# sbokov/AddingDisparityFiltering

Measured on AMD Instinct MI355X. Metric: filtered Mpixels/s (+ achieved HBM GB/s) on 4K disparity, 1/2/4/8 GPUs vs CPU ref, higher is better.
Workload: dtype f32

## Files before the change

addingdisparityfiltering_amd/__init__.py:

```python
from .ximgproc import (
    AdfError,
    COLOR_BGR2GRAY,
    DisparityFilter,
    DisparityWLSFilter,
    FastGlobalSmootherFilter,
    INTER_LINEAR,
    PATH_CONF_BAND,
    PATH_FUSED_FIRST_PASS,
    PATH_MERGED_PREP,
    PATH_SCALED_FUSED,
    PATH_SCALED_HALF,
    SGBM_COST_BT,
    SGBM_COST_CENSUS_DENSE,
    SGBM_COST_CENSUS_SPARSE,
    SOLVER_EXACT,
    SOLVER_WAVE,
    StereoBM,
    StereoMatcher,
    StereoSGBM,
    UNKNOWN_DISPARITY,
    censusTransform,
    computeBadPixelPercent,
    computeMSE,
    createDisparityWLSFilter,
    createDisparityWLSFilterGeneric,
    createFastGlobalSmootherFilter,
    createRightMatcher,
    cvtColor,
    fastGlobalSmootherFilter,
    filterSpeckles,
    releaseCachedMemory,
    getDisparityVis,
    halfSize,
    matcherViews,
    readGT,
    resize,
    speckleWorkspaceBytes,
)

__version__ = "0.1.0"
```

addingdisparityfiltering_amd/_lib.py:

```python
import ctypes as C
import os

_HERE = os.path.dirname(os.path.abspath(__file__))
LIB_PATH = os.environ.get("ADF_WLS_LIB") or os.path.join(_HERE, "libadf_wls.so")

ADF_OK, ADF_EBADARG, ADF_ESIZE, ADF_EHIP, ADF_ENOMEM, ADF_ENODEV = range(6)
SOLVER_EXACT, SOLVER_WAVE = 0, 1
PATH_CONF_BAND, PATH_FUSED_FIRST_PASS, PATH_MERGED_PREP, PATH_SCALED_FUSED, PATH_SCALED_HALF = 1, 2, 4, 8, 16
DEPTH_8U, DEPTH_16S, DEPTH_32F = 0, 3, 5
SGBM_COST_BT, SGBM_COST_CENSUS_DENSE, SGBM_COST_CENSUS_SPARSE = 0, 1, 2


class AdfError(RuntimeError):

    def __init__(self, code, msg):
        super().__init__("adf error %d: %s" % (code, msg))
        self.code = code


class KernelTime(C.Structure):
    _fields_ = [("name", C.c_char * 48), ("launches", C.c_int), ("total_ms", C.c_double),
                ("alg_bytes", C.c_double), ("moved_bytes", C.c_double)]


class Rect(C.Structure):
    _fields_ = [("x", C.c_int), ("y", C.c_int), ("width", C.c_int), ("height", C.c_int)]


_vp, _i, _d, _pd, _sz = C.c_void_p, C.c_int, C.c_double, C.c_ssize_t, C.c_size_t
_FILTER_DEV = [_vp, _i, _vp, _pd, _pd, _vp, _pd, _pd, _i, _i, _i, _vp, _pd, _pd, _vp, _pd, _pd,
               C.POINTER(Rect), _vp]
_FILTER_SCALED_DEV = [_vp, _i, _vp, _pd, _pd, _i, _i, _vp, _pd, _pd, _i, _i, _i, _vp, _pd, _pd, _vp, _pd, _pd,
                      C.POINTER(Rect), _vp]
SYMBOLS = [
    ("adf_version", _i, []),
    ("adf_last_error", C.c_char_p, []),
    ("adf_device_count", _i, []),
    ("adf_device_pci_bus_id", _i, [_i, C.c_char_p, _i]),
    ("adf_wls_create", _i, [C.POINTER(_vp), _i, _i, _i, _i, _i, _i]),
    ("adf_wls_destroy", None, [_vp]),
    ("adf_wls_set_lambda", _i, [_vp, _d]),
    ("adf_wls_get_lambda", _i, [_vp, C.POINTER(_d)]),
    ("adf_wls_set_sigma_color", _i, [_vp, _d]),
    ("adf_wls_get_sigma_color", _i, [_vp, C.POINTER(_d)]),
    ("adf_wls_set_lrc_thresh", _i, [_vp, _i]),
    ("adf_wls_get_lrc_thresh", _i, [_vp, C.POINTER(_i)]),
    ("adf_wls_set_depth_discontinuity_radius", _i, [_vp, _i]),
    ("adf_wls_get_depth_discontinuity_radius", _i, [_vp, C.POINTER(_i)]),
    ("adf_wls_set_fgs_params", _i, [_vp, _d, _i]),
    ("adf_wls_set_solver", _i, [_vp, _i]),
    ("adf_wls_get_solver", _i, [_vp, C.POINTER(_i)]),
    ("adf_wls_get_last_solver", _i, [_vp, C.POINTER(_i)]),
    ("adf_wls_get_last_path", _i, [_vp, C.POINTER(_i)]),
    ("adf_wls_filter_device", _i, _FILTER_DEV),
    ("adf_wls_filter_host", _i, _FILTER_DEV[:-1]),
    ("adf_wls_filter_scaled_device", _i, _FILTER_SCALED_DEV),
    ("adf_wls_filter_scaled_host", _i, _FILTER_SCALED_DEV[:-1]),
    ("adf_wls_filter_f32_device", _i, _FILTER_DEV),
    ("adf_wls_filter_f32_host", _i, _FILTER_DEV[:-1]),
    ("adf_wls_filter_scaled_f32_device", _i, _FILTER_SCALED_DEV),
    ("adf_wls_filter_scaled_f32_host", _i, _FILTER_SCALED_DEV[:-1]),
    ("adf_wls_get_confidence_device", _i, [_vp, _i, _vp, _pd, _vp]),
    ("adf_wls_get_confidence_host", _i, [_vp, _i, _vp, _pd]),
    ("adf_wls_get_device", _i, [_vp, C.POINTER(_i)]),
    ("adf_wls_get_roi", _i, [_vp, C.POINTER(Rect)]),
    ("adf_wls_sync", _i, [_vp, _vp]),
    ("adf_wls_workspace_bytes", _sz, [_vp]),
    ("adf_wls_profile_enable", _i, [_vp, _i]),
    ("adf_wls_profile_read", _i, [_vp, _vp, _i, C.POINTER(_i)]),
    ("adf_fgs_create", _i, [C.POINTER(_vp), _vp, _pd, _i, _i, _i, _d, _d, _d, _i, _i]),
    ("adf_fgs_create_device", _i, [C.POINTER(_vp), _vp, _pd, _i, _i, _i, _d, _d, _d, _i, _i, _vp]),
    ("adf_fgs_destroy", None, [_vp]),
    ("adf_release_cached_memory", None, []),
    ("adf_weight_table_host", _i, [C.c_float, _vp, _i]),
    ("adf_fgs_get_device", _i, [_vp, C.POINTER(_i)]),
    ("adf_fgs_get_solver", _i, [_vp, C.POINTER(_i)]),
    ("adf_fgs_filter_host", _i, [_vp, _vp, _pd, _vp, _pd, _i, _i]),
    ("adf_fgs_filter_device", _i, [_vp, _vp, _pd, _vp, _pd, _i, _i, _vp]),
    ("adf_compute_mse_host", _i, [_vp, _pd, _vp, _pd, _i, _i, C.POINTER(Rect), C.POINTER(_d)]),
    ("adf_compute_mse_device", _i, [_vp, _pd, _vp, _pd, _i, _i, C.POINTER(Rect), C.POINTER(_d), _vp]),
    ("adf_compute_bad_pixel_percent_host", _i, [_vp, _pd, _vp, _pd, _i, _i, C.POINTER(Rect), _i, C.POINTER(_d)]),
    ("adf_compute_bad_pixel_percent_device", _i, [_vp, _pd, _vp, _pd, _i, _i, C.POINTER(Rect), _i, C.POINTER(_d), _vp]),
    ("adf_get_disparity_vis_host", _i, [_vp, _pd, _vp, _pd, _i, _i, _d]),
    ("adf_get_disparity_vis_device", _i, [_vp, _pd, _vp, _pd, _i, _i, _d, _vp]),
    ("adf_bm_create", _i, [C.POINTER(_vp), _i, _i]),
    ("adf_bm_destroy", None, [_vp]),
    ("adf_bm_set_params", _i, [_vp, _i, _i, _i, _i, _i, _i]),
    ("adf_bm_get_device", _i, [_vp, C.POINTER(_i)]),
    ("adf_bm_get_params", _i, [_vp] + [C.POINTER(_i)] * 6),
    ("adf_bm_compute_device", _i, [_vp, _i, _vp, _pd, _pd, _vp, _pd, _pd, _i, _i, _vp, _pd, _pd, _vp]),
    ("adf_bm_compute_both_device", _i, [_vp, _i, _vp, _pd, _pd, _vp, _pd, _pd, _i, _i, _vp, _pd, _pd, _vp, _pd, _pd, _vp]),
    ("adf_bm_compute_host", _i, [_vp, _i, _vp, _pd, _pd, _vp, _pd, _pd, _i, _i, _vp, _pd, _pd]),
    ("adf_sgbm_create", _i, [C.POINTER(_vp), _i, _i, _i]),
    ("adf_sgbm_destroy", None, [_vp]),
    ("adf_sgbm_get_device", _i, [_vp, C.POINTER(_i)]),
    ("adf_sgbm_set_params", _i, [_vp] + [_i] * 8),
    ("adf_sgbm_get_params", _i, [_vp] + [C.POINTER(_i)] * 8),
    ("adf_sgbm_set_disp12_max_diff", _i, [_vp, _i]),
    ("adf_sgbm_get_disp12_max_diff", _i, [_vp, C.POINTER(_i)]),
    ("adf_sgbm_set_cost", _i, [_vp, _i, _i]),
    ("adf_sgbm_get_cost", _i, [_vp, C.POINTER(_i), C.POINTER(_i)]),
    ("adf_sgbm_compute_device", _i, [_vp, _i, _vp, _pd, _pd, _vp, _pd, _pd, _i, _i, _i, _vp, _pd, _pd, _vp]),
    ("adf_sgbm_compute_host", _i, [_vp, _i, _vp, _pd, _pd, _vp, _pd, _pd, _i, _i, _i, _vp, _pd, _pd]),
    ("adf_census_transform_device", _i, [_i, _vp, _pd, _pd, _i, _i, _i, _i, _vp, _pd, _pd, _vp]),
    ("adf_census_transform_host", _i, [_i, _vp, _pd, _pd, _i, _i, _i, _i, _vp, _pd, _pd]),
    ("adf_filter_speckles_workspace_bytes", _sz, [_i, _i, _i]),
    ("adf_filter_speckles_device", _i, [_i, _vp, _pd, _pd, _i, _i, _i, _i, _i, _vp, _sz, _vp]),
    ("adf_filter_speckles_host", _i, [_i, _vp, _pd, _pd, _i, _i, _i, _i, _i]),
    ("adf_half_size", _i, [_i, C.POINTER(_i)]),
    ("adf_prepare_views_device", _i, [_i, _vp, _pd, _pd, _i, _i, _i, _vp, _pd, _pd, _i, _i, _i, _vp]),
    ("adf_prepare_views_host", _i, [_i, _vp, _pd, _pd, _i, _i, _i, _vp, _pd, _pd, _i, _i, _i]),
]

_lib = None


def lib():
    global _lib
    if _lib is None:
        if not os.path.exists(LIB_PATH):
            raise ImportError(
                "%s is missing: build the HIP extension first "
                "(python -c 'import __graft_entry__ as g; g.build()')" % LIB_PATH)
        L = C.CDLL(LIB_PATH)
        for name, res, args in SYMBOLS:
            try:
                fn = getattr(L, name)
            except AttributeError:
                if os.environ.get("ADF_WLS_LIB"):
                    continue
                raise
            fn.restype = res
            fn.argtypes = args
        _lib = L
    return _lib


def check(rc):
    if rc != ADF_OK:
        raise AdfError(rc, lib().adf_last_error().decode("utf-8", "replace"))


def device_pci_bus_id(device):
    buf = C.create_string_buffer(64)
    check(lib().adf_device_pci_bus_id(int(device), buf, 64))
    return buf.value.decode()
```

addingdisparityfiltering_amd/csrc/adf_api.hip:

```cpp
#include "adf_host.h"

#include <cmath>
#include <cstdio>
#include <cstdlib>
#include <cstring>
#include <new>

using namespace adf;

static inline int round_up(int v, int m) { return (v + m - 1) / m * m; }

static Geom make_geom(int W, int H, int rx, int ry, int rw, int rh)
{
    Geom g;
    g.W = W; g.H = H; g.rx = rx; g.ry = ry; g.rw = rw; g.rh = rh;
    g.pw = round_up(rw, 64);
    g.ph = round_up(rh, 64);
    size_t a = (size_t)round_up(rh, TILE_ROWS) * g.pw, b = (size_t)rw * g.ph;
    g.plane = ((a > b ? a : b) + 63) / 64 * 64;
    g.frame = (size_t)W * H;
    g.cx0 = (4 - (rx & 3)) & 3;
    g.cpitch = round_up(W + g.cx0 + 3, 4);
    g.cframe = (size_t)g.cpitch * H;
    return g;
}

static Geom plain_conf_layout(Geom g) { g.cx0 = 0; g.cpitch = g.W; g.cframe = g.frame; return g; }

enum KClass { K_FILL = 0, K_WEIGHTS, K_DISC, K_LRC, K_PROLOGUE, K_PASS_H_FIRST, K_PASS_H, K_PASS_V, K_PASS_V_LAST, K_RESIZE, K_COUNT };
static const char* const kclass_names[K_COUNT] = {"fill_outside", "weights", "discontinuity", "lrc_confidence",
                                                  "plain_prologue", "pass_h_first", "pass_h", "pass_v", "pass_v_last", "resize"};
struct Profiler {
    bool on = false;
    struct Rec { int cls; hipEvent_t a, b; double alg, moved; };
    std::vector<Rec> recs;
    std::vector<hipEvent_t> pool;
    hipEvent_t get()
    {
        if (!pool.empty()) { hipEvent_t e = pool.back(); pool.pop_back(); return e; }
        hipEvent_t e = nullptr;
        if (hipEventCreate(&e) != hipSuccess) return nullptr;
        return e;
    }
    void clear() { for (auto& r : recs) { pool.push_back(r.a); pool.push_back(r.b); } recs.clear(); }
    void destroy() { clear(); for (auto e : pool) hipEventDestroy(e); pool.clear(); }
};
struct ProfScope {
    Profiler* p; hipStream_t st; Profiler::Rec r{};
    ProfScope(Profiler* prof, int cls, double alg, double moved, hipStream_t s) : p(prof && prof->on ? prof : nullptr), st(s)
    {
        if (!p) return;
        r.cls = cls; r.alg = alg; r.moved = moved; r.a = p->get(); r.b = p->get();
        if (r.a) hipEventRecord(r.a, st);
    }
    ~ProfScope()
    {
        if (!p) return;
        if (r.b) hipEventRecord(r.b, st);
        if (r.a && r.b) p->recs.push_back(r);
    }
};

struct SolvePlanes {
    float* CH; float* CV;
    float* D; float* F0; float* F1;
    float* A0; float* A1;
    float* B0; float* B1;
};

struct FinalOut {
    int epilogue; void* out; ptrdiff_t stride, pair_stride; int x0, y0, cn, c;
};

static double epilogue_bytes(int epilogue)
{
    return (epilogue == EPI_F32 || epilogue == EPI_WLS_CONF_F32) ? 4.0 : epilogue == EPI_U8 ? 1.0 : 2.0;
}

template <class Args>
static void set_final_out(Args& a, const FinalOut& fo)
{
    a.out = fo.out; a.out_stride = fo.stride; a.out_pair_stride = fo.pair_stride;
    a.out_x0 = fo.x0; a.out_y0 = fo.y0; a.out_cn = fo.cn; a.out_c = fo.c;
}

static int run_passes(bool wave, const Geom& g, const SolvePlanes& p, int n_rhs, float lambda, float atten, int num_iter,
                      const FinalOut& fo, int n_pairs, hipStream_t st, Profiler* prof = nullptr,
                      const FusedInputs* fuse = nullptr)
{
    const double px = (double)g.rw * g.rh * n_pairs;
    float lam = lambda;
    for (int it = 0; it < num_iter; it++, lam *= atten) {
        const bool fused = it == 0 && fuse, last = it == num_iter - 1;
        const int epi = last ? fo.epilogue : EPI_PLANES;
        const double lo_b = (fused && fuse->lo_conf) ? 6.0 * fuse->lo_scale_x * fuse->lo_scale_y : 6.0;
        const double hb = fused ? (4.0 + lo_b + 8.0) * px : (4.0 + 8.0 * n_rhs) * px;
        const double out_b = (last ? epilogue_bytes(fo.epilogue) : 4.0 * n_rhs) * px;
        const double vb = (4.0 + 4.0 * n_rhs) * px + out_b;
        if (wave) {
            WavePassArgs h{}, v{};
            h.C = p.CH; h.U0 = p.A0; h.U1 = p.A1;
            h.nscan = g.rh; h.len = g.rw; h.pitch = g.pw; h.plane = g.plane; h.lambda = lam;
            if (fused) h.fuse = *fuse;
            v.C = p.CV; v.U0 = p.A0; v.U1 = p.A1;
            v.nscan = g.rw; v.len = g.rh; v.pitch = g.pw; v.plane = g.plane; v.lambda = lam;
            if (last) set_final_out(v, fo);
            {
                ProfScope ps(prof, fused ? K_PASS_H_FIRST : K_PASS_H, hb, hb, st);
                HIP_TRY(launch_wave_hpass(h, n_rhs, n_pairs, st));
            }
            ProfScope ps(prof, last ? K_PASS_V_LAST : K_PASS_V, vb, vb, st);
            HIP_TRY(launch_wave_vpass(v, n_rhs, epi, n_pairs, st));
        } else {
            PassArgs h{}, v{};
            h.C = p.CH; h.U0 = p.A0; h.U1 = p.A1; h.D = p.D; h.F0 = p.F0; h.F1 = p.F1; h.O0 = p.B0; h.O1 = p.B1;
            h.nscan = g.rh; h.len = g.rw; h.pitch_in = g.ph; h.pitch_out = g.pw; h.plane = g.plane; h.lambda = lam;
            v.C = p.CV; v.U0 = p.B0; v.U1 = p.B1; v.D = p.D; v.F0 = p.F0; v.F1 = p.F1; v.O0 = p.A0; v.O1 = p.A1;
            v.nscan = g.rw; v.len = g.rh; v.pitch_in = g.pw; v.pitch_out = g.ph; v.plane = g.plane; v.lambda = lam;
            if (last) set_final_out(v, fo);
            {
                ProfScope ps(prof, K_PASS_H, hb, (12.0 + 16.0 * n_rhs) * px, st);
                HIP_TRY(launch_exact_pass(h, n_rhs, EPI_PLANES, n_pairs, st));
            }
            ProfScope ps(prof, last ? K_PASS_V_LAST : K_PASS_V, vb, (12.0 + 12.0 * n_rhs) * px + out_b, st);
            HIP_TRY(launch_exact_pass(v, n_rhs, epi, n_pairs, st));
        }
    }
    return ADF_OK;
}

static bool wave_fits(const Geom& g)
{
    return g.rw >= 2 && g.rh >= 2 && g.rw <= wave_max_row_len() && g.rh <= wave_max_col_len();
}

struct ConfResize {
    float* clo; int dW, dH; adf_rect rlo;
    Geom ghi;
    bool band_map;
    int n_pairs;
};

struct adf_wls {
    int device = 0;
    int left_offset = 0, right_offset = 0, top_offset = 0, bottom_offset = 0;
    int min_disp = 0;
    bool use_confidence = true;
    double lambda = 8000.0, sigma_color = 1.0;
    int lrc_thresh = 24, disc_radius = 5;
    float roll_off = 0.001f;
    double atten = 0.25; int num_iter = 3;
    int solver = ADF_SOLVER_WAVE;
    int last_solver = ADF_SOLVER_WAVE;
    adf_rect roi{0, 0, 0, 0};
    int last_W = 0, last_H = 0, last_pairs = 0;
    int last_cpitch = 0, last_cx0 = 0;
    long long conf_sig[4] = {0, 0, 0, 0};
    int last_path = 0;
    Lut lut;
    DevBuf ws;
    DevBuf conf;
    DevBuf stage;
    DevBuf scaled;
    size_t ws_limit = (size_t)64 << 30;
    Profiler prof;
    long long ws_sig[8] = {0, 0, 0, 0, 0, 0, 0, 0};
    hipStream_t side = nullptr;
    hipEvent_t ev_fork = nullptr, ev_join = nullptr;
    bool overlap = true;
    struct LazyConf { bool pending = false; ConfResize resize{}; } lazy_conf;
    bool scaled_half = true;
    bool scaled_fuse = true;
    bool conf_band = true;
    bool merge_small = true;
    static bool null_caller_of(hipStream_t s) { return s == nullptr || s == hipStreamLegacy || s == hipStreamPerThread; }
    int ensure_side(hipStream_t caller)
    {
        if (side) return ADF_OK;
        int least = 0, greatest = 0, prio = 0, cp = 0;
        if (hipDeviceGetStreamPriorityRange(&least, &greatest) != hipSuccess) { least = greatest = 0; (void)hipGetLastError(); }
        if (null_caller_of(caller) || stream_is_capturing(caller) || hipStreamGetPriority(caller, &cp) != hipSuccess) { cp = 0; (void)hipGetLastError(); }
        prio = (cp != greatest) ? greatest : (greatest < least ? greatest + 1 : greatest);
        if (null_caller_of(caller)) HIP_TRY(hipStreamCreateWithFlags(&side, hipStreamNonBlocking));
        else HIP_TRY(hipStreamCreateWithPriority(&side, hipStreamNonBlocking, prio));
        HIP_TRY(hipEventCreateWithFlags(&ev_fork, hipEventDisableTiming));
        HIP_TRY(hipEventCreateWithFlags(&ev_join, hipEventDisableTiming));
        return ADF_OK;
    }
};

extern "C" int adf_wls_create(adf_wls_t** out, int use_confidence, int l, int r, int t, int b, int min_disp)
{
    if (!out) return fail(ADF_EBADARG, "adf_wls_create: out is NULL");
    *out = nullptr;
    if (l < 0 || r < 0 || t < 0 || b < 0) return fail(ADF_EBADARG, "adf_wls_create: negative offset");
    int n = 0;
    if (hipGetDeviceCount(&n) != hipSuccess || n <= 0)
        return fail(ADF_ENODEV, "adf_wls_create: no HIP device visible");
    adf_wls* h = new (std::nothrow) adf_wls();
    if (!h) return fail(ADF_ENOMEM, "adf_wls_create: out of host memory");
    if (hipGetDevice(&h->device) != hipSuccess) { delete h; return fail(ADF_EHIP, "hipGetDevice failed"); }
    h->use_confidence = use_confidence != 0;
    h->left_offset = l; h->right_offset = r; h->top_offset = t; h->bottom_offset = b;
    h->min_disp = 0; (void)min_disp;
    if (const char* e = getenv("ADF_WS_LIMIT_GB")) {
        double gb = atof(e);
        if (gb > 0) h->ws_limit = (size_t)(gb * (double)((size_t)1 << 30));
    }
    if (const char* e = getenv("ADF_NO_OVERLAP")) h->overlap = atoi(e) == 0;
    if (const char* e = getenv("ADF_CONF_BAND")) h->conf_band = atoi(e) != 0;
    if (const char* e = getenv("ADF_SCALED_FUSE")) h->scaled_fuse = atoi(e) != 0;
    if (const char* e = getenv("ADF_LO_HALF")) h->scaled_half = atoi(e) != 0;
    if (const char* e = getenv("ADF_MERGE_SMALL")) h->merge_small = atoi(e) != 0;
    *out = h;
    return ADF_OK;
}

extern "C" void adf_wls_destroy(adf_wls_t* h)
{
    if (!h) return;
    DeviceScope ds(h->device);
    h->lut.release(); h->ws.release(); h->conf.release(); h->stage.release(); h->scaled.release();
    h->prof.destroy();
    if (h->ev_fork) hipEventDestroy(h->ev_fork);
    if (h->ev_join) hipEventDestroy(h->ev_join);
    if (h->side) hipStreamDestroy(h->side);
    delete h;
}


extern "C" int adf_wls_set_lambda(adf_wls_t* h, double v) { NEED_HANDLE(h); h->lambda = v; return ADF_OK; }
extern "C" int adf_wls_get_lambda(const adf_wls_t* h, double* v) { NEED_HANDLE(h); if (v) *v = h->lambda; return ADF_OK; }
extern "C" int adf_wls_set_sigma_color(adf_wls_t* h, double v) { NEED_HANDLE(h); h->sigma_color = v; return ADF_OK; }
extern "C" int adf_wls_get_sigma_color(const adf_wls_t* h, double* v) { NEED_HANDLE(h); if (v) *v = h->sigma_color; return ADF_OK; }
extern "C" int adf_wls_set_lrc_thresh(adf_wls_t* h, int v) { NEED_HANDLE(h); h->lrc_thresh = v; return ADF_OK; }
extern "C" int adf_wls_get_lrc_thresh(const adf_wls_t* h, int* v) { NEED_HANDLE(h); if (v) *v = h->lrc_thresh; return ADF_OK; }
extern "C" int adf_wls_set_depth_discontinuity_radius(adf_wls_t* h, int v) { NEED_HANDLE(h); h->disc_radius = v; return ADF_OK; }
extern "C" int adf_wls_get_depth_discontinuity_radius(const adf_wls_t* h, int* v) { NEED_HANDLE(h); if (v) *v = h->disc_radius; return ADF_OK; }

extern "C" int adf_wls_set_fgs_params(adf_wls_t* h, double atten, int num_iter)
{
    NEED_HANDLE(h);
    if (num_iter < 1) return fail(ADF_EBADARG, "num_iter must be >= 1 (FGS.cpp:143)");
    h->atten = atten; h->num_iter = num_iter;
    return ADF_OK;
}

extern "C" int adf_wls_set_solver(adf_wls_t* h, int solver)
{
    NEED_HANDLE(h);
    if (solver != ADF_SOLVER_EXACT && solver != ADF_SOLVER_WAVE) return fail(ADF_EBADARG, "unknown solver %d", solver);
    h->solver = solver;
    return ADF_OK;
}
extern "C" int adf_wls_get_solver(const adf_wls_t* h, int* v) { NEED_HANDLE(h); if (v) *v = h->solver; return ADF_OK; }
extern "C" int adf_wls_get_last_solver(const adf_wls_t* h, int* v) { NEED_HANDLE(h); if (v) *v = h->last_solver; return ADF_OK; }
extern "C" int adf_wls_get_last_path(const adf_wls_t* h, int* v) { NEED_HANDLE(h); if (v) *v = h->last_path; return ADF_OK; }

extern "C" int adf_wls_get_device(const adf_wls_t* h, int* device) { NEED_HANDLE(h); if (device) *device = h->device; return ADF_OK; }
extern "C" int adf_wls_get_roi(const adf_wls_t* h, adf_rect* roi) { NEED_HANDLE(h); if (roi) *roi = h->roi; return ADF_OK; }
extern "C" size_t adf_wls_workspace_bytes(const adf_wls_t* h)
{
    return h ? h->ws.bytes + h->conf.bytes + h->stage.bytes + h->scaled.bytes + h->lut.bytes() : 0;
}

extern "C" int adf_wls_sync(adf_wls_t* h, void* stream)
{
    NEED_HANDLE(h);
    DeviceScope ds(h->device);
    HIP_TRY(hipStreamSynchronize((hipStream_t)stream));
    return ADF_OK;
}

static int ensure_conf_planes(adf_wls* h, const Geom& g, int n_pairs, hipStream_t st)
{
    int rc = h->conf.reserve(g.cframe * sizeof(float) * (size_t)n_pairs, st, FILL_ZERO);
    if (rc) return rc;
    const long long sig[4] = {g.W, g.H, g.cx0, n_pairs};
    if (memcmp(sig, h->conf_sig, sizeof(sig)) != 0) {
        HIP_TRY(hipMemsetAsync(h->conf.p, 0, h->conf.bytes, st));
        memcpy(h->conf_sig, sig, sizeof(sig));
    }
    return ADF_OK;
}

static size_t wls_pair_ws_bytes(const Geom& g, bool conf, bool wave, bool disc_maps)
{
    size_t planes = wave ? (conf ? 4 : 3) : (conf ? 9 : 6);
    return planes * g.plane * sizeof(float) + (conf && disc_maps ? 2 * g.frame * sizeof(float) : 0);
}

static int resolve_roi(const adf_wls* h, const adf_rect* roi_in, int w, int hgt, adf_rect& roi)
{
    if (roi_in && roi_in->width * roi_in->height != 0) roi = *roi_in;
    else roi = adf_rect{h->left_offset, h->top_offset, w - h->left_offset - h->right_offset, hgt - h->top_offset - h->bottom_offset};
    if (roi.width <= 0 || roi.height <= 0 || roi.x < 0 || roi.y < 0 || roi.x + roi.width > w || roi.y + roi.height > hgt)
        return fail(ADF_ESIZE, "ROI (%d,%d,%d,%d) does not fit a %dx%d map", roi.x, roi.y, roi.width, roi.height, w, hgt);
    return ADF_OK;
}

static int check_right_map(const int16_t* dispR, ptrdiff_t sR, int w)
{
    if (!dispR) return fail(ADF_EBADARG, "disparity_map_right is required with use_confidence");
    if (sR < (ptrdiff_t)w * 2) return fail(ADF_ESIZE, "right disparity stride smaller than a row");
    return ADF_OK;
}

static int check_radius(const adf_wls* h)
{
    if (h->disc_radius < 0 || h->disc_radius > max_disc_radius())
        return fail(ADF_EBADARG, "depth discontinuity radius %d outside [0,%d]", h->disc_radius, max_disc_radius());
    return ADF_OK;
}

static float* const UNALLOCATED = reinterpret_cast<float*>(uintptr_t(256));

static WavePassArgs first_pass_probe(const FusedInputs& f, int len)
{
    WavePassArgs a{};
    a.fuse = f; a.len = len;
    return a;
}

static FusedInputs view_fuse(const float* conf, const int16_t* dl, ptrdiff_t sL, ptrdiff_t psL, const Geom& g)
{
    FusedInputs f{};
    f.conf_in = conf; f.conf_frame = g.cframe; f.conf_pitch = g.cpitch; f.conf_x0 = g.cx0 + g.rx; f.conf_y0 = g.ry;
    f.dl_in = dl; f.dl_stride = sL; f.dl_pair_stride = psL; f.dl_x0 = g.rx; f.dl_y0 = g.ry;
    return f;
}

struct ScaledStage {
    const int16_t* dispL; ptrdiff_t sL, psL;
    const int16_t* dispR; ptrdiff_t sR, psR;
    float resize_factor, x_ratio;
    char* dhi; size_t dhi_bytes;
    float *cl, *cr;
    ConfResize lo;
    bool fuse_lo;
    float* taps;
};

static FusedInputs lo_fuse(const adf_wls* h, const ScaledStage& s, int first, const Geom& g)
{
    const ConfResize& c = s.lo;
    const size_t lo = (size_t)c.dW * c.dH;
    FusedInputs f{};
    f.lo_conf = c.clo + (size_t)first * lo; f.lo_conf_stride = c.dW; f.lo_conf_pair = (ptrdiff_t)lo;
    f.lo_dl = (const int16_t*)((const char*)s.dispL + (ptrdiff_t)first * s.psL); f.lo_dl_stride = s.sL; f.lo_dl_pair = s.psL;
    f.lo_w = c.dW; f.lo_h = c.dH; f.hi_x0 = g.rx; f.hi_y0 = g.ry;
    f.lo_scale_x = (double)c.dW / c.ghi.W; f.lo_scale_y = (double)c.dH / c.ghi.H; f.lo_post_scale = s.x_ratio;
    if (c.band_map) {
        f.lo_zero_outside = 1; f.lo_vx0 = c.rlo.x; f.lo_vy0 = c.rlo.y; f.lo_vx1 = c.rlo.x + c.rlo.width; f.lo_vy1 = c.rlo.y + c.rlo.height;
    }
    f.lo_taps = s.taps; f.lo_half = h->scaled_half ? 1 : 0;
    return f;
}

static int resize_conf_planes(adf_wls_t* h, const ConfResize& c, hipStream_t st, Profiler* prof)
{
    const size_t lo = (size_t)c.dW * c.dH;
    const Geom& ghi = c.ghi;
    const double Fhi = (double)ghi.W * ghi.H * c.n_pairs;
    ResizeArgs rc32{c.clo, (ptrdiff_t)c.dW * 4, (ptrdiff_t)(lo * 4), c.dW, c.dH, (float*)h->conf.p + ghi.cx0, (ptrdiff_t)ghi.cpitch * 4,
                    (ptrdiff_t)(ghi.cframe * 4), ghi.W, ghi.H, (double)c.dW / ghi.W, (double)c.dH / ghi.H, 1.0f, 0};
    if (c.band_map) { rc32.zero_outside = 1; rc32.vx0 = c.rlo.x; rc32.vy0 = c.rlo.y; rc32.vx1 = c.rlo.x + c.rlo.width; rc32.vy1 = c.rlo.y + c.rlo.height; }
    ProfScope ps(prof, K_RESIZE, 4.0 * Fhi + 4.0 * (double)lo * c.n_pairs, 4.0 * Fhi + 4.0 * (double)lo * c.n_pairs, st);
    HIP_TRY(launch_resize_linear(rc32, c.n_pairs, st));
    return ADF_OK;
}

static int scaled_conf_map(adf_wls_t* h, const ScaledStage& s, hipStream_t st, Profiler* prof)
{
    const ConfResize& c = s.lo;
    const Geom glo = plain_conf_layout(make_geom(c.dW, c.dH, c.rlo.x, c.rlo.y, c.rlo.width, c.rlo.height));
    const size_t lo = (size_t)c.dW * c.dH;
    const double Plo = (double)c.rlo.width * c.rlo.height * c.n_pairs;
    const int rrx = c.dW - (c.rlo.x + c.rlo.width);
    const float roll_off = h->roll_off / (s.resize_factor * s.resize_factor);
    const int thresh_lo = (int)(s.resize_factor * h->lrc_thresh);
    if (c.band_map) {
        ConfBandArgs ba{s.dispL, s.sL, s.psL, s.dispR, s.sR, s.psR, c.clo, glo, rrx, thresh_lo, h->disc_radius, roll_off, 0};
        ProfScope ps(prof, K_LRC, 8.0 * Plo, 8.0 * Plo, st);
        HIP_TRY(launch_conf_band(ba, c.n_pairs, st));
        return ADF_OK;
    }
    DiscArgs da{{s.dispL, s.dispR}, {s.sL, s.sR}, {s.psL, s.psR}, {c.rlo.x, rrx}, c.rlo.y, c.rlo.width, c.rlo.height,
                h->disc_radius, roll_off, {s.cl, s.cr}, c.dW, lo, -1};
    {
        ProfScope ps(prof, K_DISC, 4.0 * Plo, 12.0 * Plo, st);
        HIP_TRY(launch_discontinuity(da, c.n_pairs, st));
    }
    LrcArgs la{s.dispL, s.sL, s.psL, s.dispR, s.sR, s.psR, s.cl, s.cr, c.clo, nullptr, 0, 0, 0, 0, nullptr, nullptr, glo, rrx, thresh_lo, ORIENT_N};
    ProfScope ps(prof, K_LRC, 4.0 * (double)lo * c.n_pairs, 4.0 * (double)lo * c.n_pairs + 12.0 * Plo, st);
    HIP_TRY(launch_lrc_prologue(la, c.n_pairs, st));
    return ADF_OK;
}

static int scaled_resize(adf_wls_t* h, const ScaledStage& s, hipStream_t st, Profiler* prof)
{
    const ConfResize& c = s.lo;
    int rc = h->use_confidence ? resize_conf_planes(h, c, st, prof) : ADF_OK;
    if (rc) return rc;
    const int W = c.ghi.W, H = c.ghi.H;
    const size_t lo = (size_t)c.dW * c.dH;
    const double Fhi = (double)W * H * c.n_pairs;
    ResizeArgs r16{s.dispL, s.sL, s.psL, c.dW, c.dH, s.dhi, (ptrdiff_t)W * 2, (ptrdiff_t)s.dhi_bytes, W, H, (double)c.dW / W, (double)c.dH / H, s.x_ratio, 1};
    ProfScope ps(prof, K_RESIZE, 2.0 * Fhi + 2.0 * (double)lo * c.n_pairs, 2.0 * Fhi + 2.0 * (double)lo * c.n_pairs, st);
    HIP_TRY(launch_resize_linear(r16, c.n_pairs, st));
    return ADF_OK;
}

enum ConfStage {
    CONF_NONE,
    CONF_SCALED,
    CONF_SCALED_LO,
    CONF_MERGED,
    CONF_BAND,
    CONF_LEFT,
    CONF_TWO_KERNEL,
};

struct ChunkPlan {
    ConfStage stage;
    bool fork_weights;
    bool outside_on_side;
};

struct WlsPlan {
    bool wave;
    bool fused_first;
    bool band;
    size_t per_pair; int chunk;
    ChunkPlan full, tail;
    int path;
};

static ChunkPlan plan_chunk(const adf_wls* h, ConfStage stage, bool wave)
{
    const bool fork = stage != CONF_NONE && stage != CONF_MERGED && h->overlap;
    return ChunkPlan{stage, fork, fork && wave && stage != CONF_TWO_KERNEL};
}

static WlsPlan plan_wls(const adf_wls* h, const Geom& g, int n_pairs, const int16_t* dispL, ptrdiff_t sL, ptrdiff_t psL,
                        ptrdiff_t sG, int gch, const ScaledStage* scaled)
{
    WlsPlan p{};
    const bool conf = h->use_confidence;
    p.wave = h->solver == ADF_SOLVER_WAVE && wave_fits(g);
    ConfStage stage = !conf ? CONF_NONE
                    : scaled ? (scaled->fuse_lo ? CONF_SCALED_LO : CONF_SCALED)
                    : (p.wave && h->disc_radius <= conf_left_max_radius()) ? CONF_LEFT : CONF_TWO_KERNEL;
    const float* planes = h->conf.p ? (const float*)h->conf.p : UNALLOCATED;
    p.fused_first = stage == CONF_SCALED_LO ||
                    ((stage == CONF_SCALED || stage == CONF_LEFT) && p.wave &&
                     wave_hpass_can_fuse(first_pass_probe(view_fuse(planes, dispL, sL, psL, g), g.rw)));
    p.band = stage == CONF_LEFT && p.fused_first && h->conf_band && conf_band_fits(g, h->disc_radius);
    if (p.band) stage = CONF_BAND;
    p.per_pair = wls_pair_ws_bytes(g, conf, p.wave, !p.band);
    p.chunk = (int)(h->ws_limit / p.per_pair);
    if (p.chunk < 1) p.chunk = 1;
    if (p.chunk > n_pairs) p.chunk = n_pairs;
    auto chunk_of = [&](int n) {
        const bool merged = p.band && h->merge_small && prep_small_fits(g, h->disc_radius, gch, n) && prep_small_guide_fits(g, sG, gch);
        return plan_chunk(h, merged ? CONF_MERGED : stage, p.wave);
    };
    p.full = chunk_of(p.chunk);
    p.tail = chunk_of(n_pairs % p.chunk ? n_pairs % p.chunk : p.chunk);
    p.path = ((p.band || (scaled && scaled->lo.band_map)) ? ADF_PATH_CONF_BAND : 0) |
             (p.fused_first ? ADF_PATH_FUSED_FIRST_PASS : 0) |
             ((p.full.stage == CONF_MERGED || p.tail.stage == CONF_MERGED) ? ADF_PATH_MERGED_PREP : 0);
    if (stage == CONF_SCALED_LO)
        p.path |= ADF_PATH_SCALED_FUSED |
                  (wave_hpass_lo_half(first_pass_probe(lo_fuse(h, *scaled, 0, g), g.rw)) ? ADF_PATH_SCALED_HALF : 0);
    return p;
}

struct OutMap {
    void* p; ptrdiff_t stride, pair_stride; bool f32;
    size_t esz() const { return f32 ? sizeof(float) : sizeof(int16_t); }
};

static int wls_filter_impl(adf_wls_t* h, int n_pairs,
                           const int16_t* dispL, ptrdiff_t sL, ptrdiff_t psL,
                           const uint8_t* view, ptrdiff_t sG, ptrdiff_t psG, int gch, int W, int H,
                           const OutMap& om,
                           const int16_t* dispR, ptrdiff_t sR, ptrdiff_t psR,
                           const adf_rect* roi_in, hipStream_t st, const ScaledStage* scaled = nullptr)
{
    NEED_HANDLE(h);
    if (!dispL || W <= 0 || H <= 0) return fail(ADF_EBADARG, "disparity_map_left is empty");
    if (!view || (gch != 1 && gch != 3)) return fail(ADF_EBADARG, "left_view must be CV_8UC1 or CV_8UC3");
    void* const out = om.p;
    const ptrdiff_t sO = om.stride, psO = om.pair_stride;
    const double ob_px = (double)om.esz();
    if (!out) return fail(ADF_EBADARG, "filtered_disparity_map is NULL");
    if (n_pairs < 1) return fail(ADF_EBADARG, "n_pairs must be >= 1");
    if (sL < (ptrdiff_t)W * 2 || sO < (ptrdiff_t)(W * om.esz()) || sG < (ptrdiff_t)W * gch)
        return fail(ADF_ESIZE, "row stride smaller than a row");
    if (om.f32 && ((reinterpret_cast<uintptr_t>(out) | (uintptr_t)sO | (uintptr_t)psO) & 3u))
        return fail(ADF_EBADARG, "a float filtered_disparity_map needs a 4-byte aligned base and strides");
    const bool conf = h->use_confidence;
    int rc;
    if (conf && !scaled && (rc = check_right_map(dispR, sR, W))) return rc;
    if (h->lambda < 0 || h->sigma_color < 0) return fail(ADF_EBADARG, "lambda and sigma_color must be >= 0 (FGS.cpp:143)");
    adf_rect roi;
    if ((rc = resolve_roi(h, roi_in, W, H, roi))) return rc;
    if (conf && (rc = check_radius(h))) return rc;

    DeviceScope ds(h->device);
    const Geom g = make_geom(W, H, roi.x, roi.y, roi.width, roi.height);
    h->lazy_conf.pending = false;
    h->roi = roi; h->last_W = W; h->last_H = H; h->last_pairs = n_pairs;
    h->last_cpitch = g.cpitch; h->last_cx0 = g.cx0; h->last_path = 0;

    if ((rc = h->lut.ensure((float)h->sigma_color, st))) return rc;
    const WlsPlan plan = plan_wls(h, g, n_pairs, dispL, sL, psL, sG, gch, scaled);
    const bool wave = plan.wave;
    h->last_solver = wave ? ADF_SOLVER_WAVE : ADF_SOLVER_EXACT;
    if ((rc = h->ws.reserve(plan.per_pair * (size_t)plan.chunk, st, FILL_ZERO))) return rc;
    if (conf && !scaled && (rc = ensure_conf_planes(h, g, n_pairs, st))) return rc;
    {
        const long long sig[8] = {W, H, roi.x, roi.y, roi.width, roi.height, (long long)plan.band * 4 + (long long)wave * 2 + conf, plan.chunk};
        if (memcmp(sig, h->ws_sig, sizeof(sig)) != 0) {
            HIP_TRY(hipMemsetAsync(h->ws.p, 0, h->ws.bytes, st));
            memcpy(h->ws_sig, sig, sizeof(sig));
        }
    }
    float* base = (float*)h->ws.p;
    auto take = [&](size_t elems) { float* p = base; base += elems * (size_t)plan.chunk; return p; };
    SolvePlanes p{};
    p.CH = take(g.plane); p.CV = take(g.plane); p.A0 = take(g.plane);
    if (!wave) { p.D = take(g.plane); p.F0 = take(g.plane); p.B0 = take(g.plane); }
    float *cL = nullptr, *cR = nullptr;
    if (conf) {
        p.A1 = take(g.plane);
        if (!wave) { p.F1 = take(g.plane); p.B1 = take(g.plane); }
        if (!plan.band) { cL = take(g.frame); cR = take(g.frame); }
    }
    const int orient_h = wave ? ORIENT_N : ORIENT_T;
    const int orient_u2 = wave ? ORIENT_PAIR : ORIENT_T;
    const int orient_cv = wave ? ORIENT_STRIP : ORIENT_N;
    const int16_t fill = (int16_t)(16 * (h->min_disp - 1));
    const int rrx = W - (roi.x + roi.width);
    const int thresh = (int)(1.0f * h->lrc_thresh);
    Profiler* prof = &h->prof;
    h->last_path = plan.path;

    for (int first = 0; first < n_pairs; first += plan.chunk) {
        const int n = (n_pairs - first < plan.chunk) ? n_pairs - first : plan.chunk;
        const ChunkPlan& cp = n == plan.chunk ? plan.full : plan.tail;
        const int16_t* dL = (const int16_t*)((const char*)dispL + (ptrdiff_t)first * psL);
        const int16_t* dR = dispR ? (const int16_t*)((const char*)dispR + (ptrdiff_t)first * psR) : nullptr;
        const uint8_t* gv = view + (ptrdiff_t)first * psG;
        void* o = (char*)out + (ptrdiff_t)first * psO;
        float* confp = conf ? (float*)h->conf.p + (size_t)first * g.cframe : nullptr;
        const double F = (double)g.frame * n, P = (double)g.rw * g.rh * n;
        OutsideArgs oa{o, sO, psO, fill, om.f32 ? 1 : 0, scaled ? nullptr : confp, g};
        const double ob = ((oa.conf ? 4.0 : 0.0) + ob_px) * (F - P);
        auto fill_outside = [&](hipStream_t s) { ProfScope ps(prof, K_FILL, ob, ob, s); return launch_outside(oa, n, s); };
        WeightArgs wa{gv, sG, psG, gch, h->lut.cur, p.CH, p.CV, orient_h, orient_cv, g,
                      wave ? nullptr : p.B0};
        ConfBandArgs ba{dL, sL, psL, dR, sR, psR, confp, g, rrx, thresh, h->disc_radius, h->roll_off, 0};
        DiscArgs da{{dL, dR}, {sL, sR}, {psL, psR}, {roi.x, rrx}, roi.y, roi.width, roi.height, h->disc_radius, h->roll_off,
                    {cL, cR}, W, g.frame, cp.stage == CONF_LEFT ? 1 : -1};
        const FusedInputs fuse = cp.stage == CONF_SCALED_LO ? lo_fuse(h, *scaled, first, g) : view_fuse(confp, dL, sL, psL, g);

        hipStream_t wst = st;
        if (cp.fork_weights) {
            if ((rc = h->ensure_side(st))) return rc;
            HIP_TRY(hipEventRecord(h->ev_fork, st));
            HIP_TRY(hipStreamWaitEvent(h->side, h->ev_fork, 0));
            wst = h->side;
        }
        if (cp.stage == CONF_NONE || cp.outside_on_side) HIP_TRY(fill_outside(wst));
        if (cp.stage == CONF_NONE && scaled && first == 0 && (rc = scaled_resize(h, *scaled, st, prof))) return rc;
        if (cp.stage != CONF_MERGED) {
            ProfScope ps(prof, K_WEIGHTS, (gch + 8.0) * P, (gch + 8.0) * P, wst);
            HIP_TRY(launch_weights(wa, n, wst));
        }
        if (cp.fork_weights) HIP_TRY(hipEventRecord(h->ev_join, h->side));

        switch (cp.stage) {
        case CONF_NONE: {
            PlainPrologueArgs pa{dL, sL, psL, ADF_16S, 1, 0, p.A0, g, orient_h};
            ProfScope ps(prof, K_PROLOGUE, 6.0 * P, 6.0 * P, st);
            HIP_TRY(launch_plain_prologue(pa, n, st));
            break;
        }
        case CONF_SCALED: {
            if (!cp.outside_on_side) HIP_TRY(fill_outside(st));
            if (first == 0 && ((rc = scaled_conf_map(h, *scaled, st, prof)) || (rc = scaled_resize(h, *scaled, st, prof)))) return rc;
            if (plan.fused_first) break;
            PlainPrologueArgs pa{dL, sL, psL, ADF_16S, 1, 0, p.A0, g, orient_u2, confp, p.A1};
            ProfScope ps(prof, K_PROLOGUE, 14.0 * P, 14.0 * P, st);
            HIP_TRY(launch_plain_prologue(pa, n, st));
            break;
        }
        case CONF_SCALED_LO:
            if (!cp.outside_on_side) HIP_TRY(fill_outside(st));
            if (first != 0) break;
            if ((rc = scaled_conf_map(h, *scaled, st, prof))) return rc;
            if (!stream_is_capturing(st)) h->lazy_conf = adf_wls::LazyConf{true, scaled->lo};
            else if ((rc = resize_conf_planes(h, scaled->lo, st, prof))) return rc;
            break;
        case CONF_MERGED: {
            const double b = (8.0 + gch + 8.0) * P + (4.0 + ob_px) * (F - P);
            ProfScope ps(prof, K_LRC, b, b, st);
            HIP_TRY(launch_prep_small(ba, wa, oa, n, st));
            break;
        }
        case CONF_BAND: {
            {
                ProfScope ps(prof, K_LRC, 8.0 * P, 8.0 * P, st);
                HIP_TRY(launch_conf_band(ba, n, st));
            }
            if (!cp.outside_on_side) HIP_TRY(fill_outside(st));
            break;
        }
        case CONF_LEFT: {
            {
                ProfScope ps(prof, K_DISC, 2.0 * P, 6.0 * P, st);
                HIP_TRY(launch_discontinuity(da, n, st));
            }
            const bool fused = plan.fused_first;
            ConfLeftArgs ca{dL, sL, psL, dR, sR, psR, cR, confp, fused ? nullptr : p.A0, fused ? nullptr : p.A1,
                            g, rrx, thresh, h->disc_radius, h->roll_off};
            {
                const double wu = fused ? 0.0 : 8.0;
                ProfScope ps(prof, K_LRC, (4.0 + wu) * P, (12.0 + wu) * P, st);
                HIP_TRY(launch_conf_left(ca, n, st));
            }
            if (!cp.outside_on_side) HIP_TRY(fill_outside(st));
            break;
        }
        case CONF_TWO_KERNEL: {
            {
                ProfScope ps(prof, K_DISC, 4.0 * P, 12.0 * P, st);
                HIP_TRY(launch_discontinuity(da, n, st));
            }
            LrcArgs la{dL, sL, psL, dR, sR, psR, cL, cR, confp, o, sO, psO, fill, om.f32 ? 1 : 0, p.A0, p.A1, g, rrx, thresh, orient_u2};
            ProfScope ps(prof, K_LRC, 4.0 * F + 8.0 * P + ob_px * (F - P), 4.0 * F + 20.0 * P + ob_px * (F - P), st);
            HIP_TRY(launch_lrc_prologue(la, n, st));
            break;
        }
        }
        if (cp.fork_weights) HIP_TRY(hipStreamWaitEvent(st, h->ev_join, 0));
        const int epi = conf ? (om.f32 ? EPI_WLS_CONF_F32 : EPI_WLS_CONF) : (om.f32 ? EPI_F32 : EPI_I16);
        FinalOut fo{epi, o, sO, psO, roi.x, roi.y, 1, 0};
        rc = run_passes(wave, g, p, conf ? 2 : 1, (float)h->lambda, (float)h->atten, h->num_iter, fo, n, st, prof,
                        plan.fused_first ? &fuse : nullptr);
        if (rc) return rc;
    }
    return ADF_OK;
}

static int wls_filter_scaled_device(adf_wls_t* h, int n_pairs,
                                    const int16_t* dispL, ptrdiff_t sL, ptrdiff_t psL, int dW, int dH,
                                    const uint8_t* view, ptrdiff_t sG, ptrdiff_t psG, int gch, int W, int H,
                                    const OutMap& om,
                                    const int16_t* dispR, ptrdiff_t sR, ptrdiff_t psR,
                                    const adf_rect* roi_in, hipStream_t st)
{
    NEED_HANDLE(h);
    if (dW == W && dH == H)
        return wls_filter_impl(h, n_pairs, dispL, sL, psL, view, sG, psG, gch, W, H, om, dispR, sR, psR, roi_in, st);
    if (!dispL || dW <= 0 || dH <= 0 || W <= 0 || H <= 0) return fail(ADF_EBADARG, "disparity_map_left is empty");
    if (n_pairs < 1) return fail(ADF_EBADARG, "n_pairs must be >= 1");
    if (sL < (ptrdiff_t)dW * 2) return fail(ADF_ESIZE, "row stride smaller than a row");
    const bool conf = h->use_confidence;
    int rc;
    if (conf && ((rc = check_right_map(dispR, sR, dW)) || (rc = check_radius(h)))) return rc;
    adf_rect rlo;
    if ((rc = resolve_roi(h, roi_in, dW, dH, rlo))) return rc;
    const float resize_factor = dW / (float)W;
    const float x_ratio = W / (float)dW, y_ratio = H / (float)dH;
    adf_rect rhi{(int)(rlo.x * x_ratio), (int)(rlo.y * y_ratio), (int)(rlo.width * x_ratio), (int)(rlo.height * y_ratio)};
    if (rhi.width <= 0 || rhi.height <= 0 || rhi.x + rhi.width > W || rhi.y + rhi.height > H)
        return fail(ADF_ESIZE, "scaled ROI (%d,%d,%d,%d) does not fit the %dx%d view", rhi.x, rhi.y, rhi.width, rhi.height, W, H);

    DeviceScope ds(h->device);
    h->lazy_conf.pending = false;
    const size_t lo = (size_t)dW * dH, hi = (size_t)W * H;
    const Geom ghi = make_geom(W, H, rhi.x, rhi.y, rhi.width, rhi.height);
    ScaledStage s{dispL, sL, psL, dispR, sR, psR, resize_factor, x_ratio, nullptr, 0, nullptr, nullptr,
                  ConfResize{UNALLOCATED, dW, dH, rlo, ghi, false, n_pairs}, false, nullptr};
    s.lo.band_map = conf && h->conf_band &&
                    conf_band_fits(plain_conf_layout(make_geom(dW, dH, rlo.x, rlo.y, rlo.width, rlo.height)), h->disc_radius);
    s.fuse_lo = conf && h->scaled_fuse && h->solver == ADF_SOLVER_WAVE && wave_fits(ghi) &&
                wave_hpass_can_fuse_lo(first_pass_probe(lo_fuse(h, s, 0, ghi), ghi.rw));
    s.dhi_bytes = s.fuse_lo ? 0 : (hi * 2 + 255) / 256 * 256;
    const size_t maps_bytes = ((size_t)n_pairs * (s.dhi_bytes + (conf ? 3 * lo * sizeof(float) : 0)) + 255) / 256 * 256;
    const size_t need = maps_bytes + (s.fuse_lo ? 2 * ((size_t)rhi.width + 4) * sizeof(float) : 0);
    if ((rc = h->scaled.reserve(need, st, FILL_ZERO))) return rc;
    s.dhi = (char*)h->scaled.p;
    s.cl = (float*)(s.dhi + (size_t)n_pairs * s.dhi_bytes);
    s.cr = s.cl + (size_t)n_pairs * lo;
    s.lo.clo = s.cr + (size_t)n_pairs * lo;
    s.taps = s.fuse_lo ? (float*)((char*)h->scaled.p + maps_bytes) : nullptr;
    if (conf && (rc = ensure_conf_planes(h, ghi, n_pairs, st))) return rc;
    rc = wls_filter_impl(h, n_pairs, s.fuse_lo ? dispL : (const int16_t*)s.dhi, (ptrdiff_t)W * 2, (ptrdiff_t)s.dhi_bytes,
                         view, sG, psG, gch, W, H, om, nullptr, 0, 0, &rhi, st, &s);
    h->roi = rlo;
    return rc;
}

static int wls_filter_scaled_host(adf_wls_t* h, int n_pairs,
                                  const int16_t* dispL, ptrdiff_t sL, ptrdiff_t psL, int dW, int dH,
                                  const uint8_t* view, ptrdiff_t sG, ptrdiff_t psG, int gch, int W, int H,
                                  const OutMap& om,
                                  const int16_t* dispR, ptrdiff_t sR, ptrdiff_t psR,
                                  const adf_rect* roi)
{
    NEED_HANDLE(h);
    if (!dispL || !view || !om.p || W <= 0 || H <= 0 || dW <= 0 || dH <= 0 || n_pairs < 1)
        return fail(ADF_EBADARG, "adf_wls_filter_host: empty input");
    if (gch != 1 && gch != 3) return fail(ADF_EBADARG, "left_view must be CV_8UC1 or CV_8UC3");
    if (h->use_confidence && !dispR) return fail(ADF_EBADARG, "disparity_map_right is required with use_confidence");
    DeviceScope ds(h->device);
    hipStream_t st = nullptr;
    const size_t orow = (size_t)W * om.esz();
    const size_t dbytes = (size_t)dW * dH * 2, obytes = orow * H, gbytes = (size_t)W * H * gch;
    const size_t dpad = (dbytes + 255) / 256 * 256, opad = (obytes + 255) / 256 * 256, gpad = (gbytes + 255) / 256 * 256;
    const size_t need = (size_t)n_pairs * (2 * dpad + opad + gpad);
    int rc = h->stage.reserve(need, st, FILL_ZERO);
    if (rc) return rc;
    char* dLd = (char*)h->stage.p;
    char* dRd = dLd + (size_t)n_pairs * dpad;
    char* od = dRd + (size_t)n_pairs * dpad;
    char* gd = od + (size_t)n_pairs * opad;
    if ((rc = copy_images(dLd, (size_t)dW * 2, dpad, dispL, sL, psL, (size_t)dW * 2, dH, n_pairs, hipMemcpyHostToDevice, st))) return rc;
    if (dispR && (rc = copy_images(dRd, (size_t)dW * 2, dpad, dispR, sR, psR, (size_t)dW * 2, dH, n_pairs, hipMemcpyHostToDevice, st))) return rc;
    if ((rc = copy_images(gd, (size_t)W * gch, gpad, view, sG, psG, (size_t)W * gch, H, n_pairs, hipMemcpyHostToDevice, st))) return rc;
    rc = wls_filter_scaled_device(h, n_pairs, (const int16_t*)dLd, (ptrdiff_t)dW * 2, (ptrdiff_t)dpad, dW, dH,
                                  (const uint8_t*)gd, (ptrdiff_t)W * gch, (ptrdiff_t)gpad, gch, W, H,
                                  OutMap{od, (ptrdiff_t)orow, (ptrdiff_t)opad, om.f32},
                                  dispR ? (const int16_t*)dRd : nullptr, (ptrdiff_t)dW * 2, (ptrdiff_t)dpad, roi, st);
    if (rc) return rc;
    if ((rc = copy_images(om.p, om.stride, om.pair_stride, od, orow, opad, orow, H, n_pairs, hipMemcpyDeviceToHost, st))) return rc;
    HIP_TRY(hipStreamSynchronize(st));
    return ADF_OK;
}

#define ADF_WLS_SAME_ARGS const int16_t* dispL, ptrdiff_t sL, ptrdiff_t psL, \
                          const uint8_t* view, ptrdiff_t sG, ptrdiff_t psG, int gch, int W, int H
#define ADF_WLS_SCALED_ARGS const int16_t* dispL, ptrdiff_t sL, ptrdiff_t psL, int dW, int dH, \
                            const uint8_t* view, ptrdiff_t sG, ptrdiff_t psG, int gch, int W, int H
#define ADF_WLS_RIGHT_ARGS const int16_t* dispR, ptrdiff_t sR, ptrdiff_t psR, const adf_rect* roi
#define ADF_WLS_ENTRIES(SUFFIX, T, F32)                                                                                       \
    extern "C" int adf_wls_filter##SUFFIX##_device(adf_wls_t* h, int n_pairs, ADF_WLS_SAME_ARGS, T* out, ptrdiff_t sO,        \
                                                   ptrdiff_t psO, ADF_WLS_RIGHT_ARGS, void* stream)                           \
    {                                                                                                                         \
        return wls_filter_impl(h, n_pairs, dispL, sL, psL, view, sG, psG, gch, W, H, OutMap{out, sO, psO, F32}, dispR, sR,    \
                               psR, roi, (hipStream_t)stream);                                                                \
    }                                                                                                                         \
    extern "C" int adf_wls_filter_scaled##SUFFIX##_device(adf_wls_t* h, int n_pairs, ADF_WLS_SCALED_ARGS, T* out,             \
                                                          ptrdiff_t sO, ptrdiff_t psO, ADF_WLS_RIGHT_ARGS, void* stream)      \
    {                                                                                                                         \
        return wls_filter_scaled_device(h, n_pairs, dispL, sL, psL, dW, dH, view, sG, psG, gch, W, H,                         \
                                        OutMap{out, sO, psO, F32}, dispR, sR, psR, roi, (hipStream_t)stream);                 \
    }                                                                                                                         \
    extern "C" int adf_wls_filter_scaled##SUFFIX##_host(adf_wls_t* h, int n_pairs, ADF_WLS_SCALED_ARGS, T* out, ptrdiff_t sO, \
                                                        ptrdiff_t psO, ADF_WLS_RIGHT_ARGS)                                    \
    {                                                                                                                         \
        return wls_filter_scaled_host(h, n_pairs, dispL, sL, psL, dW, dH, view, sG, psG, gch, W, H,                           \
                                      OutMap{out, sO, psO, F32}, dispR, sR, psR, roi);                                        \
    }                                                                                                                         \
    extern "C" int adf_wls_filter##SUFFIX##_host(adf_wls_t* h, int n_pairs, ADF_WLS_SAME_ARGS, T* out, ptrdiff_t sO,          \
                                                 ptrdiff_t psO, ADF_WLS_RIGHT_ARGS)                                           \
    {                                                                                                                         \
        return wls_filter_scaled_host(h, n_pairs, dispL, sL, psL, W, H, view, sG, psG, gch, W, H, OutMap{out, sO, psO, F32},  \
                                      dispR, sR, psR, roi);                                                                   \
    }
ADF_WLS_ENTRIES(, int16_t, false)
ADF_WLS_ENTRIES(_f32, float, true)
#undef ADF_WLS_ENTRIES
#undef ADF_WLS_SAME_ARGS
#undef ADF_WLS_SCALED_ARGS
#undef ADF_WLS_RIGHT_ARGS

extern "C" int adf_wls_profile_enable(adf_wls_t* h, int on)
{
    NEED_HANDLE(h);
    DeviceScope ds(h->device);
    h->prof.clear();
    h->prof.on = on != 0;
    return ADF_OK;
}

extern "C" int adf_wls_profile_read(adf_wls_t* h, adf_kernel_time* out, int capacity, int* count)
{
    NEED_HANDLE(h);
    if (!out || !count || capacity < 1) return fail(ADF_EBADARG, "adf_wls_profile_read: bad output buffer");
    DeviceScope ds(h->device);
    adf_kernel_time acc[K_COUNT];
    memset(acc, 0, sizeof(acc));
    for (int k = 0; k < K_COUNT; k++) snprintf(acc[k].name, sizeof(acc[k].name), "%s", kclass_names[k]);
    for (auto& r : h->prof.recs) {
        HIP_TRY(hipEventSynchronize(r.b));
        float ms = 0.0f;
        HIP_TRY(hipEventElapsedTime(&ms, r.a, r.b));
        acc[r.cls].launches++; acc[r.cls].total_ms += ms; acc[r.cls].alg_bytes += r.alg; acc[r.cls].moved_bytes += r.moved;
    }
    int n = 0;
    for (int k = 0; k < K_COUNT && n < capacity; k++)
        if (acc[k].launches) out[n++] = acc[k];
    *count = n;
    return ADF_OK;
}

static int conf_copy(adf_wls_t* h, int pair, float* dst, ptrdiff_t stride, hipMemcpyKind kind, hipStream_t st)
{
    if (!dst) return fail(ADF_EBADARG, "confidence destination is NULL");
    if (!h->use_confidence || !h->conf.p || h->last_pairs == 0)
        return fail(ADF_EBADARG, "no confidence map: filter() has not run with use_confidence");
    if (pair < 0 || pair >= h->last_pairs) return fail(ADF_EBADARG, "pair %d out of range [0,%d)", pair, h->last_pairs);
    if (stride < (ptrdiff_t)h->last_W * 4) return fail(ADF_ESIZE, "confidence stride smaller than a row");
    if (h->lazy_conf.pending) {
        int rc = resize_conf_planes(h, h->lazy_conf.resize, st, nullptr);
        if (rc) return rc;
        h->lazy_conf.pending = false;
    }
    const float* src = (const float*)h->conf.p + (size_t)pair * h->last_cpitch * h->last_H + h->last_cx0;
    HIP_TRY(hipMemcpy2DAsync(dst, stride, src, (size_t)h->last_cpitch * 4, (size_t)h->last_W * 4, h->last_H, kind, st));
    return ADF_OK;
}

extern "C" int adf_wls_get_confidence_device(adf_wls_t* h, int pair, float* dst, ptrdiff_t stride, void* stream)
{
    NEED_HANDLE(h);
    DeviceScope ds(h->device);
    return conf_copy(h, pair, dst, stride, hipMemcpyDeviceToDevice, (hipStream_t)stream);
}

extern "C" int adf_wls_get_confidence_host(adf_wls_t* h, int pair, float* dst, ptrdiff_t stride)
{
    NEED_HANDLE(h);
    DeviceScope ds(h->device);
    int rc = conf_copy(h, pair, dst, stride, hipMemcpyDeviceToHost, nullptr);
    if (rc) return rc;
    HIP_TRY(hipStreamSynchronize(nullptr));
    return ADF_OK;
}

struct adf_fgs {
    int device = 0;
    int w = 0, h = 0;
    float lambda = 0, sigma = 0, atten = 0.25f; int num_iter = 3; int solver = ADF_SOLVER_EXACT;
    Geom g{};
    Lut lut;
    void* block = nullptr; size_t block_bytes = 0;
    DevBuf planes, io;
    hipEvent_t busy = nullptr;
    bool in_capture = false;
};

static int fgs_begin(adf_fgs* f, hipStream_t st)
{
    if (f->busy && !stream_is_capturing(st)) HIP_TRY(hipStreamWaitEvent(st, f->busy, 0));
    return ADF_OK;
}

static int fgs_end(adf_fgs* f, hipStream_t st)
{
    if (stream_is_capturing(st)) { f->in_capture = true; return ADF_OK; }
    if (f->busy) HIP_TRY(hipEventRecord(f->busy, st));
    return ADF_OK;
}

static int fgs_create_impl(adf_fgs_t** out, const uint8_t* guide, ptrdiff_t gstride, int gch, int w, int hgt,
                           double lambda, double sigma_color, double atten, int num_iter, int solver,
                           bool guide_on_device, hipStream_t st)
{
    if (!out) return fail(ADF_EBADARG, "adf_fgs_create: out is NULL");
    *out = nullptr;
    if (!guide || w <= 0 || hgt <= 0) return fail(ADF_EBADARG, "guide is empty");
    if (lambda < 0 || sigma_color < 0 || num_iter < 1) return fail(ADF_EBADARG, "lambda>=0, sigma_color>=0, num_iter>=1 required");
    if (gch != 1 && gch != 3) return fail(ADF_EBADARG, "guide must be CV_8UC1 or CV_8UC3");
    if (gstride < (ptrdiff_t)w * gch) return fail(ADF_ESIZE, "guide stride smaller than a row");
    if (solver != ADF_SOLVER_EXACT && solver != ADF_SOLVER_WAVE) return fail(ADF_EBADARG, "unknown solver %d", solver);
    int n = 0;
    if (hipGetDeviceCount(&n) != hipSuccess || n <= 0) return fail(ADF_ENODEV, "adf_fgs_create: no HIP device visible");
    adf_fgs* f = new (std::nothrow) adf_fgs();
    if (!f) return fail(ADF_ENOMEM, "out of host memory");
    hipGetDevice(&f->device);
    f->w = w; f->h = hgt;
    f->lambda = (float)lambda; f->sigma = (float)sigma_color; f->atten = (float)atten;
    f->num_iter = num_iter;
    f->g = make_geom(w, hgt, 0, 0, w, hgt);
    f->solver = (solver == ADF_SOLVER_WAVE && wave_fits(f->g)) ? ADF_SOLVER_WAVE : ADF_SOLVER_EXACT;
    int rc = f->lut.ensure(f->sigma, st);
    if (rc) { adf_fgs_destroy(f); return rc; }
    const size_t gbytes = (size_t)w * hgt * gch;
    const size_t planes_bytes = (6 * f->g.plane * sizeof(float) + 255) / 256 * 256;
    const size_t io_bytes = ((gbytes > (size_t)w * hgt * 16 ? gbytes : (size_t)w * hgt * 16) + 255) / 256 * 256;
    hipError_t e = hipSuccess;
    f->block = cache_take(f->device, planes_bytes + io_bytes, st, &f->block_bytes);
    if (!f->block) {
        e = device_malloc(&f->block, planes_bytes + io_bytes);
        if (e != hipSuccess) {
            f->block = nullptr; adf_fgs_destroy(f);
            return fail(e == hipErrorOutOfMemory ? ADF_ENOMEM : ADF_EHIP, "adf_fgs_create: %s", hipGetErrorString(e));
        }
        f->block_bytes = planes_bytes + io_bytes;
    }
    f->planes.p = f->block; f->planes.bytes = planes_bytes;
    f->io.p = (char*)f->block + planes_bytes; f->io.bytes = io_bytes;
    e = hipMemsetAsync(f->block, 0, planes_bytes + io_bytes, st);
    if (e == hipSuccess) e = hipEventCreateWithFlags(&f->busy, hipEventDisableTiming);
    if (e == hipSuccess) e = guide_on_device
        ? hipMemcpy2DAsync(f->io.p, (size_t)w * gch, guide, gstride, (size_t)w * gch, hgt, hipMemcpyDeviceToDevice, st)
        : hipMemcpy2D(f->io.p, (size_t)w * gch, guide, gstride, (size_t)w * gch, hgt, hipMemcpyHostToDevice);
    if (e == hipSuccess) {
        float* base = (float*)f->planes.p;
        WeightArgs wa{(const uint8_t*)f->io.p, (ptrdiff_t)w * gch, 0, gch, f->lut.cur,
                      base, base + f->g.plane, f->solver == ADF_SOLVER_WAVE ? ORIENT_N : ORIENT_T,
                      f->solver == ADF_SOLVER_WAVE ? ORIENT_STRIP : ORIENT_N, f->g,
                      f->solver == ADF_SOLVER_WAVE ? nullptr : base + 5 * f->g.plane};
        e = launch_weights(wa, 1, st);
    }
    if (e == hipSuccess && !guide_on_device) e = hipStreamSynchronize(st);
    if (e != hipSuccess) { hipStreamSynchronize(st); adf_fgs_destroy(f); return fail(ADF_EHIP, "adf_fgs_create: %s", hipGetErrorString(e)); }
    if ((rc = fgs_end(f, st))) { hipStreamSynchronize(st); adf_fgs_destroy(f); return rc; }
    *out = f;
    return ADF_OK;
}

extern "C" int adf_fgs_create(adf_fgs_t** out, const uint8_t* guide, ptrdiff_t gstride, int gch, int w, int hgt,
                              double lambda, double sigma_color, double atten, int num_iter, int solver)
{
    return fgs_create_impl(out, guide, gstride, gch, w, hgt, lambda, sigma_color, atten, num_iter, solver, false, nullptr);
}

extern "C" int adf_fgs_create_device(adf_fgs_t** out, const uint8_t* guide, ptrdiff_t gstride, int gch, int w, int hgt,
                                     double lambda, double sigma_color, double atten, int num_iter, int solver, void* stream)
{
    return fgs_create_impl(out, guide, gstride, gch, w, hgt, lambda, sigma_color, atten, num_iter, solver, true,
                           (hipStream_t)stream);
}

extern "C" int adf_fgs_get_device(const adf_fgs_t* f, int* device) { NEED_HANDLE(f); if (device) *device = f->device; return ADF_OK; }
extern "C" int adf_fgs_get_solver(const adf_fgs_t* f, int* solver) { NEED_HANDLE(f); if (solver) *solver = f->solver; return ADF_OK; }

extern "C" void adf_fgs_destroy(adf_fgs_t* f)
{
    if (!f) return;
    DeviceScope ds(f->device);
    if (f->block) {
        if (f->busy && !f->in_capture) {
            cache_give_event(f->device, f->block, f->block_bytes, f->busy);
            f->busy = nullptr;
        } else {
            hipDeviceSynchronize();
            hipFree(f->block);
// ... 79 lines not shown
```

addingdisparityfiltering_amd/csrc/adf_internal.h:

```cpp
#pragma once

#include <hip/hip_runtime.h>
#include <stddef.h>
#include <stdint.h>
#include "../../include/adf_wls.h"

#define ADF_LUT_LEVELS (3 * 256 * 256)
#define ADF_EPS 1e-43f

namespace adf {

struct Geom {
    int W, H;
    int rx, ry, rw, rh;
    int pw, ph;
    size_t plane;
    size_t frame;
    int cpitch, cx0;
    size_t cframe;
};

enum Orient { ORIENT_N = 0, ORIENT_T = 1, ORIENT_PAIR = 2, ORIENT_STRIP = 3 };
#define ADF_STRIP 16
constexpr int TILE_ROWS = 2;

enum Epilogue {
    EPI_PLANES = 0,
    EPI_WLS_CONF = 1,
    EPI_I16 = 2,
    EPI_F32 = 3,
    EPI_U8 = 4,
    EPI_WLS_CONF_F32 = 5
};
constexpr int N_EPILOGUES = EPI_WLS_CONF_F32 + 1;

struct DiscArgs {
    const int16_t* disp[2]; ptrdiff_t stride[2], pair_stride[2];
    int rx[2]; int ry, rw, rh;
    int radius; float roll_off;
    float* dst[2]; int W; size_t frame;
    int only_view;
};

struct ConfLeftArgs {
    const int16_t* dL; ptrdiff_t sL, psL;
    const int16_t* dR; ptrdiff_t sR, psR;
    const float* cR;
    float* conf;
    float* U0; float* U1;
    Geom g; int rrx; int thresh;
    int radius; float roll_off;
};

struct ConfBandArgs {
    const int16_t* dL; ptrdiff_t sL, psL;
    const int16_t* dR; ptrdiff_t sR, psR;
    float* conf;
    Geom g; int rrx; int thresh;
    int radius; float roll_off;
    int rows_per_band;
};

struct OutsideArgs {
    void* out; ptrdiff_t stride, pair_stride; int16_t fill; int out_f32;
    float* conf;
    Geom g;
};

struct LrcArgs {
    const int16_t* dL; ptrdiff_t sL, psL;
    const int16_t* dR; ptrdiff_t sR, psR;
    const float* cL; const float* cR;
    float* conf;
    void* out; ptrdiff_t sO, psO; int16_t fill; int out_f32;
    float* U0; float* U1;
    Geom g; int rrx;
    int thresh; int orient;
};

struct PlainPrologueArgs {
    const void* src; ptrdiff_t stride, pair_stride;
    int depth, cn, c;
    float* U0; Geom g; int orient;
    const float* conf; float* U1;
    int pair2, c2;
};

struct ResizeArgs {
    const void* src; ptrdiff_t sstride, spair; int sw, sh;
    void* dst; ptrdiff_t dstride, dpair; int dw, dh;
    double scale_x, scale_y;
    float post_scale; int is16;
    int zero_outside = 0, vx0 = 0, vy0 = 0, vx1 = 0, vy1 = 0;
};

struct WeightArgs {
    const uint8_t* guide; ptrdiff_t stride, pair_stride; int ch;
    const float* lut;
    float* chor; float* cvert; int chor_orient, cvert_orient;
    Geom g;
    float* scratch;
};

struct PassArgs {
    const float* C; const float* U0; const float* U1;
    float* D; float* F0; float* F1;
    float* O0; float* O1;
    void* out; ptrdiff_t out_stride, out_pair_stride;
    int out_x0, out_y0, out_cn, out_c;
    int nscan, len, pitch_in, pitch_out;
    size_t plane;
    float lambda;
};

struct FusedInputs {
    const float* conf_in; size_t conf_frame; int conf_pitch, conf_x0, conf_y0;
    const int16_t* dl_in; ptrdiff_t dl_stride, dl_pair_stride; int dl_x0, dl_y0;
    const float* lo_conf; ptrdiff_t lo_conf_stride, lo_conf_pair;
    const int16_t* lo_dl; ptrdiff_t lo_dl_stride, lo_dl_pair;
    int lo_w, lo_h, hi_x0, hi_y0;
    double lo_scale_x, lo_scale_y; float lo_post_scale;
    int lo_zero_outside, lo_vx0, lo_vy0, lo_vx1, lo_vy1;
    int lo_half;
    float* lo_taps;
};

struct WavePassArgs {
    const float* C; float* U0; float* U1;
    FusedInputs fuse;
    void* out; ptrdiff_t out_stride, out_pair_stride;
    int out_x0, out_y0, out_cn, out_c;
    int nscan, len, pitch;
    size_t plane;
    float lambda;
};
static_assert(sizeof(WavePassArgs) == 280 && offsetof(WavePassArgs, out) == 208 && offsetof(WavePassArgs, nscan) == 248 &&
              offsetof(WavePassArgs, plane) == 264 && offsetof(WavePassArgs, lambda) == 272, "WavePassArgs layout");

hipError_t launch_discontinuity(const DiscArgs& a, int n_pairs, hipStream_t st);
hipError_t launch_lrc_prologue(const LrcArgs& a, int n_pairs, hipStream_t st);
hipError_t launch_conf_left(const ConfLeftArgs& a, int n_pairs, hipStream_t st);
hipError_t launch_outside(const OutsideArgs& a, int n_pairs, hipStream_t st);
bool conf_band_fits(const Geom& g, int radius);
hipError_t launch_conf_band(const ConfBandArgs& a, int n_pairs, hipStream_t st);
bool prep_small_guide_fits(const Geom& g, ptrdiff_t guide_stride, int channels);
bool prep_small_fits(const Geom& g, int radius, int channels, int n_pairs);
hipError_t launch_prep_small(const ConfBandArgs& c, const WeightArgs& w, const OutsideArgs& o, int n_pairs, hipStream_t st);
int conf_left_max_radius();
hipError_t launch_plain_prologue(const PlainPrologueArgs& a, int n_pairs, hipStream_t st);
hipError_t launch_weights(const WeightArgs& a, int n_pairs, hipStream_t st);
hipError_t launch_resize_linear(const ResizeArgs& a, int n_pairs, hipStream_t st);
hipError_t launch_exact_pass(const PassArgs& a, int n_rhs, int epilogue, int n_pairs, hipStream_t st);
hipError_t launch_wave_hpass(const WavePassArgs& a, int n_rhs, int n_pairs, hipStream_t st);
hipError_t launch_wave_vpass(const WavePassArgs& a, int n_rhs, int epilogue, int n_pairs, hipStream_t st);
int wave_max_row_len();
bool wave_hpass_can_fuse(const WavePassArgs& a);
bool wave_hpass_can_fuse_lo(const WavePassArgs& a);
bool wave_hpass_lo_half(const WavePassArgs& a);
int wave_max_col_len();
int max_disc_radius();

namespace tile {
constexpr int TX = 64;
constexpr int TY = 32;
constexpr int NT = 256;
}

#if defined(__HIPCC__)
__device__ __forceinline__ size_t pair_index(int i, int j, int pw)
{
    constexpr int TR = TILE_ROWS;
    return (size_t)(i / TR) * (size_t)(2 * TR * pw) + (size_t)((j >> 4) * (32 * TR) + (i % TR) * 32 + (j & 15));
}
__device__ __forceinline__ size_t strip_index(int i, int j, int rh)
{
    return ((size_t)(j >> 4) * (size_t)rh + (size_t)i) * ADF_STRIP + (size_t)(j & 15);
}
struct RhsPlanes { float* U0; float* U1; };
__device__ __forceinline__ RhsPlanes rhs_planes(float* U0, float* U1, int orient, size_t pz, size_t plane)
{
    const bool pair = orient == ORIENT_PAIR;
    float* u0 = U0 + pz * (pair ? 2 : 1) * plane;
    return RhsPlanes{u0, pair ? u0 + ADF_STRIP : U1 ? U1 + pz * plane : nullptr};
}
__device__ __forceinline__ size_t rhs_index(int orient, int i, int j, const Geom& g)
{
    return orient == ORIENT_PAIR ? pair_index(i, j, g.pw) : orient == ORIENT_T ? (size_t)j * g.ph + i : (size_t)i * g.pw + j;
}
struct RhsTile {
    float t0[tile::TX * (tile::TY + 1)], t1[tile::TX * (tile::TY + 1)];
    __device__ __forceinline__ void stage(int tx, int y, float v0, float v1) { t0[tx * (tile::TY + 1) + y] = v0; t1[tx * (tile::TY + 1) + y] = v1; }
    __device__ __forceinline__ void store(float* U0, float* U1, const Geom& g, int j0, int i0) const
    {
        __syncthreads();
#pragma unroll
        for (int m = 0; m < tile::TX / 8; m++) {
            const int cidx = threadIdx.x / tile::TY + 8 * m, ridx = threadIdx.x % tile::TY, j = j0 + cidx, i = i0 + ridx;
            if ((unsigned)j < (unsigned)g.rw && (unsigned)i < (unsigned)g.rh) {
                const size_t o = rhs_index(ORIENT_T, i, j, g);
                U0[o] = t0[cidx * (tile::TY + 1) + ridx];
                if (U1) U1[o] = t1[cidx * (tile::TY + 1) + ridx];
            }
        }
    }
};
__device__ __forceinline__ void store_fill(void* map, ptrdiff_t row_offset_bytes, int j, int16_t fill, int f32)
{
    char* row = reinterpret_cast<char*>(map) + row_offset_bytes;
    if (f32) reinterpret_cast<float*>(row)[j] = (float)fill;
    else reinterpret_cast<int16_t*>(row)[j] = fill;
}
__device__ __forceinline__ float wls_f32_value(float x) { return !(__builtin_fabsf(x) < 2147483648.0f) ? -32768.0f : x; }
__device__ __forceinline__ int16_t sat16(float v)
{
    if (!(v >= -2147483648.0f && v < 2147483648.0f)) return (int16_t)-32768;
    float r = rintf(v);
    r = fminf(fmaxf(r, -32768.0f), 32767.0f);
    return (int16_t)(int)r;
}
__device__ __forceinline__ uint8_t sat8(float v)
{
    if (!(v >= -2147483648.0f && v < 2147483648.0f)) return (uint8_t)0;
    float r = rintf(v);
    r = fminf(fmaxf(r, 0.0f), 255.0f);
    return (uint8_t)(int)r;
}
__device__ __forceinline__ int reflect101(int p, int len)
{
    if (len == 1) return 0;
    while (p < 0 || p >= len) p = p < 0 ? -p : 2 * (len - 1) - p;
    return p;
}
#endif

}
```

addingdisparityfiltering_amd/csrc/fgs_wave_h.hip:

```cpp
#include "fgs_wave_common.h"

#include <algorithm>

namespace adf {

namespace {
using namespace wave;

constexpr int H_TWO_WAVE_MAX = 60;

constexpr int FUSE_NONE = 0, FUSE_VIEW = 1, FUSE_LO = 2, FUSE_LO_HALF = 3;

typedef float v4f __attribute__((ext_vector_type(4)));

struct RowPos {
    int lane, wv;
    int v0;
    int nvec;
    int nvecU;
    size_t off;
    size_t offU;
};

template <int M, bool PAIR, int NW>
__device__ __forceinline__ RowPos row_pos(const WavePassArgs& a)
{
    constexpr int TR = TILE_ROWS;
    RowPos p;
    p.lane = threadIdx.x & 63; p.wv = NW == 2 ? (int)(threadIdx.x >> 6) : 0;
    p.v0 = p.wv * 16 * M;
    p.off = (size_t)blockIdx.y * a.plane + (size_t)blockIdx.x * a.pitch;
    p.nvec = a.pitch >> 2;
    p.offU = PAIR ? (size_t)blockIdx.y * 2 * a.plane + (size_t)(blockIdx.x / TR) * (size_t)(2 * TR * a.pitch) + (size_t)(blockIdx.x % TR) * 32 : p.off;
    p.nvecU = PAIR ? 2 * p.nvec : p.nvec;
    return p;
}

template <bool PAIR>
__device__ __forceinline__ constexpr int rhs_vec(int q) { return PAIR ? (((q >> 3) * (8 * TILE_ROWS)) + (q & 7)) : q; }

__device__ __forceinline__ constexpr int pair_slot(int j) { return ((j >> 4) << 3) + ((j & 15) >> 2); }

__device__ __forceinline__ float4 load_nt(const float4* p)
{
    const v4f q = __builtin_nontemporal_load(reinterpret_cast<const v4f*>(p));
    return make_float4(q.x, q.y, q.z, q.w);
}
__device__ __forceinline__ void store_nt(float4 q, float4* p)
{
    const v4f o = {q.x, q.y, q.z, q.w};
    __builtin_nontemporal_store(o, reinterpret_cast<v4f*>(p));
}


__device__ __forceinline__ float4 load_c(const WavePassArgs& a, const RowPos& p, int k)
{
    const int idx = p.v0 + 64 * k + p.lane;
    float4 t = make_float4(0.f, 0.f, 0.f, 0.f);
    if (idx < p.nvec) t = load_nt(reinterpret_cast<const float4*>(a.C + p.off) + idx);
    return t;
}

template <int M, int R>
__device__ __forceinline__ void load_planes(const WavePassArgs& a, const RowPos& p, float4 (&tC)[M / 4], float4 (&t0)[M / 4], float4 (&t1)[M / 4])
{
    constexpr bool PAIR = R > 1;
    constexpr int MQ = M / 4;
    const float4* s0 = reinterpret_cast<const float4*>(a.U0 + p.offU);
    const int u0 = PAIR ? 2 * p.v0 : p.v0;
#pragma unroll
    for (int k = 0; k < MQ; k++) {
        const int uidx = u0 + 64 * k + p.lane;
        tC[k] = load_c(a, p, k);
        t0[k] = make_float4(0.f, 0.f, 0.f, 0.f); t1[k] = t0[k];
        if (uidx < p.nvecU) t0[k] = load_nt(s0 + rhs_vec<PAIR>(uidx));
        if (PAIR && uidx + 64 * MQ < p.nvecU) t1[k] = load_nt(s0 + rhs_vec<PAIR>(uidx + 64 * MQ));
    }
}

__device__ __forceinline__ int fused_vecs(int len) { return (len >> 2) + ((len & 3) ? 1 : 0); }

template <int M>
__device__ __forceinline__ void load_fused_view(const WavePassArgs& a, const RowPos& p, float4 (&tC)[M / 4], float4 (&t0)[M / 4], float4 (&t1)[M / 4])
{
    constexpr int MQ = M / 4;
    typedef short v4s_u __attribute__((ext_vector_type(4), aligned(2)));
    const float4* sF = reinterpret_cast<const float4*>(a.fuse.conf_in + (size_t)blockIdx.y * a.fuse.conf_frame +
                                                       (size_t)(a.fuse.conf_y0 + blockIdx.x) * a.fuse.conf_pitch + a.fuse.conf_x0);
    const char* sD = reinterpret_cast<const char*>(a.fuse.dl_in) + (ptrdiff_t)blockIdx.y * a.fuse.dl_pair_stride +
                     (ptrdiff_t)(a.fuse.dl_y0 + blockIdx.x) * a.fuse.dl_stride + (ptrdiff_t)a.fuse.dl_x0 * 2;
    const int nfull = a.len >> 2, rem = a.len & 3;
    const int nfused = fused_vecs(a.len);
    const unsigned dl_last = (unsigned)a.len * 2u - 8u;
    short4 draw[MQ];
#pragma unroll
    for (int k = 0; k < MQ; k++) {
        const int idx = p.v0 + 64 * k + p.lane;
        tC[k] = load_c(a, p, k);
        t0[k] = make_float4(0.f, 0.f, 0.f, 0.f); t1[k] = t0[k];
        draw[k] = make_short4(0, 0, 0, 0);
        if (idx < nfused) {
            const unsigned doff = min((unsigned)idx * 8u, dl_last);
            t1[k] = load_nt(sF + idx);
            const v4s_u dq = __builtin_nontemporal_load(reinterpret_cast<const v4s_u*>(sD + doff));
            draw[k] = make_short4(dq.x, dq.y, dq.z, dq.w);
        }
    }
    const int tl = nfull - p.v0;
    const int ktail = (rem && tl >= 0 && tl < 16 * M) ? (tl >> 6) : -1;
#pragma unroll
    for (int k = 0; k < MQ; k++) {
        if (k == ktail && p.lane == (tl & 63)) {
            const int sh = 16 * (4 - rem);
            unsigned long long w = (unsigned long long)(unsigned short)draw[k].x | ((unsigned long long)(unsigned short)draw[k].y << 16) |
                                   ((unsigned long long)(unsigned short)draw[k].z << 32) | ((unsigned long long)(unsigned short)draw[k].w << 48);
            w >>= sh;
            draw[k] = make_short4((short)(w & 0xffff), (short)((w >> 16) & 0xffff), (short)((w >> 32) & 0xffff), (short)(w >> 48));
            if (rem < 2) t1[k].y = 0.0f;
            if (rem < 3) t1[k].z = 0.0f;
            t1[k].w = 0.0f;
        }
        t0[k] = make_float4(t1[k].x * (float)draw[k].x, t1[k].y * (float)draw[k].y, t1[k].z * (float)draw[k].z, t1[k].w * (float)draw[k].w);
    }
}

__host__ __device__ __forceinline__ void lin_tap(int d, double scale, int sn, int& s0, float& fx)
{
    fx = (float)(((double)d + 0.5) * scale - 0.5);
    s0 = (int)floorf(fx);
    fx -= (float)s0;
    if (s0 < 0) { fx = 0.0f; s0 = 0; }
    if (s0 >= sn - 1) { fx = 0.0f; s0 = sn - 1; }
}
__global__ void __launch_bounds__(256) lo_tap_table_kernel(float* table, int n, int len, int hi_x0, double scale, int sn)
{
    const int j = blockIdx.x * 256 + threadIdx.x;
    if (j >= n) return;
    int s0; float fx;
    lin_tap(hi_x0 + min(j, len - 1), scale, sn, s0, fx);
    table[j] = (float)s0 + fx;
}
__host__ __device__ constexpr int lo_row_cap(int m) { return (((m * 64) / 3) & ~7) < 168 ? 168 : (((m * 64) / 3) & ~7); }
__host__ __device__ constexpr int lo_stage_vec4(int m) { return 12 * lo_row_cap(m) > 256 * m ? (12 * lo_row_cap(m) + 15) / 16 : m * 16; }

template <int M>
struct LoShape {
    static constexpr int MQ = M / 4;
    static constexpr int KH = (MQ + 1) / 2;
    static constexpr int CROW = lo_row_cap(M);
    static constexpr int TC4 = (CROW / 4 + 63) / 64, TD8 = (CROW / 8 + 63) / 64;
    static_assert(12 * CROW <= 16 * lo_stage_vec4(M) && CROW % 8 == 0, "two confidence rows and two disparity rows fit the staging buffer");
};
typedef float f4u __attribute__((ext_vector_type(4), aligned(4)));
typedef short s8u __attribute__((ext_vector_type(8), aligned(2)));

template <int M>
struct LoRaw { v4f c[2][LoShape<M>::TC4]; s8u d[2][LoShape<M>::TD8]; };

struct LoRow {
    int yr[2];
    float b0, b1;
    int ss[2], ns[2];
    bool need_mask[2];
};

template <int M>
__device__ __forceinline__ LoRow lo_row(const FusedInputs& f, int wv, int len)
{
    constexpr int MQ = LoShape<M>::MQ, KH = LoShape<M>::KH;
    const int sw = f.lo_w, sh = f.lo_h;
    LoRow r;
    int sy; float fy;
    {
        const int dy = f.hi_y0 + (int)blockIdx.x;
        fy = (float)(((double)dy + 0.5) * f.lo_scale_y - 0.5);
        sy = (int)floorf(fy);
        fy -= (float)sy;
    }
    r.b0 = 1.0f - fy; r.b1 = fy;
    r.yr[0] = min(max(sy, 0), sh - 1); r.yr[1] = min(max(sy + 1, 0), sh - 1);
    r.yr[0] = __builtin_amdgcn_readfirstlane(r.yr[0]); r.yr[1] = __builtin_amdgcn_readfirstlane(r.yr[1]);
#pragma unroll
    for (int hh = 0; hh < 2; hh++) {
        const int cfirst = 64 * M * wv + 256 * (hh ? KH : 0);
        const int clast = min(64 * M * wv + 256 * (hh ? MQ : KH), len) - 1;
        int s_first = 0, s_last = -2; float f_;
        if (clast >= cfirst) { lin_tap(f.hi_x0 + cfirst, f.lo_scale_x, sw, s_first, f_); lin_tap(f.hi_x0 + clast, f.lo_scale_x, sw, s_last, f_); }
        r.ss[hh] = __builtin_amdgcn_readfirstlane(s_first);
        r.ns[hh] = __builtin_amdgcn_readfirstlane(s_last + 2 - s_first);
    }
#pragma unroll
    for (int hh = 0; hh < 2; hh++)
        r.need_mask[hh] = f.lo_zero_outside && (r.yr[0] < f.lo_vy0 || r.yr[1] >= f.lo_vy1 || r.ss[hh] < f.lo_vx0 || min(r.ss[hh] + r.ns[hh], sw) > f.lo_vx1);
    return r;
}

template <int M>
__device__ inline void lo_fetch(const FusedInputs& f, const LoRow& row, int hh, int lane, LoRaw<M>& q)
{
    const int sw = f.lo_w;
    const float* cbase = f.lo_conf + (ptrdiff_t)blockIdx.y * f.lo_conf_pair;
    const char* dbase = reinterpret_cast<const char*>(f.lo_dl) + (ptrdiff_t)blockIdx.y * f.lo_dl_pair;
#pragma unroll
    for (int r = 0; r < 2; r++) {
        const float* crow = cbase + (ptrdiff_t)row.yr[r] * f.lo_conf_stride;
        const int16_t* drow = reinterpret_cast<const int16_t*>(dbase + (ptrdiff_t)row.yr[r] * f.lo_dl_stride);
#pragma unroll
        for (int t = 0; t < LoShape<M>::TC4; t++) {
            const int e = row.ss[hh] + 4 * (64 * t + lane);
            q.c[r][t] = v4f{0.f, 0.f, 0.f, 0.f};
            if (4 * (64 * t + lane) < row.ns[hh]) {
                if (e + 3 < sw) q.c[r][t] = *reinterpret_cast<const f4u*>(crow + e);
                else {
#pragma unroll
                    for (int c = 0; c < 4; c++) q.c[r][t][c] = crow[min(e + c, sw - 1)];
                }
            }
        }
#pragma unroll
        for (int t = 0; t < LoShape<M>::TD8; t++) {
            const int e = row.ss[hh] + 8 * (64 * t + lane);
            q.d[r][t] = s8u{0, 0, 0, 0, 0, 0, 0, 0};
            if (8 * (64 * t + lane) < row.ns[hh]) {
                if (e + 7 < sw) q.d[r][t] = *reinterpret_cast<const s8u*>(drow + e);
                else {
#pragma unroll
                    for (int c = 0; c < 8; c++) q.d[r][t][c] = drow[min(e + c, sw - 1)];
                }
            }
        }
    }
}

template <int M>
__device__ inline void lo_put(const FusedInputs& f, const LoRow& row, int hh, int lane, const LoRaw<M>& q, float4* stage)
{
    constexpr int CROW = LoShape<M>::CROW;
    typedef short s8a __attribute__((ext_vector_type(8)));
    v4f* Lf4 = reinterpret_cast<v4f*>(stage);
    s8a* Ls8 = reinterpret_cast<s8a*>(stage) + CROW / 2;
    const int sw = f.lo_w;
    const bool rin0 = !f.lo_zero_outside || (row.yr[0] >= f.lo_vy0 && row.yr[0] < f.lo_vy1);
    const bool rin1 = !f.lo_zero_outside || (row.yr[1] >= f.lo_vy0 && row.yr[1] < f.lo_vy1);
#pragma unroll
    for (int t = 0; t < LoShape<M>::TC4; t++) {
        const int i4 = 64 * t + lane, e = row.ss[hh] + 4 * i4;
        v4f q0 = q.c[0][t], q1 = q.c[1][t];
        if (row.need_mask[hh]) {
#pragma unroll
            for (int c = 0; c < 4; c++) {
                const int ec = min(e + c, sw - 1);
                const bool cin = ec >= f.lo_vx0 && ec < f.lo_vx1;
                if (!(rin0 && cin)) q0[c] = 0.0f;
                if (!(rin1 && cin)) q1[c] = 0.0f;
            }
        }
        if (4 * i4 < CROW) {
            Lf4[2 * i4] = v4f{q0[0], q1[0], q0[1], q1[1]};
            Lf4[2 * i4 + 1] = v4f{q0[2], q1[2], q0[3], q1[3]};
        }
    }
#pragma unroll
    for (int t = 0; t < LoShape<M>::TD8; t++) {
        const int i8 = 64 * t + lane;
        const s8u q0 = q.d[0][t], q1 = q.d[1][t];
        if (8 * i8 < CROW) {
            Ls8[2 * i8] = s8a{q0[0], q1[0], q0[1], q1[1], q0[2], q1[2], q0[3], q1[3]};
            Ls8[2 * i8 + 1] = s8a{q0[4], q1[4], q0[5], q1[5], q0[6], q1[6], q0[7], q1[7]};
        }
    }
}

template <int M>
__device__ inline void lo_load_taps(const WavePassArgs& a, const RowPos& p, int hh, v4f (&tp)[M / 4])
{
    constexpr int MQ = LoShape<M>::MQ, KH = LoShape<M>::KH;
    const int nfused = fused_vecs(a.len);
#pragma unroll
    for (int k = (hh ? KH : 0); k < (hh ? MQ : KH); k++) {
        const int idx = p.v0 + 64 * k + p.lane;
        tp[k] = v4f{0.f, 0.f, 0.f, 0.f};
        if (idx < nfused) tp[k] = reinterpret_cast<const v4f*>(a.fuse.lo_taps)[idx];
    }
}

template <int M, bool HALF>
__device__ inline void lo_interp4(const WavePassArgs& a, const LoRow& row, int hh, const float4* stage, v4f tpk, int vec0, int lane,
                                           float4& u0, float4& u1)
{
    const int idx = vec0 + lane;
    constexpr int CROW = LoShape<M>::CROW;
    typedef float f4a8 __attribute__((ext_vector_type(4), aligned(8)));
    typedef short s4a4 __attribute__((ext_vector_type(4), aligned(4)));
    const float* Lf = reinterpret_cast<const float*>(stage);
    const short* Ls = reinterpret_cast<const short*>(stage) + 4 * CROW;
    const v2f bb0 = {row.b0, row.b0}, bb1 = {row.b1, row.b1};
    const bool post_scaled = a.fuse.lo_post_scale != 1.0f;
    f4a8 cq[4]; s4a4 dq[4]; float fxs[4];
    if constexpr (HALF) {
        typedef short s8a4 __attribute__((ext_vector_type(8), aligned(4)));
        const int sl0 = min(max((int)tpk[0] - row.ss[hh], 0), CROW - 4);
        const f4a8 ca = *reinterpret_cast<const f4a8*>(Lf + 2 * sl0), cb = *reinterpret_cast<const f4a8*>(Lf + 2 * sl0 + 4);
        const s8a4 da = *reinterpret_cast<const s8a4*>(Ls + 2 * sl0);
        cq[0] = f4a8{ca[0], ca[1], ca[2], ca[3]}; dq[0] = s4a4{da[0], da[1], da[2], da[3]};
        cq[1] = f4a8{ca[2], ca[3], cb[0], cb[1]}; dq[1] = s4a4{da[2], da[3], da[4], da[5]};
        cq[2] = cq[1]; dq[2] = dq[1];
        cq[3] = f4a8{cb[0], cb[1], cb[2], cb[3]}; dq[3] = s4a4{da[4], da[5], da[6], da[7]};
#pragma unroll
        for (int c = 0; c < 4; c++) fxs[c] = __builtin_amdgcn_fractf(tpk[c]);
    } else {
#pragma unroll
        for (int c = 0; c < 4; c++) {
            const float t = tpk[c];
            fxs[c] = __builtin_amdgcn_fractf(t);
            const int sl = min(max((int)t - row.ss[hh], 0), CROW - 2);
            cq[c] = *reinterpret_cast<const f4a8*>(Lf + 2 * sl);
            dq[c] = *reinterpret_cast<const s4a4*>(Ls + 2 * sl);
        }
    }
    float cv[4], dv[4];
#pragma unroll
    for (int c = 0; c < 4; c++) {
        const float a0 = 1.0f - fxs[c], a1 = fxs[c];
        const v2f aa0 = {a0, a0}, aa1 = {a1, a1};
        const v2f p0 = {cq[c][0], (float)dq[c][0]}, p1 = {cq[c][1], (float)dq[c][1]};
        const v2f n0 = {cq[c][2], (float)dq[c][2]}, n1 = {cq[c][3], (float)dq[c][3]};
        const v2f h0 = p0 * aa0 + n0 * aa1, h1 = p1 * aa0 + n1 * aa1;
        const v2f v = h0 * bb0 + h1 * bb1;
        const float q1 = fminf(fmaxf(rintf(v[1]), -32768.0f), 32767.0f);
        const float q2 = fminf(fmaxf(rintf(q1 * a.fuse.lo_post_scale), -32768.0f), 32767.0f);
        cv[c] = v[0];
        dv[c] = post_scaled ? q2 : q1;
    }
    if (4 * (vec0 + 64) > a.len) {
        const int left = a.len - 4 * idx;
#pragma unroll
        for (int c = 0; c < 4; c++) { const bool on = c < left; cv[c] = on ? cv[c] : 0.0f; dv[c] = on ? dv[c] : 0.0f; }
    }
    u1 = make_float4(cv[0], cv[1], cv[2], cv[3]);
    u0 = make_float4(cv[0] * dv[0], cv[1] * dv[1], cv[2] * dv[2], cv[3] * dv[3]);
}

template <int M, bool HALF>
__device__ __forceinline__ void load_fused_lo(const WavePassArgs& a, const RowPos& p, float4* stage, float4 (&tC)[M / 4], float4 (&t0)[M / 4], float4 (&t1)[M / 4])
{
    constexpr int MQ = LoShape<M>::MQ, KH = LoShape<M>::KH;
#pragma unroll
    for (int k = 0; k < MQ; k++) {
        tC[k] = load_c(a, p, k);
        t0[k] = make_float4(0.f, 0.f, 0.f, 0.f); t1[k] = t0[k];
    }
    const LoRow row = lo_row<M>(a.fuse, p.wv, a.len);
    LoRaw<M> raw[2];
    v4f tp[MQ];
    lo_fetch<M>(a.fuse, row, 0, p.lane, raw[0]);
    lo_load_taps<M>(a, p, 0, tp); lo_load_taps<M>(a, p, 1, tp);
#pragma unroll
    for (int hh = 0; hh < 2; hh++) {
        lo_put<M>(a.fuse, row, hh, p.lane, raw[hh], stage);
        __syncthreads();
        if (hh == 0) {
            asm volatile("" ::: "memory");
            lo_fetch<M>(a.fuse, row, 1, p.lane, raw[1]);
        }
#pragma unroll
        for (int k = (hh ? KH : 0); k < (hh ? MQ : KH); k++) {
            int lane_t = p.lane;
            asm volatile("" : "+v"(lane_t) :: "memory");
            lo_interp4<M, HALF>(a, row, hh, stage, tp[k], p.v0 + 64 * k, lane_t, t0[k], t1[k]);
            asm volatile("" : "+v"(t1[k].x), "+v"(t1[k].y), "+v"(t1[k].z), "+v"(t1[k].w),
                              "+v"(t0[k].x), "+v"(t0[k].y), "+v"(t0[k].z), "+v"(t0[k].w));
            __builtin_amdgcn_sched_barrier(0);
        }
        __syncthreads();
    }
}

template <int M>
__device__ __forceinline__ void transpose_in(float4* stage, int lane, const float4 (&t)[M / 4], float (&dst)[M], float scale)
{
#pragma unroll
    for (int k = 0; k < M / 4; k++) stage[64 * k + lane] = t[k];
    __syncthreads();
#pragma unroll
    for (int k = 0; k < M / 4; k++) {
        const float4 v = stage[lane * (M / 4) + k];
        dst[4 * k + 0] = v.x * scale; dst[4 * k + 1] = v.y * scale;
        dst[4 * k + 2] = v.z * scale; dst[4 * k + 3] = v.w * scale;
    }
    __syncthreads();
}

template <int M>
__device__ __forceinline__ void pair_in(float4* stage, int lane, const float4 (&t)[M / 4], int half, float (&f0)[M], float (&f1)[M])
{
    constexpr int MQ = M / 4;
#pragma unroll
    for (int k = 0; k < MQ; k++) stage[64 * k + lane] = t[k];
    __syncthreads();
    if ((lane >> 5) == half) {
#pragma unroll
        for (int k = 0; k < MQ; k++) {
            const int sidx = pair_slot((lane & 31) * M + 4 * k);
            const float4 v = stage[sidx], w = stage[sidx + 4];
            f0[4 * k + 0] = v.x; f0[4 * k + 1] = v.y; f0[4 * k + 2] = v.z; f0[4 * k + 3] = v.w;
            f1[4 * k + 0] = w.x; f1[4 * k + 1] = w.y; f1[4 * k + 2] = w.z; f1[4 * k + 3] = w.w;
        }
    }
    __syncthreads();
}

template <int M>
__device__ __forceinline__ void store_plain(const WavePassArgs& a, const RowPos& p, float4* stage, int lane, const float (&f0)[M])
{
    constexpr int MQ = M / 4;
#pragma unroll
    for (int k = 0; k < MQ; k++)
        stage[p.lane * MQ + k] = make_float4(f0[4 * k], f0[4 * k + 1], f0[4 * k + 2], f0[4 * k + 3]);
    __syncthreads();
    float4* d4 = reinterpret_cast<float4*>(a.U0 + p.off);
#pragma unroll
    for (int k = 0; k < MQ; k++) {
        const int idx = 64 * k + lane;
        if (p.v0 + idx < p.nvec) store_nt(stage[idx], d4 + p.v0 + idx);
    }
}

template <int M>
__device__ __forceinline__ void store_pair(const WavePassArgs& a, const RowPos& p, float4* stage, int lane, const float (&f0)[M], const float (&f1)[M])
{
    constexpr int MQ = M / 4;
    float4* d4 = reinterpret_cast<float4*>(a.U0 + p.offU);
#pragma unroll
    for (int half = 0; half < 2; half++) {
        if ((p.lane >> 5) == half) {
#pragma unroll
            for (int k = 0; k < MQ; k++) {
                const int sidx = pair_slot((p.lane & 31) * M + 4 * k);
                stage[sidx] = make_float4(f0[4 * k], f0[4 * k + 1], f0[4 * k + 2], f0[4 * k + 3]);
                stage[sidx + 4] = make_float4(f1[4 * k], f1[4 * k + 1], f1[4 * k + 2], f1[4 * k + 3]);
            }
        }
        __syncthreads();
#pragma unroll
        for (int k = 0; k < MQ; k++) {
            const int idx = 2 * p.v0 + 64 * (k + half * MQ) + lane;
            if (idx < p.nvecU) store_nt(stage[64 * k + lane], d4 + rhs_vec<true>(idx));
        }
        __syncthreads();
    }
}

template <int M, int R, int FUSED, int NW = 1>
__global__ void __launch_bounds__(64 * NW, (M > (NW == 2 ? 40 : H_TWO_WAVE_MAX) && R > 1) ? 1 : 2) wave_hpass_kernel(WavePassArgs a)
{
    static_assert(M % 4 == 0 && M >= 4, "chunk length must be a multiple of 4");
    static_assert(NW == 1 || NW == 2, "one or two wavefronts per row");
    constexpr bool LO = FUSED == FUSE_LO || FUSED == FUSE_LO_HALF;
    constexpr bool PAIR = R > 1;
    __shared__ float4 stage_all[NW][LO ? lo_stage_vec4(M) : M * 16];
    __shared__ float xch[NW == 2 ? 5 : 1];
    __shared__ float red[NW == 2 ? 5 : 1][NW == 2 ? 128 : 1];
    __shared__ float xsol[NW == 2 ? 2 : 1][NW == 2 ? 128 : 1];
    const RowPos p = row_pos<M, PAIR, NW>(a);
    const int lane = p.lane, wv = p.wv;
    float4* stage = stage_all[wv];

    float4 tC[M / 4], t0[M / 4], t1[M / 4];
    if constexpr (LO) load_fused_lo<M, FUSED == FUSE_LO_HALF>(a, p, stage, tC, t0, t1);
    else if constexpr (FUSED == FUSE_VIEW) load_fused_view<M>(a, p, tC, t0, t1);
    else load_planes<M, R>(a, p, tC, t0, t1);

    float c[M], f0[M], f1[M];
    transpose_in<M>(stage, lane, tC, c, a.lambda);
    if constexpr (PAIR && FUSED == FUSE_NONE) {
        pair_in<M>(stage, lane, t0, 0, f0, f1);
        pair_in<M>(stage, lane, t1, 1, f0, f1);
    } else {
        transpose_in<M>(stage, lane, t0, f0, 1.0f);
        if constexpr (R > 1) transpose_in<M>(stage, lane, t1, f1, 1.0f);
        else {
#pragma unroll
            for (int i = 0; i < M; i++) f1[i] = 0.0f;
        }
    }

    float a_s = __shfl_up(c[M - 1], 1);
    if (lane == 0) a_s = 0.0f;
    if constexpr (NW == 2) {
        if (wv == 0 && lane == 63) xch[0] = c[M - 1];
        __syncthreads();
        if (wv == 1 && lane == 0) a_s = xch[0];
    }

    Boundary<float, R> bd;
    chunk_boundary<M, R>(c, f0, f1, a_s, bd);
    float nGS0 = __shfl_down(bd.GS0, 1), nGS1 = (R > 1) ? __shfl_down(bd.GS1, 1) : 0.0f;
    float nPS = __shfl_down(bd.PS, 1), nQS = __shfl_down(bd.QS, 1);
    if (lane == 63) { nGS0 = 0.0f; nGS1 = 0.0f; nPS = 0.0f; nQS = 0.0f; }
    if constexpr (NW == 2) {
        if (wv == 1 && lane == 0) { xch[1] = bd.GS0; xch[2] = (R > 1) ? bd.GS1 : 0.0f; xch[3] = bd.PS; xch[4] = bd.QS; }
        __syncthreads();
        if (wv == 0 && lane == 63) { nGS0 = xch[1]; nGS1 = xch[2]; nPS = xch[3]; nQS = xch[4]; }
    }
    float al, be, ga, p0, p1, xs0, xs1;
    separator_row<M, R>(c, f0, f1, bd, nGS0, nGS1, nPS, nQS, al, be, ga, p0, p1);
    float xL0, xL1;
    if constexpr (NW == 2) {
        const int g = 64 * wv + lane;
        red[0][g] = al; red[1][g] = be; red[2][g] = ga; red[3][g] = p0; red[4][g] = p1;
        __syncthreads();
        if (wv == 0) reduced128<R>(lane, red[0], red[1], red[2], red[3], red[4], 1, xsol[0], xsol[1]);
        __syncthreads();
        xs0 = xsol[0][g]; xs1 = (R > 1) ? xsol[1][g] : 0.0f;
        xL0 = g > 0 ? xsol[0][g - 1] : 0.0f; xL1 = (R > 1 && g > 0) ? xsol[1][g - 1] : 0.0f;
    } else {
        pcr64<R>(lane, al, be, ga, p0, p1, xs0, xs1);
        xL0 = __shfl_up(xs0, 1); xL1 = (R > 1) ? __shfl_up(xs1, 1) : 0.0f;
        if (lane == 0) { xL0 = 0.0f; xL1 = 0.0f; }
    }
    chunk_solve<M, R>(c, f0, f1, a_s, xL0, xL1, xs0, xs1);

    int lane_s = lane;
    asm volatile("" : "+v"(lane_s));
    if constexpr (PAIR) store_pair<M>(a, p, stage, lane_s, f0, f1);
    else store_plain<M>(a, p, stage, lane_s, f0);
}

constexpr bool lo_half_bucket(int m, int nw) { return !(m == 60 && nw == 1); }

template <int M, int NW = 1>
hipError_t launch_h(const WavePassArgs& a, int n_rhs, int n_pairs, hipStream_t st)
{
    dim3 grid(a.nscan, n_pairs), block(64 * NW);
    if (a.fuse.lo_conf) {
        if (n_rhs != 2 || !a.fuse.lo_taps) return hipErrorInvalidValue;
        const int n = ((a.len + 3) / 4) * 4;
        hipLaunchKernelGGL(lo_tap_table_kernel, dim3((n + 255) / 256), dim3(256), 0, st, a.fuse.lo_taps, n, a.len, a.fuse.hi_x0, a.fuse.lo_scale_x, a.fuse.lo_w);
        bool half = false;
        if constexpr (lo_half_bucket(M, NW)) {
            half = wave_hpass_lo_half(a);
            if (half) hipLaunchKernelGGL((wave_hpass_kernel<M, 2, FUSE_LO_HALF, NW>), grid, block, 0, st, a);
        }
        if (!half) hipLaunchKernelGGL((wave_hpass_kernel<M, 2, FUSE_LO, NW>), grid, block, 0, st, a);
    } else if (a.fuse.conf_in) {
        if (n_rhs != 2) return hipErrorInvalidValue;
        hipLaunchKernelGGL((wave_hpass_kernel<M, 2, FUSE_VIEW, NW>), grid, block, 0, st, a);
    } else if (n_rhs == 2) hipLaunchKernelGGL((wave_hpass_kernel<M, 2, FUSE_NONE, NW>), grid, block, 0, st, a);
    else hipLaunchKernelGGL((wave_hpass_kernel<M, 1, FUSE_NONE, NW>), grid, block, 0, st, a);
    return hipGetLastError();
}

constexpr Bucket ROW_BUCKETS[] = {{4, 64}, {8, 64}, {16, 64}, {20, 64}, {28, 64}, {40, 64}, {56, 64}, {60, 64}, {64, 64},
                                  {40, 128}, {48, 128}, {56, 128}, {60, 128}, {64, 128}};
constexpr int N_ROW_BUCKETS = sizeof(ROW_BUCKETS) / sizeof(ROW_BUCKETS[0]);

void pick_row_bucket(int len, int& m, int& nw)
{
    const Bucket& b = ROW_BUCKETS[bucket_index(ROW_BUCKETS, len)];
    m = b.m; nw = b.chunks / 64;
}

}

int wave_max_row_len() { return ROW_BUCKETS[N_ROW_BUCKETS - 1].m * ROW_BUCKETS[N_ROW_BUCKETS - 1].chunks; }

bool wave_hpass_can_fuse(const WavePassArgs& a)
{
    if (!a.fuse.conf_in || !a.fuse.dl_in) return false;
    if (a.len < 4 || a.fuse.conf_pitch % 4 != 0 || a.fuse.conf_x0 % 4 != 0 || a.fuse.conf_frame % 4 != 0) return false;
    if ((reinterpret_cast<uintptr_t>(a.fuse.conf_in) & 15u) != 0) return false;
    if (a.fuse.dl_stride % 2 != 0 || a.fuse.dl_pair_stride % 2 != 0 || (reinterpret_cast<uintptr_t>(a.fuse.dl_in) & 1u) != 0) return false;
    return true;
}

bool wave_hpass_lo_half(const WavePassArgs& a)
{
    if (!(a.fuse.lo_conf && a.fuse.lo_half && a.fuse.lo_scale_x == 0.5 && (a.fuse.hi_x0 & 1) == 0 && a.fuse.hi_x0 >= 2)) return false;
    int m, nw;
    pick_row_bucket(a.len, m, nw);
    return lo_half_bucket(m, nw);
}

bool wave_hpass_can_fuse_lo(const WavePassArgs& a)
{
    if (!a.fuse.lo_conf || !a.fuse.lo_dl || a.fuse.lo_w < 2 || a.fuse.lo_w > 65535 || a.fuse.lo_h < 1 || a.len < 2 || a.len > wave_max_row_len()) return false;
    if ((reinterpret_cast<uintptr_t>(a.fuse.lo_conf) & 3u) != 0 || (reinterpret_cast<uintptr_t>(a.fuse.lo_dl) & 1u) != 0) return false;
    if (a.fuse.lo_dl_stride % 2 != 0 || a.fuse.lo_dl_pair % 2 != 0) return false;
    if (!(a.fuse.lo_scale_x > 0.0 && a.fuse.lo_scale_y > 0.0) || a.fuse.hi_x0 < 0 || a.fuse.hi_y0 < 0) return false;
    int m, nw;
    pick_row_bucket(a.len, m, nw);
    const int mq = m / 4, kh = (mq + 1) / 2, cap = lo_row_cap(m);
    for (int wv = 0; wv < nw; wv++)
        for (int hh = 0; hh < 2; hh++) {
            const int cfirst = 64 * m * wv + 256 * (hh ? kh : 0);
            const int clast = std::min(64 * m * wv + 256 * (hh ? mq : kh), a.len) - 1;
            if (clast < cfirst) continue;
            int s_first, s_last; float f_;
            lin_tap(a.fuse.hi_x0 + cfirst, a.fuse.lo_scale_x, a.fuse.lo_w, s_first, f_);
            lin_tap(a.fuse.hi_x0 + clast, a.fuse.lo_scale_x, a.fuse.lo_w, s_last, f_);
            if (s_last + 2 - s_first > cap) return false;
        }
    return true;
}

hipError_t launch_wave_hpass(const WavePassArgs& a, int n_rhs, int n_pairs, hipStream_t st)
{
    if (a.len < 2 || a.len > wave_max_row_len() || a.pitch % 64 != 0 || a.pitch < a.len) return hipErrorInvalidValue;
    if (a.fuse.lo_conf && !wave_hpass_can_fuse_lo(a)) return hipErrorInvalidValue;
    if (!a.fuse.lo_conf && a.fuse.conf_in && !wave_hpass_can_fuse(a)) return hipErrorInvalidValue;
    return dispatch_index<N_ROW_BUCKETS>(bucket_index(ROW_BUCKETS, a.len), [&](auto I) {
        constexpr Bucket b = ROW_BUCKETS[decltype(I)::value];
        return launch_h<b.m, b.chunks / 64>(a, n_rhs, n_pairs, st);
    });
}

}
```

addingdisparityfiltering_amd/csrc/prep_bodies.h:

```cpp
#pragma once
#include "adf_internal.h"

namespace adf {
namespace prep {

#define ADF_PREP_ST(p, v) __builtin_nontemporal_store((v), (p))

constexpr int WS_U = 4;
constexpr int WS_NT = 128;
constexpr int WS_COLS = 4;
constexpr int WS_BCOLS = WS_NT * WS_COLS;
constexpr int WS_LUT_HEAD = 2048;

template <int CH>
struct WsShared {
    float lut_head[WS_LUT_HEAD];
};

typedef unsigned ws_v4u __attribute__((ext_vector_type(4)));
typedef unsigned ws_v2u __attribute__((ext_vector_type(2)));
typedef float ws_v4f __attribute__((ext_vector_type(4)));

template <int CH> struct WsWin;
template <> struct WsWin<3> { ws_v4u a; unsigned b; };
template <> struct WsWin<1> { ws_v2u a; };
template <int CH> struct WsPrev { unsigned q[WS_COLS], qa[WS_COLS]; };

struct WsGuide {
    __amdgpu_buffer_rsrc_t rsrc; unsigned mis, stride;
};
__device__ __forceinline__ WsGuide ws_guide(uintptr_t base0, ptrdiff_t stride_bytes, int rows, int row_bytes)
{
    WsGuide gd;
    gd.mis = (unsigned)__builtin_amdgcn_readfirstlane((int)(base0 & 3u));
    const unsigned blo = (unsigned)__builtin_amdgcn_readfirstlane((int)(unsigned)((base0 - gd.mis) & 0xffffffffu));
    const unsigned bhi = (unsigned)__builtin_amdgcn_readfirstlane((int)(unsigned)((base0 - gd.mis) >> 32));
    gd.stride = (unsigned)__builtin_amdgcn_readfirstlane((int)(unsigned)stride_bytes);
    const unsigned records = (unsigned)__builtin_amdgcn_readfirstlane(
        (int)((gd.mis + (unsigned)(rows - 1) * gd.stride + (unsigned)row_bytes + 3u) & ~3u));
    gd.rsrc = __builtin_amdgcn_make_buffer_rsrc(reinterpret_cast<void*>((uintptr_t)blo | ((uintptr_t)bhi << 32)), (short)0, (int)records, 0x00020000);
    return gd;
}

template <int CH>
__device__ __forceinline__ WsWin<CH> ws_load(const WsGuide& gd, unsigned wo)
{
    WsWin<CH> w;
    if constexpr (CH == 3) {
        w.a = __builtin_amdgcn_raw_buffer_load_b128(gd.rsrc, wo, 0, 0);
        w.b = __builtin_amdgcn_raw_buffer_load_b32(gd.rsrc, wo + 16u, 0, 0);
    } else {
        w.a = __builtin_amdgcn_raw_buffer_load_b64(gd.rsrc, wo, 0, 0);
    }
    return w;
}

template <int CH>
__device__ __forceinline__ void ws_indices(const WsWin<CH>& w, unsigned m, WsPrev<CH>& pv, int (&hidx)[WS_COLS], int (&vidx)[WS_COLS])
{
    if constexpr (CH == 3) {
        const unsigned e0 = __builtin_amdgcn_alignbyte(w.a.y, w.a.x, m), e1 = __builtin_amdgcn_alignbyte(w.a.z, w.a.y, m);
        const unsigned e2 = __builtin_amdgcn_alignbyte(w.a.w, w.a.z, m), e3 = __builtin_amdgcn_alignbyte(w.b, w.a.w, m);
        unsigned p[WS_COLS + 1], pa[WS_COLS + 1];
        p[0] = e0 & 0x00ffffffu;
        p[1] = __builtin_amdgcn_perm(e1, e0, 0x0c050403u);
        p[2] = __builtin_amdgcn_perm(e2, e1, 0x0c040302u);
        p[3] = e2 >> 8;
        p[4] = e3 & 0x00ffffffu;
#pragma unroll
        for (int k = 0; k <= WS_COLS; k++) pa[k] = __builtin_amdgcn_udot4(p[k], p[k], 0u, false);
#pragma unroll
        for (int k = 0; k < WS_COLS; k++) {
            hidx[k] = (int)(pa[k] + pa[k + 1]) - 2 * (int)__builtin_amdgcn_udot4(p[k], p[k + 1], 0u, false);
            vidx[k] = (int)(pa[k] + pv.qa[k]) - 2 * (int)__builtin_amdgcn_udot4(p[k], pv.q[k], 0u, false);
            pv.q[k] = p[k]; pv.qa[k] = pa[k];
        }
    } else {
        const unsigned e = __builtin_amdgcn_alignbyte(w.a.y, w.a.x, m);
        const unsigned nb = __builtin_amdgcn_alignbyte(0u, w.a.y, m) & 0xffu;
#pragma unroll
        for (int k = 0; k < WS_COLS; k++) {
            const int v = (int)((e >> (8 * k)) & 0xffu);
            const int r = k < WS_COLS - 1 ? (int)((e >> (8 * k + 8)) & 0xffu) : (int)nb;
            const int u = (int)((pv.q[0] >> (8 * k)) & 0xffu);
            hidx[k] = (v - r) * (v - r);
            vidx[k] = (u - v) * (u - v);
        }
        pv.q[0] = e;
    }
}

__device__ __forceinline__ __amdgpu_buffer_rsrc_t ws_window(const void* p, size_t bytes)
{
    const uintptr_t b = reinterpret_cast<uintptr_t>(p);
    const unsigned lo = (unsigned)__builtin_amdgcn_readfirstlane((int)(unsigned)(b & 0xffffffffu));
    const unsigned hi = (unsigned)__builtin_amdgcn_readfirstlane((int)(unsigned)(b >> 32));
    const unsigned n = (unsigned)__builtin_amdgcn_readfirstlane((int)(unsigned)bytes);
    return __builtin_amdgcn_make_buffer_rsrc(reinterpret_cast<void*>((uintptr_t)lo | ((uintptr_t)hi << 32)), (short)0, (int)n, 0x00020000);
}
constexpr unsigned WS_DROP = 0x80000000u;

struct WsPending { float wl[2 * WS_COLS]; unsigned g[2 * WS_COLS]; };
__device__ __forceinline__ void ws_lookup_issue(const float* lut_head, const __amdgpu_buffer_rsrc_t& lutwin, const int (&hidx)[WS_COLS],
                                                const int (&vidx)[WS_COLS], WsPending& p)
{
#pragma unroll
    for (int k = 0; k < WS_COLS; k++) {
        p.wl[k] = lut_head[min(hidx[k], WS_LUT_HEAD - 1)];
        p.wl[WS_COLS + k] = lut_head[min(vidx[k], WS_LUT_HEAD - 1)];
    }
#pragma unroll
    for (int k = 0; k < WS_COLS; k++) {
        p.g[k] = __builtin_amdgcn_raw_buffer_load_b32(lutwin, hidx[k] >= WS_LUT_HEAD ? (unsigned)hidx[k] * 4u : WS_DROP, 0, 0);
        p.g[WS_COLS + k] = __builtin_amdgcn_raw_buffer_load_b32(lutwin, vidx[k] >= WS_LUT_HEAD ? (unsigned)vidx[k] * 4u : WS_DROP, 0, 0);
    }
}
__device__ __forceinline__ void ws_lookup_finish(const WsPending& p, float (&wh)[WS_COLS], float (&wv)[WS_COLS])
{
#pragma unroll
    for (int k = 0; k < WS_COLS; k++) {
        wh[k] = p.g[k] != 0u ? __uint_as_float(p.g[k]) : p.wl[k];
        wv[k] = p.g[WS_COLS + k] != 0u ? __uint_as_float(p.g[WS_COLS + k]) : p.wl[WS_COLS + k];
    }
}

struct WsOut {
    __amdgpu_buffer_rsrc_t chor, cvert; unsigned mh[WS_COLS], mv[WS_COLS]; unsigned ho, vo, hstep, vstep; bool st_ok, strip;
    __device__ __forceinline__ void init(const WeightArgs& a, size_t pz, int j0, int y_first)
    {
        const Geom& g = a.g;
        chor = ws_window(a.chor + pz * g.plane, g.plane * sizeof(float));
        cvert = ws_window(a.cvert + pz * g.plane, g.plane * sizeof(float));
        strip = a.cvert_orient == ORIENT_STRIP;
#pragma unroll
        for (int k = 0; k < WS_COLS; k++) { mh[k] = (j0 + k < g.rw - 1) ? 0xffffffffu : 0u; mv[k] = (j0 + k < g.rw) ? 0xffffffffu : 0u; }
        st_ok = j0 >= 0 && j0 < g.pw;
        ho = ((unsigned)y_first * (unsigned)g.pw + (unsigned)j0) * 4u;
        vo = (strip ? ((unsigned)(j0 >> 4) * (unsigned)g.rh + (unsigned)y_first) * ADF_STRIP + (unsigned)(j0 & 15)
                    : (unsigned)y_first * (unsigned)g.pw + (unsigned)j0) * 4u;
        hstep = (unsigned)g.pw * 4u; vstep = (strip ? (unsigned)ADF_STRIP : (unsigned)g.pw) * 4u;
    }
    __device__ __forceinline__ void store_h(int t, const float (&wh)[WS_COLS], bool on) const
    {
        ws_v4u o;
#pragma unroll
        for (int k = 0; k < WS_COLS; k++) o[k] = __float_as_uint(wh[k]) & mh[k];
        __builtin_amdgcn_raw_buffer_store_b128(o, chor, (on && st_ok) ? ho + (unsigned)t * hstep : WS_DROP, 0, 2 );
    }
    __device__ __forceinline__ void store_v(int t, const float (&wv)[WS_COLS], bool last_row, bool on) const
    {
        const unsigned last = last_row ? 0u : 0xffffffffu;
        ws_v4u o;
#pragma unroll
        for (int k = 0; k < WS_COLS; k++) o[k] = __float_as_uint(wv[k]) & mv[k] & last;
        const unsigned off = (on && st_ok) ? vo + (unsigned)t * vstep : WS_DROP;
        if (strip) __builtin_amdgcn_raw_buffer_store_b128(o, cvert, off, 0, 0);
        else __builtin_amdgcn_raw_buffer_store_b128(o, cvert, off, 0, 2);
    }
};

template <int CH>
__device__ __forceinline__ void weights_stream_body(const WeightArgs& a, int bx, int by, int nby, size_t pz, WsShared<CH>& sh, bool active)
{
    static_assert(CH == 1 || CH == 3, "guides have one or three channels");
    float (&lut_head)[WS_LUT_HEAD] = sh.lut_head;
    const Geom& g = a.g;
    const int tid = active ? (int)threadIdx.x : 0;
    if (active)
        for (int q = tid; q < WS_LUT_HEAD; q += WS_NT) lut_head[q] = a.lut[q];
    __syncthreads();
    const int ws_rows = (g.rh + nby - 1) / nby;
    const int x0 = bx * WS_BCOLS, y0 = by * ws_rows;
    if (!active || y0 >= g.rh) return;
    constexpr int WS_PRIO = 3;
    __builtin_amdgcn_s_setprio(WS_PRIO);
    const int nrows = min(ws_rows, g.rh - y0) + 1;
    const int j0 = x0 + WS_COLS * tid;

    const int r_first = g.ry + y0, r_last = g.ry + min(y0 + nrows - 1, g.rh - 1);
    const WsGuide gd = ws_guide(reinterpret_cast<uintptr_t>(a.guide) + (uintptr_t)((ptrdiff_t)pz * a.pair_stride + (ptrdiff_t)r_first * a.stride),
                                a.stride, r_last - r_first + 1, g.W * CH);
    const unsigned col_off = gd.mis + (unsigned)((g.rx + x0) * CH);
    const unsigned lane_off = (unsigned)(tid * WS_COLS * CH);
    auto row_off = [&](int n) -> unsigned { return col_off + (unsigned)(min(y0 + n, g.rh - 1) - y0) * gd.stride; };
    auto load = [&](int n) -> WsWin<CH> { return ws_load<CH>(gd, (row_off(n) & ~3u) + lane_off); };

    WsOut out;
    out.init(a, pz, j0, y0);
    const __amdgpu_buffer_rsrc_t lutwin = ws_window(a.lut, sizeof(float) * ADF_LUT_LEVELS);
    WsPrev<CH> pv;
#pragma unroll
    for (int k = 0; k < WS_COLS; k++) { pv.q[k] = 0; pv.qa[k] = 0; }
    WsWin<CH> nxt[WS_U], cur[WS_U];
#pragma unroll
    for (int s = 0; s < WS_U; s++) nxt[s] = load(s < nrows ? s : nrows - 1);
    WsPending pend;
    {
        int hidx[WS_COLS], vidx[WS_COLS];
        ws_indices<CH>(nxt[0], row_off(0) & 3u, pv, hidx, vidx);
        ws_lookup_issue(lut_head, lutwin, hidx, vidx, pend);
    }
    for (int n0 = 0; n0 < nrows; n0 += WS_U) {
#pragma unroll
        for (int s = 0; s < WS_U; s++) {
            cur[s] = nxt[s];
            if constexpr (CH == 3) asm volatile("" : "+v"(cur[s].a), "+v"(cur[s].b)); else asm volatile("" : "+v"(cur[s].a));
        }
#pragma unroll
        for (int s = 0; s < WS_U; s++) nxt[s] = load(min(n0 + WS_U + s, nrows - 1));
#pragma unroll
        for (int s = 0; s < WS_U; s++) {
            const int n = n0 + s;
            WsPending ahead;
            {
                int hidx[WS_COLS], vidx[WS_COLS];
                ws_indices<CH>(s + 1 < WS_U ? cur[s + 1 < WS_U ? s + 1 : 0] : nxt[0], row_off(min(n + 1, nrows - 1)) & 3u, pv, hidx, vidx);
                ws_lookup_issue(lut_head, lutwin, hidx, vidx, ahead);
            }
            float wh[WS_COLS], wv[WS_COLS];
            ws_lookup_finish(pend, wh, wv);
            out.store_h(n, wh, n < nrows - 1);
            out.store_v(n - 1, wv, y0 + n - 1 == g.rh - 1, n >= 1 && n < nrows);
            pend = ahead;
        }
    }
}


}
}
```

addingdisparityfiltering_amd/csrc/weights_kernels.hip:

```cpp
#include "adf_internal.h"
#include "prep_bodies.h"
#include <cstdlib>

namespace adf {

namespace {

#define ADF_ST(p, v) __builtin_nontemporal_store((v), (p))
constexpr int TX = 64, TY = 32, NT = 256;
constexpr int LUT_HEAD = 2048;

template <int CH>
__global__ void __launch_bounds__(NT) weights_kernel(WeightArgs a)
{
    constexpr int RB = (TX + 1) * CH;
    constexpr int RW = (RB + 3) / 4 + 1;
    __shared__ unsigned gw[(TY + 1) * RW];
    __shared__ int mis[TY + 1];
    __shared__ float th[TX * (TY + 1)];
    __shared__ float lut_head[LUT_HEAD];
    const Geom& g = a.g;
    const int tid = threadIdx.x, tx = tid % TX, ty = tid / TX;
    const int x0 = blockIdx.x * TX, y0 = blockIdx.y * TY;
    const size_t pz = blockIdx.z;
    const unsigned char* gp = a.guide + (ptrdiff_t)pz * a.pair_stride;
    const int last_px = min(x0 + TX, g.rw - 1);
    const int need = (last_px - x0 + 1) * CH;

    for (int rr = ty; rr < TY + 1; rr += NT / TX) {
        const int gi = min(y0 + rr, g.rh - 1);
        const unsigned char* rowp = gp + (ptrdiff_t)(g.ry + gi) * a.stride + (ptrdiff_t)(g.rx + x0) * CH;
        const int m = (int)(reinterpret_cast<uintptr_t>(rowp) & 3u);
        const unsigned* wp = reinterpret_cast<const unsigned*>(rowp - m);
        const int nw = (m + need + 3) >> 2;
        for (int w = tx; w < nw; w += TX) gw[rr * RW + w] = wp[w];
        if (tx == 0) mis[rr] = m;
    }
    for (int q = tid; q < LUT_HEAD; q += NT) lut_head[q] = a.lut[q];
    __syncthreads();

    const unsigned char* gb = reinterpret_cast<const unsigned char*>(gw);
    float* chor = a.chor + pz * g.plane;
    float* cvert = a.cvert + pz * g.plane;
    int hidx[TY / 4], vidx[TY / 4];
#pragma unroll
    for (int kk = 0; kk < TY / 4; kk++) {
        const int r = ty + 4 * kk;
        const unsigned char* p = gb + r * (RW * 4) + mis[r] + tx * CH;
        const unsigned char* pd = gb + (r + 1) * (RW * 4) + mis[r + 1] + tx * CH;
        int hi = 0, vi = 0;
#pragma unroll
        for (int c = 0; c < CH; c++) {
            const int v = p[c];
            const int dh = v - (int)p[CH + c];
            const int dv = v - (int)pd[c];
            hi += dh * dh; vi += dv * dv;
        }
        hidx[kk] = hi; vidx[kk] = vi;
    }
    float wh[TY / 4], wv[TY / 4];
    bool big = false;
#pragma unroll
    for (int kk = 0; kk < TY / 4; kk++) {
        wh[kk] = lut_head[min(hidx[kk], LUT_HEAD - 1)];
        wv[kk] = lut_head[min(vidx[kk], LUT_HEAD - 1)];
        big = big || hidx[kk] >= LUT_HEAD || vidx[kk] >= LUT_HEAD;
    }
    if (big) {
#pragma unroll
        for (int kk = 0; kk < TY / 4; kk++) {
            if (hidx[kk] >= LUT_HEAD) wh[kk] = a.lut[hidx[kk]];
            if (vidx[kk] >= LUT_HEAD) wv[kk] = a.lut[vidx[kk]];
        }
    }
    const int j = x0 + tx;
#pragma unroll
    for (int kk = 0; kk < TY / 4; kk++) {
        const int r = ty + 4 * kk;
        const int i = y0 + r;
        const bool ok = i < g.rh && j < g.rw;
        const float h = (j == g.rw - 1) ? 0.0f : wh[kk];
        const float v = (i == g.rh - 1) ? 0.0f : wv[kk];
        if (a.chor_orient == ORIENT_N) { if (ok) chor[(size_t)i * g.pw + j] = h; }
        else th[tx * (TY + 1) + r] = ok ? h : 0.0f;
        if (ok) cvert[a.cvert_orient == ORIENT_STRIP ? strip_index(i, j, g.rh) : (size_t)i * g.pw + j] = v;
    }
    if (a.chor_orient == ORIENT_T) {
        __syncthreads();
#pragma unroll
        for (int m = 0; m < TX / 8; m++) {
            const int cidx = tid / TY + 8 * m, ridx = tid % TY;
            const int jj = x0 + cidx, ii = y0 + ridx;
            if (jj < g.rw && ii < g.rh) chor[(size_t)jj * g.ph + ii] = th[cidx * (TY + 1) + ridx];
        }
    }
}

template <int CH>
__global__ void __launch_bounds__(prep::WS_NT) weights_stream_kernel(WeightArgs a)
{
    __shared__ prep::WsShared<CH> sh;
    prep::weights_stream_body<CH>(a, blockIdx.x, blockIdx.y, gridDim.y, blockIdx.z, sh, true);
}

__global__ void __launch_bounds__(256) transpose_n_to_t_kernel(const float* __restrict__ src, float* __restrict__ dst, Geom g)
{
    __shared__ float tile[64][65];
    const int tid = threadIdx.x;
    const int j0 = blockIdx.x * 64, i0 = blockIdx.y * 64;
    const size_t pb = (size_t)blockIdx.z * g.plane;
    const int c4 = tid & 15, r = tid >> 4;
#pragma unroll
    for (int m = 0; m < 4; m++) {
        const int row = r + 16 * m;
        float4 v = make_float4(0.f, 0.f, 0.f, 0.f);
        if (i0 + row < g.rh) v = *reinterpret_cast<const float4*>(src + pb + (size_t)(i0 + row) * g.pw + j0 + 4 * c4);
        tile[row][4 * c4 + 0] = v.x; tile[row][4 * c4 + 1] = v.y; tile[row][4 * c4 + 2] = v.z; tile[row][4 * c4 + 3] = v.w;
    }
    __syncthreads();
#pragma unroll
    for (int m = 0; m < 4; m++) {
        const int col = r + 16 * m;
        if (j0 + col < g.rw) {
            const float4 v = make_float4(tile[4 * c4 + 0][col], tile[4 * c4 + 1][col], tile[4 * c4 + 2][col], tile[4 * c4 + 3][col]);
            *reinterpret_cast<float4*>(dst + pb + (size_t)(j0 + col) * g.ph + i0 + 4 * c4) = v;
        }
    }
}

}

hipError_t launch_weights(const WeightArgs& a, int n_pairs, hipStream_t st)
{
    if (a.chor_orient == ORIENT_T && a.cvert_orient == ORIENT_N && a.scratch) {
        WeightArgs b = a;
        b.chor = a.scratch; b.chor_orient = ORIENT_N; b.scratch = nullptr;
        hipError_t e = launch_weights(b, n_pairs, st);
        if (e != hipSuccess) return e;
        dim3 grid(a.g.pw / 64, a.g.ph / 64, n_pairs);
        hipLaunchKernelGGL(transpose_n_to_t_kernel, grid, dim3(256), 0, st, a.scratch, a.chor, a.g);
        return hipGetLastError();
    }
    if (a.cvert_orient != ORIENT_N && !(a.cvert_orient == ORIENT_STRIP && a.chor_orient == ORIENT_N)) return hipErrorInvalidValue;
    static const bool force_generic = [] { const char* e = getenv("ADF_WEIGHTS_GENERIC"); return e && atoi(e) != 0; }();
    if (!force_generic && a.chor_orient == ORIENT_N && a.stride > 0 && a.stride < ((ptrdiff_t)1 << 29) && (size_t)a.g.W * a.ch < ((size_t)1 << 29)) {
        dim3 sgrid((a.g.rw + prep::WS_BCOLS - 1) / prep::WS_BCOLS, 1, n_pairs);
        {
            int rpb = 128;
            while (rpb > 16 && ((a.g.rh + rpb - 1) / rpb) * (int)(sgrid.x * sgrid.z) < 2048) rpb >>= 1;
            while (rpb > 4 && ((a.g.rh + rpb - 1) / rpb) * (int)(sgrid.x * sgrid.z) < 512) rpb >>= 1;
            while (rpb > 1 && (size_t)(rpb + 1) * (size_t)a.stride >= ((size_t)1 << 30)) rpb >>= 1;
            sgrid.y = (a.g.rh + rpb - 1) / rpb;
        }
        if (a.ch == 1) hipLaunchKernelGGL(weights_stream_kernel<1>, sgrid, dim3(prep::WS_NT), 0, st, a);
        else if (a.ch == 3) hipLaunchKernelGGL(weights_stream_kernel<3>, sgrid, dim3(prep::WS_NT), 0, st, a);
        else return hipErrorInvalidValue;
        return hipGetLastError();
    }
    dim3 grid((a.g.rw + TX - 1) / TX, (a.g.rh + TY - 1) / TY, n_pairs);
    if (a.ch == 1) hipLaunchKernelGGL(weights_kernel<1>, grid, dim3(NT), 0, st, a);
    else if (a.ch == 3) hipLaunchKernelGGL(weights_kernel<3>, grid, dim3(NT), 0, st, a);
    else return hipErrorInvalidValue;
    return hipGetLastError();
}

}
```

addingdisparityfiltering_amd/ximgproc.py:

```python
import ctypes as C
import math

import numpy as np

from . import _lib
from ._lib import SGBM_COST_BT, SGBM_COST_CENSUS_DENSE, SGBM_COST_CENSUS_SPARSE
from ._lib import AdfError, PATH_CONF_BAND, PATH_FUSED_FIRST_PASS, PATH_MERGED_PREP, PATH_SCALED_FUSED, PATH_SCALED_HALF, Rect, SOLVER_EXACT, SOLVER_WAVE

try:
    import torch
except Exception:
    torch = None


def _is_torch(a):
    return torch is not None and isinstance(a, torch.Tensor)


def _as_rect(roi):
    if roi is None:
        return None
    if isinstance(roi, Rect):
        return roi
    x, y, w, h = roi
    return Rect(int(x), int(y), int(w), int(h))


_ITEMSIZE = {np.int16: 2, np.uint8: 1, np.float32: 4, np.uint64: 8}
_TORCH_DTYPE = {np.int16: torch.int16, np.uint8: torch.uint8, np.float32: torch.float32, np.uint64: torch.int64} if torch is not None else {}
_raw_stream = getattr(getattr(torch, "_C", None), "_cuda_getCurrentRawStream", None) if torch is not None else None


class _Image:

    def __init__(self, arr, dtype_np, what, batched, allow_channels=(1,)):
        self.keep = arr
        if _is_torch(arr):
            if not arr.is_cuda:
                arr = arr.cpu().numpy()
            else:
                if arr.dtype != _TORCH_DTYPE[dtype_np]:
                    raise AdfError(_lib.ADF_EBADARG, "%s must have dtype %s" % (what, _TORCH_DTYPE[dtype_np]))
                self.device = True
                isz = _ITEMSIZE[dtype_np]
                self.ptr = arr.data_ptr()
                self._finish(arr.shape, [q * isz for q in arr.stride()], isz, what, batched, allow_channels)
                return
        a = np.asarray(arr)
        if a.dtype != np.dtype(dtype_np):
            raise AdfError(_lib.ADF_EBADARG, "%s must have dtype %s (got %s)" % (what, np.dtype(dtype_np), a.dtype))
        self.device = False
        self.keep = a
        self.ptr = a.ctypes.data
        self._finish(a.shape, a.strides, a.itemsize, what, batched, allow_channels)

    def _finish(self, shape, strides, itemsize, what, batched, allow_channels):
        nd = len(shape)
        k = 1 if batched else 0
        if nd - k == 2:
            self.c, sc, sx = 1, itemsize, strides[k + 1]
        elif nd - k == 3:
            self.c, sc, sx = shape[k + 2], strides[k + 2], strides[k + 1]
        else:
            raise AdfError(_lib.ADF_EBADARG, "%s has an unsupported shape %s" % (what, tuple(shape)))
        self.n, self.pair_stride = (shape[0], strides[0]) if batched else (1, 0)
        self.h, self.w, self.stride = shape[k], shape[k + 1], strides[k]
        if self.n < 1 or self.h < 1 or self.w < 1:
            raise AdfError(_lib.ADF_EBADARG, "%s is empty" % what)
        if self.c not in allow_channels:
            raise AdfError(_lib.ADF_EBADARG, "%s must have %s channel(s)" % (what, " or ".join(map(str, allow_channels))))
        if sc != itemsize or sx != itemsize * self.c:
            raise AdfError(_lib.ADF_ESIZE, "%s rows must be dense (channel-interleaved, unit pixel stride)" % what)


def _empty(img, shape, dtype_np):
    if img.device:
        return torch.empty(shape, dtype=_TORCH_DTYPE[dtype_np], device=img.keep.device)
    return np.empty(shape, dtype_np)


def _out_like(img, batched, dtype_np):
    return _empty(img, (img.n, img.h, img.w) if batched else (img.h, img.w), dtype_np)


def _stream_of(img):
    if img.device:
        dev = img.keep.device
        if _raw_stream is not None and dev.index is not None:
            return _raw_stream(dev.index)
        return torch.cuda.current_stream(dev).cuda_stream
    return None


def _read(fn, ctype, *args):
    v = ctype()
    _lib.check(fn(*args, C.byref(v)))
    return v.value


_entries = {}


def _call(name, img, args):
    pair = _entries.get(name)
    if pair is None:
        pair = _entries[name] = (getattr(_lib.lib(), name + "_host"), getattr(_lib.lib(), name + "_device"))
    if img.device:
        _lib.check(pair[1](*args, _stream_of(img)))
    else:
        _lib.check(pair[0](*args))


class _Handle:
    _h, _destroy = None, None

    def __del__(self):
        h, self._h = self._h, None
        if h:
            try:
                getattr(_lib.lib(), self._destroy)(h)
            except Exception:
                pass


def _check_device(dev, imgs, what):
    for im in imgs:
        if im is not None and im.device and im.keep.device.index != dev:
            raise AdfError(_lib.ADF_EBADARG, "%s lives on cuda:%d; tensors on cuda:%s cannot be passed to it "
                                             "(create one handle per GPU)" % (what, dev, im.keep.device.index))


class DisparityFilter:

    def filter(self, disparity_map_left, left_view, filtered_disparity_map=None,
               disparity_map_right=None, ROI=None, right_view=None):
        raise NotImplementedError


class DisparityWLSFilter(_Handle, DisparityFilter):
    _destroy = "adf_wls_destroy"

    def __init__(self, use_confidence, left_offset=0, right_offset=0, top_offset=0, bottom_offset=0,
                 min_disp=0):
        self._h = C.c_void_p()
        _lib.check(_lib.lib().adf_wls_create(C.byref(self._h), int(bool(use_confidence)), left_offset,
                                             right_offset, top_offset, bottom_offset, min_disp))
        self._use_confidence = bool(use_confidence)
        self._last = None
        self._dev = _read(_lib.lib().adf_wls_get_device, C.c_int, self._h)

    def getLambda(self):
        return _read(_lib.lib().adf_wls_get_lambda, C.c_double, self._h)

    def setLambda(self, _lambda):
        _lib.check(_lib.lib().adf_wls_set_lambda(self._h, float(_lambda)))

    def getSigmaColor(self):
        return _read(_lib.lib().adf_wls_get_sigma_color, C.c_double, self._h)

    def setSigmaColor(self, _sigma_color):
        _lib.check(_lib.lib().adf_wls_set_sigma_color(self._h, float(_sigma_color)))

    def getLRCthresh(self):
        return _read(_lib.lib().adf_wls_get_lrc_thresh, C.c_int, self._h)

    def setLRCthresh(self, _LRC_thresh):
        _lib.check(_lib.lib().adf_wls_set_lrc_thresh(self._h, int(_LRC_thresh)))

    def getDepthDiscontinuityRadius(self):
        return _read(_lib.lib().adf_wls_get_depth_discontinuity_radius, C.c_int, self._h)

    def setDepthDiscontinuityRadius(self, _disc_radius):
        _lib.check(_lib.lib().adf_wls_set_depth_discontinuity_radius(self._h, int(_disc_radius)))

    def setFGSParams(self, lambda_attenuation=0.25, num_iter=3):
        _lib.check(_lib.lib().adf_wls_set_fgs_params(self._h, float(lambda_attenuation), int(num_iter)))

    def setSolver(self, solver):
        _lib.check(_lib.lib().adf_wls_set_solver(self._h, int(solver)))

    def getSolver(self):
        return _read(_lib.lib().adf_wls_get_solver, C.c_int, self._h)

    def getLastSolver(self):
        return _read(_lib.lib().adf_wls_get_last_solver, C.c_int, self._h)

    def getLastPath(self):
        return _read(_lib.lib().adf_wls_get_last_path, C.c_int, self._h)

    def enableProfiling(self, on=True):
        _lib.check(_lib.lib().adf_wls_profile_enable(self._h, int(bool(on))))

    def readProfile(self):
        buf = (_lib.KernelTime * 16)()
        n = C.c_int()
        _lib.check(_lib.lib().adf_wls_profile_read(self._h, buf, 16, C.byref(n)))
        return {buf[k].name.decode(): dict(launches=buf[k].launches, total_ms=buf[k].total_ms,
                                           alg_bytes=buf[k].alg_bytes, moved_bytes=buf[k].moved_bytes)
                for k in range(n.value)}

    def workspaceBytes(self):
        return int(_lib.lib().adf_wls_workspace_bytes(self._h))

    def filter(self, disparity_map_left, left_view, filtered_disparity_map=None,
               disparity_map_right=None, ROI=None, right_view=None):
        return self._filter("adf_wls_filter_scaled", np.int16, disparity_map_left, left_view, filtered_disparity_map,
                            disparity_map_right, ROI)

    def filterFloat(self, disparity_map_left, left_view, filtered_disparity_map=None,
                    disparity_map_right=None, ROI=None):
        return self._filter("adf_wls_filter_scaled_f32", np.float32, disparity_map_left, left_view, filtered_disparity_map,
                            disparity_map_right, ROI)

    def _filter(self, entry, out_dtype, disparity_map_left, left_view, filtered_disparity_map, disparity_map_right, ROI):
        if disparity_map_left is None:
            raise AdfError(_lib.ADF_EBADARG, "disparity_map_left is empty")
        if left_view is None:
            raise AdfError(_lib.ADF_EBADARG, "left_view is empty")
        batched = len(disparity_map_left.shape) == 3
        dl = _Image(disparity_map_left, np.int16, "disparity_map_left", batched)
        gv = _Image(left_view, np.uint8, "left_view", batched, allow_channels=(1, 3))
        if gv.n != dl.n:
            raise AdfError(_lib.ADF_ESIZE, "batch sizes of disparity maps and views differ")
        dr = None
        if disparity_map_right is not None and getattr(disparity_map_right, "size", 1) != 0:
            dr = _Image(disparity_map_right, np.int16, "disparity_map_right", batched)
            if (dr.n, dr.h, dr.w) != (dl.n, dl.h, dl.w):
                raise AdfError(_lib.ADF_ESIZE, "left and right disparity maps differ in size")
        elif self._use_confidence:
            raise AdfError(_lib.ADF_EBADARG, "disparity_map_right is required with use_confidence")
        if gv.device != dl.device or (dr is not None and dr.device != dl.device):
            raise AdfError(_lib.ADF_EBADARG, "inputs must all be numpy arrays or all be CUDA tensors")
        if filtered_disparity_map is None:
            filtered_disparity_map = _out_like(gv, batched, out_dtype)
        out = _Image(filtered_disparity_map, out_dtype, "filtered_disparity_map", batched)
        if (out.n, out.h, out.w) != (gv.n, gv.h, gv.w) or out.device != dl.device:
            raise AdfError(_lib.ADF_ESIZE, "filtered_disparity_map has the wrong size or placement")
        if dl.device:
            _check_device(self._dev, (dl, gv, dr, out), "this DisparityWLSFilter")
        roi = _as_rect(ROI)
        args = (self._h, dl.n,
                dl.ptr, dl.stride, dl.pair_stride, dl.w, dl.h,
                gv.ptr, gv.stride, gv.pair_stride, gv.c, gv.w, gv.h,
                out.ptr, out.stride, out.pair_stride,
                dr.ptr if dr else None, dr.stride if dr else 0, dr.pair_stride if dr else 0,
                C.byref(roi) if roi is not None else None)
        if dl.device:
            _lib.check(getattr(_lib.lib(), entry + "_device")(*args, _stream_of(dl)))
        else:
            _lib.check(getattr(_lib.lib(), entry + "_host")(*args))
        self._last = (batched, dl.device, gv)
        return filtered_disparity_map

    def getConfidenceMap(self, pair=None):
        if self._last is None or not self._use_confidence:
            return np.zeros((0, 0), np.float32)
        batched, device, ex = self._last
        pairs = range(ex.n) if pair is None else [pair]
        outs = []
        for k in pairs:
            o = _empty(ex, (ex.h, ex.w), np.float32)
            _call("adf_wls_get_confidence", ex, (self._h, k, o.data_ptr() if device else o.ctypes.data, ex.w * 4))
            outs.append(o)
        if pair is not None or not batched:
            return outs[0]
        return torch.stack(outs) if device else np.stack(outs)

    def getROI(self):
        r = Rect()
        _lib.check(_lib.lib().adf_wls_get_roi(self._h, C.byref(r)))
        return (r.x, r.y, r.width, r.height)

    def sync(self, stream=None):
        _lib.check(_lib.lib().adf_wls_sync(self._h, stream))


def _accessors(*names):
    def pair(name):
        return (lambda self: getattr(self, name)), (lambda self, v: setattr(self, name, v))

    def add(cls):
        for name in names:
            for prefix, fn in zip(("get", "set"), pair(name)):
                fn.__name__ = prefix + name[0].upper() + name[1:]
                setattr(cls, fn.__name__, fn)
        return cls
    return add


@_accessors("minDisparity", "numDisparities", "blockSize", "disp12MaxDiff", "speckleWindowSize", "uniquenessRatio")
class StereoMatcher(_Handle):
    _channels = (1,)

    def __init__(self, minDisparity=0, numDisparities=16, blockSize=3):
        self.minDisparity, self.numDisparities, self.blockSize = minDisparity, numDisparities, blockSize
        self.disp12MaxDiff, self.speckleWindowSize, self.uniquenessRatio = -1, 0, 10

    def _views(self, left, right, device_only=None):
        nd = len(left.shape)
        color = 3 in self._channels and nd in (3, 4) and left.shape[-1] == 3
        batched = nd == (4 if color else 3)
        L = _Image(left, np.uint8, "left", batched, self._channels)
        R = _Image(right, np.uint8, "right", batched, self._channels)
        if device_only and not (L.device and R.device):
            raise AdfError(_lib.ADF_EBADARG, device_only)
        if (L.n, L.h, L.w, L.c) != (R.n, R.h, R.w, R.c):
            raise AdfError(_lib.ADF_ESIZE, "All the images must have the same size")
        return L, R, batched

    @staticmethod
    def _outputs(maps, names, L, batched, mismatch):
        maps = [_out_like(L, batched, np.int16) if m is None else m for m in maps]
        descs = [_Image(m, np.int16, what, batched) for m, what in zip(maps, names)]
        for D in descs:
            if (D.n, D.h, D.w) != (L.n, L.h, L.w) or D.device != L.device:
                raise AdfError(_lib.ADF_ESIZE, mismatch)
        return maps, descs

    def compute(self, left, right, disparity=None):
        self._refuse()
        if self.speckleWindowSize > 0:
            raise AdfError(_lib.ADF_EBADARG, "speckle filtering is not implemented inside compute(); "
                                             "use filterSpeckles on the result")
        L, R, batched = self._views(left, right)
        if L.device != R.device:
            raise AdfError(_lib.ADF_EBADARG, "left and right must live on the same side (host or device)")
        (disparity,), (D,) = self._outputs((disparity,), ("disparity",), L, batched, "disparity must match the views")
        self._prepare((L, R, D))
        _call(self._entry, L, self._args(L, R, D))
        return disparity


@_accessors("textureThreshold", "preFilterCap")
class StereoBM(StereoMatcher):
    _destroy, _entry = "adf_bm_destroy", "adf_bm_compute"

    def __init__(self, numDisparities=0, blockSize=21):
        super().__init__(0, numDisparities if numDisparities > 0 else 64, blockSize)
        self.textureThreshold, self.uniquenessRatio, self.preFilterCap = 10, 15, 31

    @staticmethod
    def create(numDisparities=0, blockSize=21):
        return StereoBM(numDisparities, blockSize)

    def _left_right_check_on(self):
        return 0 <= self.disp12MaxDiff < 1000000

    def _refuse(self):
        if self._left_right_check_on():
            raise AdfError(_lib.ADF_EBADARG, "disp12MaxDiff (left-right check inside the matcher) is not implemented")

    def _prepare(self, imgs):
        lib = _lib.lib()
        if self._h is None:
            h = C.c_void_p()
            _lib.check(lib.adf_bm_create(C.byref(h), int(self.numDisparities), int(self.blockSize)))
            self._h = h
        _check_device(_read(lib.adf_bm_get_device, C.c_int, self._h), imgs, "this StereoBM")
        _lib.check(lib.adf_bm_set_params(self._h, int(self.minDisparity), int(self.numDisparities), int(self.blockSize),
                                         int(self.preFilterCap), int(self.textureThreshold), int(self.uniquenessRatio)))

    def _args(self, L, R, D):
        return (self._h, L.n, L.ptr, L.stride, L.pair_stride, R.ptr, R.stride, R.pair_stride, L.w, L.h,
                D.ptr, D.stride, D.pair_stride)

    def computeBoth(self, left, right, disparity_left=None, disparity_right=None):
        L, R, batched = self._views(left, right, "computeBoth takes device tensors; use two compute() calls on the host")
        if self._left_right_check_on() or self.speckleWindowSize > 0:
            raise AdfError(_lib.ADF_EBADARG, "the matcher's own left-right check and speckle filter are not implemented")
        (disparity_left, disparity_right), (DL, DR) = self._outputs(
            (disparity_left, disparity_right), ("disparity_left", "disparity_right"), L, batched, "disparity maps must match the views")
        if self.preFilterCap != 31:
            if getattr(self, "_right", None) is None:
                self._right = StereoBM(1, 5)
            rm = createRightMatcher(self)
            for k in ("minDisparity", "numDisparities", "blockSize", "textureThreshold", "uniquenessRatio",
                      "preFilterCap", "disp12MaxDiff", "speckleWindowSize"):
                setattr(self._right, k, getattr(rm, k))
            self.compute(left, right, disparity_left)
            self._right.compute(right, left, disparity_right)
            return disparity_left, disparity_right
        self._prepare((L, R, DL, DR))
        _lib.check(_lib.lib().adf_bm_compute_both_device(*self._args(L, R, DL), DR.ptr, DR.stride, DR.pair_stride, _stream_of(L)))
        return disparity_left, disparity_right


@_accessors("P1", "P2", "mode", "preFilterCap", "costType", "censusSize")
class StereoSGBM(StereoMatcher):
    MODE_SGBM, MODE_HH, MODE_SGBM_3WAY = 0, 1, 2
    _destroy, _entry, _channels = "adf_sgbm_destroy", "adf_sgbm_compute", (1, 3)

    def __init__(self, minDisparity=0, numDisparities=16, blockSize=3, P1=0, P2=0, mode=0, preFilterCap=0):
        super().__init__(minDisparity, numDisparities, blockSize)
        self.P1, self.P2, self.mode, self.preFilterCap = P1, P2, mode, preFilterCap
        self.disp12MaxDiff, self.uniquenessRatio = 0, 0
        self.costType, self.censusSize = SGBM_COST_BT, 7

    @staticmethod
    def create(minDisparity=0, numDisparities=16, blockSize=3, P1=0, P2=0, disp12MaxDiff=0, preFilterCap=0,
               uniquenessRatio=0, speckleWindowSize=0, speckleRange=0, mode=0):
        m = StereoSGBM(minDisparity, numDisparities, blockSize, P1, P2, mode, preFilterCap)
        m.disp12MaxDiff, m.uniquenessRatio, m.speckleWindowSize = disp12MaxDiff, uniquenessRatio, speckleWindowSize
        return m

    def _refuse(self):
        if self.mode not in (StereoSGBM.MODE_SGBM, StereoSGBM.MODE_HH, StereoSGBM.MODE_SGBM_3WAY):
            raise AdfError(_lib.ADF_EBADARG, "mode must be StereoSGBM.MODE_SGBM, MODE_HH or MODE_SGBM_3WAY")

    def _prepare(self, imgs):
        lib = _lib.lib()
        if self._h is None:
            h = C.c_void_p()
            _lib.check(lib.adf_sgbm_create(C.byref(h), int(self.minDisparity), int(self.numDisparities), int(self.blockSize)))
            self._h = h
        _check_device(_read(lib.adf_sgbm_get_device, C.c_int, self._h), imgs, "this StereoSGBM")
        _lib.check(lib.adf_sgbm_set_params(self._h, int(self.minDisparity), int(self.numDisparities), int(self.blockSize),
                                           int(self.P1), int(self.P2), int(self.preFilterCap), int(self.uniquenessRatio),
                                           int(self.mode)))
        _lib.check(lib.adf_sgbm_set_disp12_max_diff(self._h, int(self.disp12MaxDiff)))
        _lib.check(lib.adf_sgbm_set_cost(self._h, int(self.costType), int(self.censusSize)))

    def _args(self, L, R, D):
        return (self._h, L.n, L.ptr, L.stride, L.pair_stride, R.ptr, R.stride, R.pair_stride, L.c, L.w, L.h,
                D.ptr, D.stride, D.pair_stride)


_INT32_MAX = 2 ** 31 - 1


def _round_half_even(v, what):
    v = float(v)
    if not math.isfinite(v):
        raise AdfError(_lib.ADF_EBADARG, "%s must be finite" % what)
    return int(round(v))


def filterSpeckles(img, newVal, maxSpeckleSize, maxDiff, buf=None):
    if img is None:
        raise AdfError(_lib.ADF_EBADARG, "img is empty")
    dt = img.dtype if _is_torch(img) else np.asarray(img).dtype
    if dt == np.uint8 or (torch is not None and dt == torch.uint8):
        raise AdfError(_lib.ADF_EBADARG, "filterSpeckles supports CV_16SC1 only (CV_8UC1 is not supported)")
    nd = len(img.shape)
    if nd not in (2, 3):
        raise AdfError(_lib.ADF_EBADARG, "img must be (H,W) or a batch (N,H,W)")
    im = _Image(img, np.int16, "img", nd == 3)
    nv = _round_half_even(newVal, "newVal")
    if not -32768 <= nv <= 32767:
        raise AdfError(_lib.ADF_EBADARG, "newVal %r is outside the CV_16S range" % (newVal,))
    md = max(-_INT32_MAX, min(_INT32_MAX, _round_half_even(maxDiff, "maxDiff")))
    ms = max(-_INT32_MAX, min(_INT32_MAX, int(maxSpeckleSize)))
    args = (im.n, im.ptr, im.stride, im.pair_stride, im.w, im.h, nv, ms, md)
    if not im.device:
        _call("adf_filter_speckles", im, args)
        return img, buf
    ws, ws_bytes = None, 0
    if buf is not None:
        if not (_is_torch(buf) and buf.is_cuda and buf.is_contiguous()):
            raise AdfError(_lib.ADF_EBADARG, "buf must be a contiguous CUDA tensor (or None)")
        if buf.device != img.device:
            raise AdfError(_lib.ADF_EBADARG, "buf lives on %s, img on %s" % (buf.device, img.device))
        ws, ws_bytes = buf.data_ptr(), buf.numel() * buf.element_size()
        if ws_bytes < speckleWorkspaceBytes(im.n, im.h, im.w):
            raise AdfError(_lib.ADF_ESIZE, "buf holds %d bytes; %d needed" % (ws_bytes, speckleWorkspaceBytes(im.n, im.h, im.w)))
    with torch.cuda.device(img.device):
        _call("adf_filter_speckles", im, args + (ws, ws_bytes))
    return img, buf


def censusTransform(image, kernelSize, type, dst=None):
    if image is None:
        raise AdfError(_lib.ADF_EBADARG, "image is empty")
    nd = len(image.shape)
    if nd not in (2, 3):
        raise AdfError(_lib.ADF_EBADARG, "image must be (H,W) or a batch (N,H,W) of CV_8UC1 images")
    im = _Image(image, np.uint8, "image", nd == 3)
    if dst is None:
        dst = _out_like(im, nd == 3, np.uint64)
    D = _Image(dst, np.uint64, "dst", nd == 3)
    if (D.n, D.h, D.w) != (im.n, im.h, im.w) or D.device != im.device:
        raise AdfError(_lib.ADF_ESIZE, "dst must have the image's shape on its side (host or device)")
    args = (im.n, im.ptr, im.stride, im.pair_stride, im.w, im.h, int(type), int(kernelSize), D.ptr, D.stride, D.pair_stride)
    if not im.device:
        _call("adf_census_transform", im, args)
        return dst
    if dst.device != im.keep.device:
        raise AdfError(_lib.ADF_EBADARG, "dst lives on %s, image on %s" % (dst.device, im.keep.device))
    with torch.cuda.device(im.keep.device):
        _call("adf_census_transform", im, args)
    return dst

# ... 269 lines not shown
```

include/adf_wls.h:

```cpp
#ifndef ADF_WLS_H
#define ADF_WLS_H

#include <stddef.h>
#include <stdint.h>

#ifdef __cplusplus
extern "C" {
#endif

#define ADF_VERSION 100

enum adf_status {
    ADF_OK = 0,
    ADF_EBADARG = 1,
    ADF_ESIZE = 2,
    ADF_EHIP = 3,
    ADF_ENOMEM = 4,
    ADF_ENODEV = 5
};

enum adf_solver { ADF_SOLVER_EXACT = 0, ADF_SOLVER_WAVE = 1 };

enum adf_depth { ADF_8U = 0, ADF_16S = 3, ADF_32F = 5 };

typedef struct adf_wls adf_wls_t;
typedef struct adf_fgs adf_fgs_t;

typedef struct adf_rect { int x, y, width, height; } adf_rect;

int adf_version(void);
const char* adf_last_error(void);
int adf_device_count(void);
int adf_device_pci_bus_id(int device, char* buf, int len);


int adf_wls_create(adf_wls_t** out, int use_confidence, int left_offset, int right_offset,
                   int top_offset, int bottom_offset, int min_disp);
void adf_wls_destroy(adf_wls_t* h);

int adf_wls_set_lambda(adf_wls_t* h, double lambda);
int adf_wls_get_lambda(const adf_wls_t* h, double* lambda);
int adf_wls_set_sigma_color(adf_wls_t* h, double sigma_color);
int adf_wls_get_sigma_color(const adf_wls_t* h, double* sigma_color);
int adf_wls_set_lrc_thresh(adf_wls_t* h, int lrc_thresh);
int adf_wls_get_lrc_thresh(const adf_wls_t* h, int* lrc_thresh);
int adf_wls_set_depth_discontinuity_radius(adf_wls_t* h, int radius);
int adf_wls_get_depth_discontinuity_radius(const adf_wls_t* h, int* radius);

int adf_wls_set_fgs_params(adf_wls_t* h, double lambda_attenuation, int num_iter);
int adf_wls_set_solver(adf_wls_t* h, int solver);
int adf_wls_get_solver(const adf_wls_t* h, int* solver);
int adf_wls_get_last_solver(const adf_wls_t* h, int* solver);
#define ADF_PATH_CONF_BAND 1
#define ADF_PATH_FUSED_FIRST_PASS 2
#define ADF_PATH_MERGED_PREP 4
#define ADF_PATH_SCALED_FUSED 8
#define ADF_PATH_SCALED_HALF 16
int adf_wls_get_last_path(const adf_wls_t* h, int* path_flags);

int adf_wls_filter_device(adf_wls_t* h, int n_pairs,
                          const int16_t* disp_left, ptrdiff_t disp_left_stride, ptrdiff_t disp_left_pair_stride,
                          const uint8_t* left_view, ptrdiff_t view_stride, ptrdiff_t view_pair_stride,
                          int view_channels, int W, int H,
                          int16_t* out, ptrdiff_t out_stride, ptrdiff_t out_pair_stride,
                          const int16_t* disp_right, ptrdiff_t disp_right_stride, ptrdiff_t disp_right_pair_stride,
                          const adf_rect* roi, void* stream);

int adf_wls_filter_host(adf_wls_t* h, int n_pairs,
                        const int16_t* disp_left, ptrdiff_t disp_left_stride, ptrdiff_t disp_left_pair_stride,
                        const uint8_t* left_view, ptrdiff_t view_stride, ptrdiff_t view_pair_stride,
                        int view_channels, int W, int H,
                        int16_t* out, ptrdiff_t out_stride, ptrdiff_t out_pair_stride,
                        const int16_t* disp_right, ptrdiff_t disp_right_stride, ptrdiff_t disp_right_pair_stride,
                        const adf_rect* roi);

int adf_wls_filter_scaled_device(adf_wls_t* h, int n_pairs,
                                 const int16_t* disp_left, ptrdiff_t disp_left_stride, ptrdiff_t disp_left_pair_stride,
                                 int disp_W, int disp_H,
                                 const uint8_t* left_view, ptrdiff_t view_stride, ptrdiff_t view_pair_stride,
                                 int view_channels, int W, int H,
                                 int16_t* out, ptrdiff_t out_stride, ptrdiff_t out_pair_stride,
                                 const int16_t* disp_right, ptrdiff_t disp_right_stride, ptrdiff_t disp_right_pair_stride,
                                 const adf_rect* roi, void* stream);
int adf_wls_filter_scaled_host(adf_wls_t* h, int n_pairs,
                               const int16_t* disp_left, ptrdiff_t disp_left_stride, ptrdiff_t disp_left_pair_stride,
                               int disp_W, int disp_H,
                               const uint8_t* left_view, ptrdiff_t view_stride, ptrdiff_t view_pair_stride,
                               int view_channels, int W, int H,
                               int16_t* out, ptrdiff_t out_stride, ptrdiff_t out_pair_stride,
                               const int16_t* disp_right, ptrdiff_t disp_right_stride, ptrdiff_t disp_right_pair_stride,
                               const adf_rect* roi);

int adf_wls_filter_f32_device(adf_wls_t* h, int n_pairs,
                              const int16_t* disp_left, ptrdiff_t disp_left_stride, ptrdiff_t disp_left_pair_stride,
                              const uint8_t* left_view, ptrdiff_t view_stride, ptrdiff_t view_pair_stride,
                              int view_channels, int W, int H,
                              float* out, ptrdiff_t out_stride, ptrdiff_t out_pair_stride,
                              const int16_t* disp_right, ptrdiff_t disp_right_stride, ptrdiff_t disp_right_pair_stride,
                              const adf_rect* roi, void* stream);
int adf_wls_filter_f32_host(adf_wls_t* h, int n_pairs,
                            const int16_t* disp_left, ptrdiff_t disp_left_stride, ptrdiff_t disp_left_pair_stride,
                            const uint8_t* left_view, ptrdiff_t view_stride, ptrdiff_t view_pair_stride,
                            int view_channels, int W, int H,
                            float* out, ptrdiff_t out_stride, ptrdiff_t out_pair_stride,
                            const int16_t* disp_right, ptrdiff_t disp_right_stride, ptrdiff_t disp_right_pair_stride,
                            const adf_rect* roi);
int adf_wls_filter_scaled_f32_device(adf_wls_t* h, int n_pairs,
                                     const int16_t* disp_left, ptrdiff_t disp_left_stride, ptrdiff_t disp_left_pair_stride,
                                     int disp_W, int disp_H,
                                     const uint8_t* left_view, ptrdiff_t view_stride, ptrdiff_t view_pair_stride,
                                     int view_channels, int W, int H,
                                     float* out, ptrdiff_t out_stride, ptrdiff_t out_pair_stride,
                                     const int16_t* disp_right, ptrdiff_t disp_right_stride, ptrdiff_t disp_right_pair_stride,
                                     const adf_rect* roi, void* stream);
int adf_wls_filter_scaled_f32_host(adf_wls_t* h, int n_pairs,
                                   const int16_t* disp_left, ptrdiff_t disp_left_stride, ptrdiff_t disp_left_pair_stride,
                                   int disp_W, int disp_H,
                                   const uint8_t* left_view, ptrdiff_t view_stride, ptrdiff_t view_pair_stride,
                                   int view_channels, int W, int H,
                                   float* out, ptrdiff_t out_stride, ptrdiff_t out_pair_stride,
                                   const int16_t* disp_right, ptrdiff_t disp_right_stride, ptrdiff_t disp_right_pair_stride,
                                   const adf_rect* roi);

int adf_wls_get_confidence_device(adf_wls_t* h, int pair, float* dst, ptrdiff_t dst_stride, void* stream);
int adf_wls_get_confidence_host(adf_wls_t* h, int pair, float* dst, ptrdiff_t dst_stride);
int adf_wls_get_device(const adf_wls_t* h, int* device);
int adf_wls_get_roi(const adf_wls_t* h, adf_rect* roi);
int adf_wls_sync(adf_wls_t* h, void* stream);
size_t adf_wls_workspace_bytes(const adf_wls_t* h);

typedef struct adf_kernel_time {
    char name[48];
    int launches;
    double total_ms;
    double alg_bytes;
    double moved_bytes;
} adf_kernel_time;
int adf_wls_profile_enable(adf_wls_t* h, int on);
int adf_wls_profile_read(adf_wls_t* h, adf_kernel_time* out, int capacity, int* count);


int adf_fgs_create(adf_fgs_t** out, const uint8_t* guide, ptrdiff_t guide_stride, int guide_channels,
                   int w, int h, double lambda, double sigma_color, double lambda_attenuation,
                   int num_iter, int solver);
int adf_fgs_create_device(adf_fgs_t** out, const uint8_t* guide, ptrdiff_t guide_stride, int guide_channels,
                          int w, int h, double lambda, double sigma_color, double lambda_attenuation,
                          int num_iter, int solver, void* stream);
void adf_fgs_destroy(adf_fgs_t* h);
void adf_release_cached_memory(void);
#define ADF_WEIGHT_TABLE_LEVELS (3 * 256 * 256)
int adf_weight_table_host(float sigma_color, float* table, int levels);
int adf_fgs_get_device(const adf_fgs_t* h, int* device);
int adf_fgs_get_solver(const adf_fgs_t* h, int* solver);

int adf_fgs_filter_host(adf_fgs_t* h, const void* src, ptrdiff_t src_stride, void* dst,
                        ptrdiff_t dst_stride, int depth, int channels);
int adf_fgs_filter_device(adf_fgs_t* h, const void* src, ptrdiff_t src_stride, void* dst,
                          ptrdiff_t dst_stride, int depth, int channels, void* stream);


#define ADF_UNKNOWN_DISPARITY 16320

int adf_compute_mse_host(const int16_t* gt, ptrdiff_t gt_stride, const int16_t* src, ptrdiff_t src_stride,
                         int W, int H, const adf_rect* roi, double* mse);
int adf_compute_mse_device(const int16_t* gt, ptrdiff_t gt_stride, const int16_t* src, ptrdiff_t src_stride,
                           int W, int H, const adf_rect* roi, double* mse, void* stream);
int adf_compute_bad_pixel_percent_host(const int16_t* gt, ptrdiff_t gt_stride, const int16_t* src, ptrdiff_t src_stride,
                                       int W, int H, const adf_rect* roi, int thresh, double* percent);
int adf_compute_bad_pixel_percent_device(const int16_t* gt, ptrdiff_t gt_stride, const int16_t* src, ptrdiff_t src_stride,
                                         int W, int H, const adf_rect* roi, int thresh, double* percent, void* stream);
int adf_get_disparity_vis_host(const int16_t* src, ptrdiff_t src_stride, uint8_t* dst, ptrdiff_t dst_stride,
                               int W, int H, double scale);
int adf_get_disparity_vis_device(const int16_t* src, ptrdiff_t src_stride, uint8_t* dst, ptrdiff_t dst_stride,
                                 int W, int H, double scale, void* stream);

typedef struct adf_bm adf_bm_t;
int adf_bm_create(adf_bm_t** out, int num_disparities, int block_size);
void adf_bm_destroy(adf_bm_t* h);
int adf_bm_set_params(adf_bm_t* h, int min_disparity, int num_disparities, int block_size,
                      int prefilter_cap, int texture_threshold, int uniqueness_ratio);
int adf_bm_get_device(const adf_bm_t* h, int* device);
int adf_bm_get_params(const adf_bm_t* h, int* min_disparity, int* num_disparities, int* block_size,
                      int* prefilter_cap, int* texture_threshold, int* uniqueness_ratio);
int adf_bm_compute_device(adf_bm_t* h, int n_pairs,
                          const uint8_t* left, ptrdiff_t left_stride, ptrdiff_t left_pair_stride,
                          const uint8_t* right, ptrdiff_t right_stride, ptrdiff_t right_pair_stride,
                          int W, int H,
                          int16_t* disparity, ptrdiff_t disp_stride, ptrdiff_t disp_pair_stride,
                          void* stream);
int adf_bm_compute_both_device(adf_bm_t* h, int n_pairs,
                               const uint8_t* left, ptrdiff_t left_stride, ptrdiff_t left_pair_stride,
                               const uint8_t* right, ptrdiff_t right_stride, ptrdiff_t right_pair_stride,
                               int W, int H,
                               int16_t* disp_left, ptrdiff_t disp_left_stride, ptrdiff_t disp_left_pair_stride,
                               int16_t* disp_right, ptrdiff_t disp_right_stride, ptrdiff_t disp_right_pair_stride,
                               void* stream);
int adf_bm_compute_host(adf_bm_t* h, int n_pairs,
                        const uint8_t* left, ptrdiff_t left_stride, ptrdiff_t left_pair_stride,
                        const uint8_t* right, ptrdiff_t right_stride, ptrdiff_t right_pair_stride,
                        int W, int H,
                        int16_t* disparity, ptrdiff_t disp_stride, ptrdiff_t disp_pair_stride);

#define ADF_SGBM_MODE_SGBM 0
#define ADF_SGBM_MODE_HH 1
#define ADF_SGBM_MODE_3WAY 2
typedef struct adf_sgbm adf_sgbm_t;
int adf_sgbm_create(adf_sgbm_t** out, int min_disparity, int num_disparities, int block_size);
void adf_sgbm_destroy(adf_sgbm_t* h);
int adf_sgbm_get_device(const adf_sgbm_t* h, int* device);
int adf_sgbm_set_params(adf_sgbm_t* h, int min_disparity, int num_disparities, int block_size, int P1, int P2,
                        int prefilter_cap, int uniqueness_ratio, int mode);
int adf_sgbm_set_disp12_max_diff(adf_sgbm_t* h, int disp12_max_diff);
int adf_sgbm_get_disp12_max_diff(const adf_sgbm_t* h, int* disp12_max_diff);
int adf_sgbm_get_params(const adf_sgbm_t* h, int* min_disparity, int* num_disparities, int* block_size, int* P1, int* P2,
                        int* prefilter_cap, int* uniqueness_ratio, int* mode);
#define ADF_SGBM_COST_BT 0
#define ADF_SGBM_COST_CENSUS_DENSE 1
#define ADF_SGBM_COST_CENSUS_SPARSE 2
int adf_sgbm_set_cost(adf_sgbm_t* h, int cost_type, int census_size);
int adf_sgbm_get_cost(const adf_sgbm_t* h, int* cost_type, int* census_size);
int adf_sgbm_compute_device(adf_sgbm_t* h, int n_pairs,
                            const uint8_t* left, ptrdiff_t left_stride, ptrdiff_t left_pair_stride,
                            const uint8_t* right, ptrdiff_t right_stride, ptrdiff_t right_pair_stride,
                            int channels, int W, int H,
                            int16_t* disparity, ptrdiff_t disp_stride, ptrdiff_t disp_pair_stride,
                            void* stream);
int adf_sgbm_compute_host(adf_sgbm_t* h, int n_pairs,
                          const uint8_t* left, ptrdiff_t left_stride, ptrdiff_t left_pair_stride,
                          const uint8_t* right, ptrdiff_t right_stride, ptrdiff_t right_pair_stride,
                          int channels, int W, int H,
                          int16_t* disparity, ptrdiff_t disp_stride, ptrdiff_t disp_pair_stride);

int adf_census_transform_device(int n_images, const uint8_t* src, ptrdiff_t src_stride, ptrdiff_t src_image_stride,
                                int W, int H, int census_type, int census_size,
                                uint64_t* dst, ptrdiff_t dst_stride, ptrdiff_t dst_image_stride, void* stream);
int adf_census_transform_host(int n_images, const uint8_t* src, ptrdiff_t src_stride, ptrdiff_t src_image_stride,
                              int W, int H, int census_type, int census_size,
                              uint64_t* dst, ptrdiff_t dst_stride, ptrdiff_t dst_image_stride);

size_t adf_filter_speckles_workspace_bytes(int n_maps, int W, int H);
int adf_filter_speckles_device(int n_maps, int16_t* img, ptrdiff_t stride, ptrdiff_t map_stride, int W, int H,
                               int new_val, int max_speckle_size, int max_diff,
                               void* workspace, size_t workspace_bytes, void* stream);
int adf_filter_speckles_host(int n_maps, int16_t* img, ptrdiff_t stride, ptrdiff_t map_stride, int W, int H,
                             int new_val, int max_speckle_size, int max_diff);

int adf_half_size(int n, int* half);
int adf_prepare_views_device(int n_images, const uint8_t* src, ptrdiff_t src_stride, ptrdiff_t src_image_stride,
                             int W, int H, int src_channels,
                             uint8_t* dst, ptrdiff_t dst_stride, ptrdiff_t dst_image_stride,
                             int dst_W, int dst_H, int dst_channels, void* stream);
int adf_prepare_views_host(int n_images, const uint8_t* src, ptrdiff_t src_stride, ptrdiff_t src_image_stride,
                           int W, int H, int src_channels,
                           uint8_t* dst, ptrdiff_t dst_stride, ptrdiff_t dst_image_stride,
                           int dst_W, int dst_H, int dst_channels);

#ifdef __cplusplus
}
#endif
#endif
```

Measured before the change: 40740.

## Compute horizontal smoothness weights from the guide inside the wave row pass

When the wave solver runs unscaled, the weights kernel no longer writes the horizontal weight plane. The horizontal wave pass instead loads the guide row and the LUT head directly and computes the weights in registers. This removes one float plane of writes and later reads per iteration, in exchange for more guide traffic and ALU work in every horizontal pass. It also adds register pressure and template variants of the h-pass and weights stream kernels.

```diff
diff --git a/addingdisparityfiltering_amd/__init__.py b/addingdisparityfiltering_amd/__init__.py
--- a/addingdisparityfiltering_amd/__init__.py
+++ b/addingdisparityfiltering_amd/__init__.py
@@ -8,6 +8,7 @@
     PATH_CONF_BAND,
     PATH_FUSED_FIRST_PASS,
     PATH_MERGED_PREP,
+    PATH_ROW_WEIGHTS_GUIDE,
     PATH_SCALED_FUSED,
     PATH_SCALED_HALF,
     SGBM_COST_BT,
diff --git a/addingdisparityfiltering_amd/_lib.py b/addingdisparityfiltering_amd/_lib.py
--- a/addingdisparityfiltering_amd/_lib.py
+++ b/addingdisparityfiltering_amd/_lib.py
@@ -7,6 +7,7 @@
 ADF_OK, ADF_EBADARG, ADF_ESIZE, ADF_EHIP, ADF_ENOMEM, ADF_ENODEV = range(6)
 SOLVER_EXACT, SOLVER_WAVE = 0, 1
 PATH_CONF_BAND, PATH_FUSED_FIRST_PASS, PATH_MERGED_PREP, PATH_SCALED_FUSED, PATH_SCALED_HALF = 1, 2, 4, 8, 16
+PATH_ROW_WEIGHTS_GUIDE = 32
 DEPTH_8U, DEPTH_16S, DEPTH_32F = 0, 3, 5
 SGBM_COST_BT, SGBM_COST_CENSUS_DENSE, SGBM_COST_CENSUS_SPARSE = 0, 1, 2
 
@@ -52,6 +53,7 @@
     ("adf_wls_get_solver", _i, [_vp, C.POINTER(_i)]),
     ("adf_wls_get_last_solver", _i, [_vp, C.POINTER(_i)]),
     ("adf_wls_get_last_path", _i, [_vp, C.POINTER(_i)]),
+    ("adf_wls_get_last_solver_path", _i, [_vp, C.POINTER(_i)]),
     ("adf_wls_filter_device", _i, _FILTER_DEV),
     ("adf_wls_filter_host", _i, _FILTER_DEV[:-1]),
     ("adf_wls_filter_scaled_device", _i, _FILTER_SCALED_DEV),
diff --git a/addingdisparityfiltering_amd/csrc/adf_api.hip b/addingdisparityfiltering_amd/csrc/adf_api.hip
--- a/addingdisparityfiltering_amd/csrc/adf_api.hip
+++ b/addingdisparityfiltering_amd/csrc/adf_api.hip
@@ -86,7 +86,7 @@
 
 static int run_passes(bool wave, const Geom& g, const SolvePlanes& p, int n_rhs, float lambda, float atten, int num_iter,
                       const FinalOut& fo, int n_pairs, hipStream_t st, Profiler* prof = nullptr,
-                      const FusedInputs* fuse = nullptr)
+                      const FusedInputs* fuse = nullptr, const GuideWeights* gw = nullptr)
 {
     const double px = (double)g.rw * g.rh * n_pairs;
     float lam = lambda;
@@ -94,7 +94,8 @@
         const bool fused = it == 0 && fuse, last = it == num_iter - 1;
         const int epi = last ? fo.epilogue : EPI_PLANES;
         const double lo_b = (fused && fuse->lo_conf) ? 6.0 * fuse->lo_scale_x * fuse->lo_scale_y : 6.0;
-        const double hb = fused ? (4.0 + lo_b + 8.0) * px : (4.0 + 8.0 * n_rhs) * px;
+        const double wb = gw ? (double)gw->ch : 4.0;
+        const double hb = fused ? (wb + lo_b + 8.0) * px : (wb + 8.0 * n_rhs) * px;
         const double out_b = (last ? epilogue_bytes(fo.epilogue) : 4.0 * n_rhs) * px;
         const double vb = (4.0 + 4.0 * n_rhs) * px + out_b;
         if (wave) {
@@ -102,6 +103,7 @@
             h.C = p.CH; h.U0 = p.A0; h.U1 = p.A1;
             h.nscan = g.rh; h.len = g.rw; h.pitch = g.pw; h.plane = g.plane; h.lambda = lam;
             if (fused) h.fuse = *fuse;
+            if (gw) h.gw = *gw;
             v.C = p.CV; v.U0 = p.A0; v.U1 = p.A1;
             v.nscan = g.rw; v.len = g.rh; v.pitch = g.pw; v.plane = g.plane; v.lambda = lam;
             if (last) set_final_out(v, fo);
@@ -157,6 +159,7 @@
     int last_cpitch = 0, last_cx0 = 0;
     long long conf_sig[4] = {0, 0, 0, 0};
     int last_path = 0;
+    int last_solver_path = 0;
     Lut lut;
     DevBuf ws;
     DevBuf conf;
@@ -173,6 +176,7 @@
     bool scaled_fuse = true;
     bool conf_band = true;
     bool merge_small = true;
+    bool row_weights_guide = true;
     static bool null_caller_of(hipStream_t s) { return s == nullptr || s == hipStreamLegacy || s == hipStreamPerThread; }
     int ensure_side(hipStream_t caller)
     {
@@ -210,6 +214,7 @@
     if (const char* e = getenv("ADF_NO_OVERLAP")) h->overlap = atoi(e) == 0;
     if (const char* e = getenv("ADF_CONF_BAND")) h->conf_band = atoi(e) != 0;
     if (const char* e = getenv("ADF_SCALED_FUSE")) h->scaled_fuse = atoi(e) != 0;
+    if (const char* e = getenv("ADF_ROW_WEIGHTS_GUIDE")) h->row_weights_guide = atoi(e) != 0;
     if (const char* e = getenv("ADF_LO_HALF")) h->scaled_half = atoi(e) != 0;
     if (const char* e = getenv("ADF_MERGE_SMALL")) h->merge_small = atoi(e) != 0;
     *out = h;
@@ -256,6 +261,7 @@
 extern "C" int adf_wls_get_solver(const adf_wls_t* h, int* v) { NEED_HANDLE(h); if (v) *v = h->solver; return ADF_OK; }
 extern "C" int adf_wls_get_last_solver(const adf_wls_t* h, int* v) { NEED_HANDLE(h); if (v) *v = h->last_solver; return ADF_OK; }
 extern "C" int adf_wls_get_last_path(const adf_wls_t* h, int* v) { NEED_HANDLE(h); if (v) *v = h->last_path; return ADF_OK; }
+extern "C" int adf_wls_get_last_solver_path(const adf_wls_t* h, int* v) { NEED_HANDLE(h); if (v) *v = h->last_solver_path; return ADF_OK; }
 
 extern "C" int adf_wls_get_device(const adf_wls_t* h, int* device) { NEED_HANDLE(h); if (device) *device = h->device; return ADF_OK; }
 extern "C" int adf_wls_get_roi(const adf_wls_t* h, adf_rect* roi) { NEED_HANDLE(h); if (roi) *roi = h->roi; return ADF_OK; }
@@ -425,6 +431,7 @@
     ConfStage stage;
     bool fork_weights;
     bool outside_on_side;
+    bool guide_rows;
 };
 
 struct WlsPlan {
@@ -434,16 +441,22 @@
     size_t per_pair; int chunk;
     ChunkPlan full, tail;
     int path;
-};
-
-static ChunkPlan plan_chunk(const adf_wls* h, ConfStage stage, bool wave)
+    int solver_path;
+};
+
+static ChunkPlan plan_chunk(const adf_wls* h, ConfStage stage, bool wave, bool guide_rows)
 {
     const bool fork = stage != CONF_NONE && stage != CONF_MERGED && h->overlap;
-    return ChunkPlan{stage, fork, fork && wave && stage != CONF_TWO_KERNEL};
+    return ChunkPlan{stage, fork, fork && wave && stage != CONF_TWO_KERNEL, guide_rows && stage != CONF_MERGED};
+}
+
+static GuideWeights guide_weights(const adf_wls* h, const uint8_t* guide, ptrdiff_t sG, ptrdiff_t psG, int gch, const Geom& g)
+{
+    return GuideWeights{guide, sG, psG, gch, g.rx, g.ry, h->lut.cur};
 }
 
 static WlsPlan plan_wls(const adf_wls* h, const Geom& g, int n_pairs, const int16_t* dispL, ptrdiff_t sL, ptrdiff_t psL,
-                        ptrdiff_t sG, int gch, const ScaledStage* scaled)
+                        const uint8_t* view, ptrdiff_t sG, ptrdiff_t psG, int gch, const ScaledStage* scaled)
 {
     WlsPlan p{};
     const bool conf = h->use_confidence;
@@ -461,15 +474,24 @@
     p.chunk = (int)(h->ws_limit / p.per_pair);
     if (p.chunk < 1) p.chunk = 1;
     if (p.chunk > n_pairs) p.chunk = n_pairs;
+    bool guide_rows = false;
+    if (p.wave && !scaled && h->row_weights_guide) {
+        WavePassArgs probe{};
+        probe.len = g.rw; probe.gw = guide_weights(h, view, sG, psG, gch, g);
+        WeightArgs wprobe{};
+        wprobe.stride = sG; wprobe.ch = gch; wprobe.chor_orient = ORIENT_N; wprobe.g = g;
+        guide_rows = wave_hpass_guide_fits(probe) && weights_stream_fits(wprobe);
+    }
     auto chunk_of = [&](int n) {
         const bool merged = p.band && h->merge_small && prep_small_fits(g, h->disc_radius, gch, n) && prep_small_guide_fits(g, sG, gch);
-        return plan_chunk(h, merged ? CONF_MERGED : stage, p.wave);
+        return plan_chunk(h, merged ? CONF_MERGED : stage, p.wave, guide_rows);
     };
     p.full = chunk_of(p.chunk);
     p.tail = chunk_of(n_pairs % p.chunk ? n_pairs % p.chunk : p.chunk);
     p.path = ((p.band || (scaled && scaled->lo.band_map)) ? ADF_PATH_CONF_BAND : 0) |
              (p.fused_first ? ADF_PATH_FUSED_FIRST_PASS : 0) |
              ((p.full.stage == CONF_MERGED || p.tail.stage == CONF_MERGED) ? ADF_PATH_MERGED_PREP : 0);
+    p.solver_path = (p.full.guide_rows || p.tail.guide_rows) ? ADF_PATH_ROW_WEIGHTS_GUIDE : 0;
     if (stage == CONF_SCALED_LO)
         p.path |= ADF_PATH_SCALED_FUSED |
                   (wave_hpass_lo_half(first_pass_probe(lo_fuse(h, *scaled, 0, g), g.rw)) ? ADF_PATH_SCALED_HALF : 0);
@@ -512,10 +534,10 @@
     const Geom g = make_geom(W, H, roi.x, roi.y, roi.width, roi.height);
     h->lazy_conf.pending = false;
     h->roi = roi; h->last_W = W; h->last_H = H; h->last_pairs = n_pairs;
-    h->last_cpitch = g.cpitch; h->last_cx0 = g.cx0; h->last_path = 0;
+    h->last_cpitch = g.cpitch; h->last_cx0 = g.cx0; h->last_path = 0; h->last_solver_path = 0;
 
     if ((rc = h->lut.ensure((float)h->sigma_color, st))) return rc;
-    const WlsPlan plan = plan_wls(h, g, n_pairs, dispL, sL, psL, sG, gch, scaled);
+    const WlsPlan plan = plan_wls(h, g, n_pairs, dispL, sL, psL, view, sG, psG, gch, scaled);
     const bool wave = plan.wave;
     h->last_solver = wave ? ADF_SOLVER_WAVE : ADF_SOLVER_EXACT;
     if ((rc = h->ws.reserve(plan.per_pair * (size_t)plan.chunk, st, FILL_ZERO))) return rc;
@@ -545,7 +567,7 @@
     const int rrx = W - (roi.x + roi.width);
     const int thresh = (int)(1.0f * h->lrc_thresh);
     Profiler* prof = &h->prof;
-    h->last_path = plan.path;
+    h->last_path = plan.path; h->last_solver_path = plan.solver_path;
 
     for (int first = 0; first < n_pairs; first += plan.chunk) {
         const int n = (n_pairs - first < plan.chunk) ? n_pairs - first : plan.chunk;
@@ -559,8 +581,9 @@
         OutsideArgs oa{o, sO, psO, fill, om.f32 ? 1 : 0, scaled ? nullptr : confp, g};
         const double ob = ((oa.conf ? 4.0 : 0.0) + ob_px) * (F - P);
         auto fill_outside = [&](hipStream_t s) { ProfScope ps(prof, K_FILL, ob, ob, s); return launch_outside(oa, n, s); };
-        WeightArgs wa{gv, sG, psG, gch, h->lut.cur, p.CH, p.CV, orient_h, orient_cv, g,
+        WeightArgs wa{gv, sG, psG, gch, h->lut.cur, cp.guide_rows ? nullptr : p.CH, p.CV, orient_h, orient_cv, g,
                       wave ? nullptr : p.B0};
+        const GuideWeights gw = guide_weights(h, gv, sG, psG, gch, g);
         ConfBandArgs ba{dL, sL, psL, dR, sR, psR, confp, g, rrx, thresh, h->disc_radius, h->roll_off, 0};
         DiscArgs da{{dL, dR}, {sL, sR}, {psL, psR}, {roi.x, rrx}, roi.y, roi.width, roi.height, h->disc_radius, h->roll_off,
                     {cL, cR}, W, g.frame, cp.stage == CONF_LEFT ? 1 : -1};
@@ -576,7 +599,8 @@
         if (cp.stage == CONF_NONE || cp.outside_on_side) HIP_TRY(fill_outside(wst));
         if (cp.stage == CONF_NONE && scaled && first == 0 && (rc = scaled_resize(h, *scaled, st, prof))) return rc;
         if (cp.stage != CONF_MERGED) {
-            ProfScope ps(prof, K_WEIGHTS, (gch + 8.0) * P, (gch + 8.0) * P, wst);
+            const double wb = (gch + (cp.guide_rows ? 4.0 : 8.0)) * P;
+            ProfScope ps(prof, K_WEIGHTS, wb, wb, wst);
             HIP_TRY(launch_weights(wa, n, wst));
         }
         if (cp.fork_weights) HIP_TRY(hipEventRecord(h->ev_join, h->side));
@@ -649,7 +673,7 @@
         const int epi = conf ? (om.f32 ? EPI_WLS_CONF_F32 : EPI_WLS_CONF) : (om.f32 ? EPI_F32 : EPI_I16);
         FinalOut fo{epi, o, sO, psO, roi.x, roi.y, 1, 0};
         rc = run_passes(wave, g, p, conf ? 2 : 1, (float)h->lambda, (float)h->atten, h->num_iter, fo, n, st, prof,
-                        plan.fused_first ? &fuse : nullptr);
+                        plan.fused_first ? &fuse : nullptr, cp.guide_rows ? &gw : nullptr);
         if (rc) return rc;
     }
     return ADF_OK;
diff --git a/addingdisparityfiltering_amd/csrc/adf_internal.h b/addingdisparityfiltering_amd/csrc/adf_internal.h
--- a/addingdisparityfiltering_amd/csrc/adf_internal.h
+++ b/addingdisparityfiltering_amd/csrc/adf_internal.h
@@ -125,6 +125,12 @@
     float* lo_taps;
 };
 
+struct GuideWeights {
+    const uint8_t* guide; ptrdiff_t stride, pair_stride;
+    int ch, x0, y0;
+    const float* lut;
+};
+
 struct WavePassArgs {
     const float* C; float* U0; float* U1;
     FusedInputs fuse;
@@ -133,9 +139,11 @@
     int nscan, len, pitch;
     size_t plane;
     float lambda;
-};
-static_assert(sizeof(WavePassArgs) == 280 && offsetof(WavePassArgs, out) == 208 && offsetof(WavePassArgs, nscan) == 248 &&
-              offsetof(WavePassArgs, plane) == 264 && offsetof(WavePassArgs, lambda) == 272, "WavePassArgs layout");
+    GuideWeights gw;
+};
+static_assert(sizeof(WavePassArgs) == 328 && offsetof(WavePassArgs, out) == 208 && offsetof(WavePassArgs, nscan) == 248 &&
+              offsetof(WavePassArgs, plane) == 264 && offsetof(WavePassArgs, lambda) == 272 && offsetof(WavePassArgs, gw) == 280 &&
+              sizeof(GuideWeights) == 48, "WavePassArgs layout");
 
 hipError_t launch_discontinuity(const DiscArgs& a, int n_pairs, hipStream_t st);
 hipError_t launch_lrc_prologue(const LrcArgs& a, int n_pairs, hipStream_t st);
@@ -149,6 +157,7 @@
 int conf_left_max_radius();
 hipError_t launch_plain_prologue(const PlainPrologueArgs& a, int n_pairs, hipStream_t st);
 hipError_t launch_weights(const WeightArgs& a, int n_pairs, hipStream_t st);
+bool weights_stream_fits(const WeightArgs& a);
 hipError_t launch_resize_linear(const ResizeArgs& a, int n_pairs, hipStream_t st);
 hipError_t launch_exact_pass(const PassArgs& a, int n_rhs, int epilogue, int n_pairs, hipStream_t st);
 hipError_t launch_wave_hpass(const WavePassArgs& a, int n_rhs, int n_pairs, hipStream_t st);
@@ -157,6 +166,7 @@
 bool wave_hpass_can_fuse(const WavePassArgs& a);
 bool wave_hpass_can_fuse_lo(const WavePassArgs& a);
 bool wave_hpass_lo_half(const WavePassArgs& a);
+bool wave_hpass_guide_fits(const WavePassArgs& a);
 int wave_max_col_len();
 int max_disc_radius();
 
diff --git a/addingdisparityfiltering_amd/csrc/fgs_wave_h.hip b/addingdisparityfiltering_amd/csrc/fgs_wave_h.hip
--- a/addingdisparityfiltering_amd/csrc/fgs_wave_h.hip
+++ b/addingdisparityfiltering_amd/csrc/fgs_wave_h.hip
@@ -1,4 +1,5 @@
 #include "fgs_wave_common.h"
+#include "prep_bodies.h"
 
 #include <algorithm>
 
@@ -10,6 +11,7 @@
 constexpr int H_TWO_WAVE_MAX = 60;
 
 constexpr int FUSE_NONE = 0, FUSE_VIEW = 1, FUSE_LO = 2, FUSE_LO_HALF = 3;
+constexpr int WS_PLANE = 0, WS_GUIDE1 = 1, WS_GUIDE3 = 3;
 
 typedef float v4f __attribute__((ext_vector_type(4)));
 
@@ -61,7 +63,7 @@
     return t;
 }
 
-template <int M, int R>
+template <int M, int R, bool WITH_C>
 __device__ __forceinline__ void load_planes(const WavePassArgs& a, const RowPos& p, float4 (&tC)[M / 4], float4 (&t0)[M / 4], float4 (&t1)[M / 4])
 {
     constexpr bool PAIR = R > 1;
@@ -71,7 +73,7 @@
 #pragma unroll
     for (int k = 0; k < MQ; k++) {
         const int uidx = u0 + 64 * k + p.lane;
-        tC[k] = load_c(a, p, k);
+        if constexpr (WITH_C) tC[k] = load_c(a, p, k);
         t0[k] = make_float4(0.f, 0.f, 0.f, 0.f); t1[k] = t0[k];
         if (uidx < p.nvecU) t0[k] = load_nt(s0 + rhs_vec<PAIR>(uidx));
         if (PAIR && uidx + 64 * MQ < p.nvecU) t1[k] = load_nt(s0 + rhs_vec<PAIR>(uidx + 64 * MQ));
@@ -80,7 +82,7 @@
 
 __device__ __forceinline__ int fused_vecs(int len) { return (len >> 2) + ((len & 3) ? 1 : 0); }
 
-template <int M>
+template <int M, bool WITH_C>
 __device__ __forceinline__ void load_fused_view(const WavePassArgs& a, const RowPos& p, float4 (&tC)[M / 4], float4 (&t0)[M / 4], float4 (&t1)[M / 4])
 {
     constexpr int MQ = M / 4;
@@ -96,7 +98,7 @@
 #pragma unroll
     for (int k = 0; k < MQ; k++) {
         const int idx = p.v0 + 64 * k + p.lane;
-        tC[k] = load_c(a, p, k);
+        if constexpr (WITH_C) tC[k] = load_c(a, p, k);
         t0[k] = make_float4(0.f, 0.f, 0.f, 0.f); t1[k] = t0[k];
         draw[k] = make_short4(0, 0, 0, 0);
         if (idx < nfused) {
@@ -376,6 +378,128 @@
     }
 }
 
+constexpr int GW_HEAD = 1024;
+
+template <int M, int CH>
+struct GuideShape {
+    static constexpr int NV = (CH * (64 * M + 1) + 15 + 1023) / 1024;
+    static constexpr int ND = (CH * (M + 1) + 3 + 3) / 4;
+    static constexpr int NH = GW_HEAD / 256;
+    static_assert(NV * 1024 <= 256 * M, "the guide vectors fit the wave's staging buffer");
+    static_assert(4 * (3 + 63 * (CH * M / 4) + ND) <= 256 * M, "the last lane reads inside the staging buffer");
+};
+template <int M, int CH>
+struct GuideRaw { prep::ws_v4u g[GuideShape<M, CH>::NV]; prep::ws_v4f h[GuideShape<M, CH>::NH]; unsigned mis; };
+template <int M>
+struct GuideRaw<M, WS_PLANE> {};
+
+template <int M, int CH>
+__device__ __forceinline__ void guide_fetch(const WavePassArgs& a, int lane, GuideRaw<M, CH>& q)
+{
+    const uintptr_t row = reinterpret_cast<uintptr_t>(a.gw.guide) + (uintptr_t)((ptrdiff_t)blockIdx.y * a.gw.pair_stride +
+                          (ptrdiff_t)(a.gw.y0 + (int)blockIdx.x) * a.gw.stride + (ptrdiff_t)a.gw.x0 * CH);
+    q.mis = (unsigned)__builtin_amdgcn_readfirstlane((int)(row & 15u));
+    const __amdgpu_buffer_rsrc_t win = prep::ws_window(reinterpret_cast<const void*>(row - q.mis), (q.mis + (unsigned)a.len * CH + 3u) & ~3u);
+#pragma unroll
+    for (int k = 0; k < GuideShape<M, CH>::NV; k++)
+        q.g[k] = __builtin_amdgcn_raw_buffer_load_b128(win, (unsigned)(64 * k + lane) * 16u, 0, 2 );
+#pragma unroll
+    for (int k = 0; k < GuideShape<M, CH>::NH; k++)
+        q.h[k] = reinterpret_cast<const prep::ws_v4f*>(a.gw.lut)[64 * k + lane];
+}
+
+template <int M, bool FAR>
+__device__ __forceinline__ void guide_finish(const float* head, int lim, float lambda, float (&c)[M])
+{
+#pragma unroll
+    for (int i = 0; i < M; i++) {
+        const unsigned u = __float_as_uint(c[i]);
+        float w = head[min(u, (unsigned)(GW_HEAD - 1))];
+        if (FAR) {
+            asm volatile("" : "+v"(w));
+            w = (int)u < 0 ? c[i] : w;
+        }
+        c[i] = (i < lim ? w : 0.0f) * lambda;
+    }
+}
+
+template <int M, int CH>
+__device__ __forceinline__ void guide_weights(const WavePassArgs& a, float4* stage, float* head, int lane, const GuideRaw<M, CH>& q, float (&c)[M])
+{
+    typedef GuideShape<M, CH> S;
+#pragma unroll
+    for (int k = 0; k < S::NH; k++) reinterpret_cast<prep::ws_v4f*>(head)[64 * k + lane] = q.h[k];
+#pragma unroll
+    for (int k = 0; k < S::NV; k++) reinterpret_cast<prep::ws_v4u*>(stage)[64 * k + lane] = q.g[k];
+    __syncthreads();
+    if (lane == 0) {
+        unsigned char* B = reinterpret_cast<unsigned char*>(stage) + q.mis + (unsigned)(a.len - 1) * CH;
+#pragma unroll
+        for (int ci = 0; ci < CH; ci++) B[CH + ci] = B[ci];
+    }
+    __syncthreads();
+    const unsigned* L = reinterpret_cast<const unsigned*>(stage) + (q.mis >> 2) + lane * (CH * M / 4);
+    const unsigned mb = q.mis & 3u;
+    unsigned d[S::ND];
+#pragma unroll
+    for (int j = 0; j < S::ND; j++) d[j] = L[j];
+    auto e = [&](int j) -> unsigned { return __builtin_amdgcn_alignbyte(j + 1 < S::ND ? d[j + 1 < S::ND ? j + 1 : 0] : 0u, d[j], mb); };
+    int far = 0;
+    if constexpr (CH == 3) {
+        unsigned p[5], pa[5];
+        p[4] = e(0) & 0x00ffffffu; pa[4] = prep::ws_norm2(p[4]);
+#pragma unroll
+        for (int g = 0; g < M / 4; g++) {
+            prep::ws_unpack3(e(3 * g), e(3 * g + 1), e(3 * g + 2), p);
+            pa[0] = pa[4];
+            p[4] = e(3 * g + 3) & 0x00ffffffu;
+#pragma unroll
+            for (int k = 1; k <= 4; k++) pa[k] = prep::ws_norm2(p[k]);
+#pragma unroll
+            for (int k = 0; k < 4; k++) {
+                const int idx = prep::ws_dist2(p[k], pa[k], p[k + 1], pa[k + 1]);
+                far = max(far, idx);
+                c[4 * g + k] = __int_as_float(idx);
+            }
+        }
+    } else {
+#pragma unroll
+        for (int g = 0; g < M / 4; g++) {
+            const unsigned eg = e(g), nb = e(g + 1) & 0xffu;
+#pragma unroll
+            for (int k = 0; k < 4; k++) {
+                const int v = (int)((eg >> (8 * k)) & 0xffu);
+                const int r = k < 3 ? (int)((eg >> (8 * k + 8)) & 0xffu) : (int)nb;
+                const int idx = prep::ws_dist2_c1(v, r);
+                far = max(far, idx);
+                c[4 * g + k] = __int_as_float(idx);
+            }
+        }
+    }
+    const int lim = a.len - 1 - lane * M;
+    if (__builtin_amdgcn_ballot_w64(far >= GW_HEAD) != 0) {
+        const __amdgpu_buffer_rsrc_t lutwin = prep::ws_window(a.gw.lut, sizeof(float) * ADF_LUT_LEVELS);
+        constexpr int G = 16;
+#pragma unroll
+        for (int i0 = 0; i0 < M; i0 += G) {
+            unsigned w[G];
+#pragma unroll
+            for (int k = 0; k < G; k++)
+                if (i0 + k < M) {
+                    const int idx = __float_as_int(c[i0 + k]);
+                    w[k] = __builtin_amdgcn_raw_buffer_load_b32(lutwin, idx >= GW_HEAD ? (unsigned)idx * 4u : prep::WS_DROP, 0, 0);
+                }
+#pragma unroll
+            for (int k = 0; k < G; k++)
+                if (i0 + k < M) c[i0 + k] = w[k] != 0u ? __uint_as_float(w[k]) : c[i0 + k];
+        }
+        guide_finish<M, true>(head, lim, a.lambda, c);
+    } else {
+        guide_finish<M, false>(head, lim, a.lambda, c);
+    }
+    __syncthreads();
+}
+
 template <int M>
 __device__ __forceinline__ void transpose_in(float4* stage, int lane, const float4 (&t)[M / 4], float (&dst)[M], float scale)
 {
@@ -451,13 +575,16 @@
     }
 }
 
-template <int M, int R, int FUSED, int NW = 1>
+template <int M, int R, int FUSED, int NW = 1, int WS = WS_PLANE>
 __global__ void __launch_bounds__(64 * NW, (M > (NW == 2 ? 40 : H_TWO_WAVE_MAX) && R > 1) ? 1 : 2) wave_hpass_kernel(WavePassArgs a)
 {
     static_assert(M % 4 == 0 && M >= 4, "chunk length must be a multiple of 4");
     static_assert(NW == 1 || NW == 2, "one or two wavefronts per row");
     constexpr bool LO = FUSED == FUSE_LO || FUSED == FUSE_LO_HALF;
     constexpr bool PAIR = R > 1;
+    constexpr bool GUIDE = WS != WS_PLANE;
+    static_assert(!GUIDE || (NW == 1 && !LO), "the guide forms: one-wave rows whose prologue leaves the staging buffer alone");
+    __shared__ __attribute__((aligned(16))) float lut_head[GUIDE ? GW_HEAD : 1];
     __shared__ float4 stage_all[NW][LO ? lo_stage_vec4(M) : M * 16];
     __shared__ float xch[NW == 2 ? 5 : 1];
     __shared__ float red[NW == 2 ? 5 : 1][NW == 2 ? 128 : 1];
@@ -467,12 +594,15 @@
     float4* stage = stage_all[wv];
 
     float4 tC[M / 4], t0[M / 4], t1[M / 4];
+    GuideRaw<M, WS> tG;
+    if constexpr (GUIDE) guide_fetch<M, WS>(a, lane, tG);
     if constexpr (LO) load_fused_lo<M, FUSED == FUSE_LO_HALF>(a, p, stage, tC, t0, t1);
-    else if constexpr (FUSED == FUSE_VIEW) load_fused_view<M>(a, p, tC, t0, t1);
-    else load_planes<M, R>(a, p, tC, t0, t1);
+    else if constexpr (FUSED == FUSE_VIEW) load_fused_view<M, !GUIDE>(a, p, tC, t0, t1);
+    else load_planes<M, R, !GUIDE>(a, p, tC, t0, t1);
 
     float c[M], f0[M], f1[M];
-    transpose_in<M>(stage, lane, tC, c, a.lambda);
+    if constexpr (GUIDE) guide_weights<M, WS>(a, stage, lut_head, lane, tG, c);
+    else transpose_in<M>(stage, lane, tC, c, a.lambda);
     if constexpr (PAIR && FUSED == FUSE_NONE) {
         pair_in<M>(stage, lane, t0, 0, f0, f1);
         pair_in<M>(stage, lane, t1, 1, f0, f1);
@@ -529,10 +659,30 @@
 
 constexpr bool lo_half_bucket(int m, int nw) { return !(m == 60 && nw == 1); }
 
+constexpr bool guide_bucket(int nw) { return nw == 1; }
+
+template <int M, int WS>
+hipError_t launch_h_guide(const WavePassArgs& a, int n_rhs, dim3 grid, hipStream_t st)
+{
+    if (a.fuse.conf_in) {
+        if (n_rhs != 2) return hipErrorInvalidValue;
+        hipLaunchKernelGGL((wave_hpass_kernel<M, 2, FUSE_VIEW, 1, WS>), grid, dim3(64), 0, st, a);
+    } else if (n_rhs == 2) hipLaunchKernelGGL((wave_hpass_kernel<M, 2, FUSE_NONE, 1, WS>), grid, dim3(64), 0, st, a);
+    else hipLaunchKernelGGL((wave_hpass_kernel<M, 1, FUSE_NONE, 1, WS>), grid, dim3(64), 0, st, a);
+    return hipGetLastError();
+}
+
 template <int M, int NW = 1>
 hipError_t launch_h(const WavePassArgs& a, int n_rhs, int n_pairs, hipStream_t st)
 {
     dim3 grid(a.nscan, n_pairs), block(64 * NW);
+    if (a.gw.guide) {
+        if constexpr (guide_bucket(NW)) {
+            if (a.gw.ch == 1) return launch_h_guide<M, WS_GUIDE1>(a, n_rhs, grid, st);
+            if (a.gw.ch == 3) return launch_h_guide<M, WS_GUIDE3>(a, n_rhs, grid, st);
+        }
+        return hipErrorInvalidValue;
+    }
     if (a.fuse.lo_conf) {
         if (n_rhs != 2 || !a.fuse.lo_taps) return hipErrorInvalidValue;
         const int n = ((a.len + 3) / 4) * 4;
@@ -572,6 +722,16 @@
     if ((reinterpret_cast<uintptr_t>(a.fuse.conf_in) & 15u) != 0) return false;
     if (a.fuse.dl_stride % 2 != 0 || a.fuse.dl_pair_stride % 2 != 0 || (reinterpret_cast<uintptr_t>(a.fuse.dl_in) & 1u) != 0) return false;
     return true;
+}
+
+bool wave_hpass_guide_fits(const WavePassArgs& a)
+{
+    if (!a.gw.guide || !a.gw.lut || (a.gw.ch != 1 && a.gw.ch != 3) || a.fuse.lo_conf) return false;
+    if ((reinterpret_cast<uintptr_t>(a.gw.lut) & 15u) != 0 || a.gw.x0 < 0 || a.gw.y0 < 0) return false;
+    if (a.len < 2 || a.len > wave_max_row_len()) return false;
+    int m, nw;
+    pick_row_bucket(a.len, m, nw);
+    return guide_bucket(nw);
 }
 
 bool wave_hpass_lo_half(const WavePassArgs& a)
@@ -609,6 +769,7 @@
     if (a.len < 2 || a.len > wave_max_row_len() || a.pitch % 64 != 0 || a.pitch < a.len) return hipErrorInvalidValue;
     if (a.fuse.lo_conf && !wave_hpass_can_fuse_lo(a)) return hipErrorInvalidValue;
     if (!a.fuse.lo_conf && a.fuse.conf_in && !wave_hpass_can_fuse(a)) return hipErrorInvalidValue;
+    if (a.gw.guide && !wave_hpass_guide_fits(a)) return hipErrorInvalidValue;
     return dispatch_index<N_ROW_BUCKETS>(bucket_index(ROW_BUCKETS, a.len), [&](auto I) {
         constexpr Bucket b = ROW_BUCKETS[decltype(I)::value];
         return launch_h<b.m, b.chunks / 64>(a, n_rhs, n_pairs, st);
diff --git a/addingdisparityfiltering_amd/csrc/prep_bodies.h b/addingdisparityfiltering_amd/csrc/prep_bodies.h
--- a/addingdisparityfiltering_amd/csrc/prep_bodies.h
+++ b/addingdisparityfiltering_amd/csrc/prep_bodies.h
@@ -42,37 +42,48 @@
     return gd;
 }
 
-template <int CH>
+template <int CH, bool HOR>
 __device__ __forceinline__ WsWin<CH> ws_load(const WsGuide& gd, unsigned wo)
 {
     WsWin<CH> w;
     if constexpr (CH == 3) {
         w.a = __builtin_amdgcn_raw_buffer_load_b128(gd.rsrc, wo, 0, 0);
-        w.b = __builtin_amdgcn_raw_buffer_load_b32(gd.rsrc, wo + 16u, 0, 0);
+        w.b = HOR ? __builtin_amdgcn_raw_buffer_load_b32(gd.rsrc, wo + 16u, 0, 0) : 0u;
     } else {
         w.a = __builtin_amdgcn_raw_buffer_load_b64(gd.rsrc, wo, 0, 0);
     }
     return w;
 }
 
-template <int CH>
+__device__ __forceinline__ void ws_unpack3(unsigned e0, unsigned e1, unsigned e2, unsigned* p)
+{
+    p[0] = e0 & 0x00ffffffu;
+    p[1] = __builtin_amdgcn_perm(e1, e0, 0x0c050403u);
+    p[2] = __builtin_amdgcn_perm(e2, e1, 0x0c040302u);
+    p[3] = e2 >> 8;
+}
+__device__ __forceinline__ unsigned ws_norm2(unsigned p) { return __builtin_amdgcn_udot4(p, p, 0u, false); }
+__device__ __forceinline__ int ws_dist2(unsigned p, unsigned pa, unsigned q, unsigned qa)
+{
+    return (int)(pa + qa) - 2 * (int)__builtin_amdgcn_udot4(p, q, 0u, false);
+}
+__device__ __forceinline__ int ws_dist2_c1(int v, int r) { return (v - r) * (v - r); }
+
+template <int CH, bool HOR>
 __device__ __forceinline__ void ws_indices(const WsWin<CH>& w, unsigned m, WsPrev<CH>& pv, int (&hidx)[WS_COLS], int (&vidx)[WS_COLS])
 {
     if constexpr (CH == 3) {
         const unsigned e0 = __builtin_amdgcn_alignbyte(w.a.y, w.a.x, m), e1 = __builtin_amdgcn_alignbyte(w.a.z, w.a.y, m);
         const unsigned e2 = __builtin_amdgcn_alignbyte(w.a.w, w.a.z, m), e3 = __builtin_amdgcn_alignbyte(w.b, w.a.w, m);
         unsigned p[WS_COLS + 1], pa[WS_COLS + 1];
-        p[0] = e0 & 0x00ffffffu;
-        p[1] = __builtin_amdgcn_perm(e1, e0, 0x0c050403u);
-        p[2] = __builtin_amdgcn_perm(e2, e1, 0x0c040302u);
-        p[3] = e2 >> 8;
+        ws_unpack3(e0, e1, e2, p);
         p[4] = e3 & 0x00ffffffu;
 #pragma unroll
-        for (int k = 0; k <= WS_COLS; k++) pa[k] = __builtin_amdgcn_udot4(p[k], p[k], 0u, false);
+        for (int k = 0; k <= WS_COLS; k++) pa[k] = ws_norm2(p[k]);
 #pragma unroll
         for (int k = 0; k < WS_COLS; k++) {
-            hidx[k] = (int)(pa[k] + pa[k + 1]) - 2 * (int)__builtin_amdgcn_udot4(p[k], p[k + 1], 0u, false);
-            vidx[k] = (int)(pa[k] + pv.qa[k]) - 2 * (int)__builtin_amdgcn_udot4(p[k], pv.q[k], 0u, false);
+            hidx[k] = HOR ? ws_dist2(p[k], pa[k], p[k + 1], pa[k + 1]) : 0;
+            vidx[k] = ws_dist2(p[k], pa[k], pv.q[k], pv.qa[k]);
             pv.q[k] = p[k]; pv.qa[k] = pa[k];
         }
     } else {
@@ -83,8 +94,8 @@
             const int v = (int)((e >> (8 * k)) & 0xffu);
             const int r = k < WS_COLS - 1 ? (int)((e >> (8 * k + 8)) & 0xffu) : (int)nb;
             const int u = (int)((pv.q[0] >> (8 * k)) & 0xffu);
-            hidx[k] = (v - r) * (v - r);
-            vidx[k] = (u - v) * (u - v);
+            hidx[k] = HOR ? ws_dist2_c1(v, r) : 0;
+            vidx[k] = ws_dist2_c1(u, v);
         }
         pv.q[0] = e;
     }
@@ -101,25 +112,27 @@
 constexpr unsigned WS_DROP = 0x80000000u;
 
 struct WsPending { float wl[2 * WS_COLS]; unsigned g[2 * WS_COLS]; };
+template <bool HOR>
 __device__ __forceinline__ void ws_lookup_issue(const float* lut_head, const __amdgpu_buffer_rsrc_t& lutwin, const int (&hidx)[WS_COLS],
                                                 const int (&vidx)[WS_COLS], WsPending& p)
 {
 #pragma unroll
     for (int k = 0; k < WS_COLS; k++) {
-        p.wl[k] = lut_head[min(hidx[k], WS_LUT_HEAD - 1)];
+        p.wl[k] = HOR ? lut_head[min(hidx[k], WS_LUT_HEAD - 1)] : 0.0f;
         p.wl[WS_COLS + k] = lut_head[min(vidx[k], WS_LUT_HEAD - 1)];
     }
 #pragma unroll
     for (int k = 0; k < WS_COLS; k++) {
-        p.g[k] = __builtin_amdgcn_raw_buffer_load_b32(lutwin, hidx[k] >= WS_LUT_HEAD ? (unsigned)hidx[k] * 4u : WS_DROP, 0, 0);
+        p.g[k] = HOR ? __builtin_amdgcn_raw_buffer_load_b32(lutwin, hidx[k] >= WS_LUT_HEAD ? (unsigned)hidx[k] * 4u : WS_DROP, 0, 0) : 0u;
         p.g[WS_COLS + k] = __builtin_amdgcn_raw_buffer_load_b32(lutwin, vidx[k] >= WS_LUT_HEAD ? (unsigned)vidx[k] * 4u : WS_DROP, 0, 0);
     }
 }
+template <bool HOR>
 __device__ __forceinline__ void ws_lookup_finish(const WsPending& p, float (&wh)[WS_COLS], float (&wv)[WS_COLS])
 {
 #pragma unroll
     for (int k = 0; k < WS_COLS; k++) {
-        wh[k] = p.g[k] != 0u ? __uint_as_float(p.g[k]) : p.wl[k];
+        wh[k] = !HOR ? 0.0f : p.g[k] != 0u ? __uint_as_float(p.g[k]) : p.wl[k];
         wv[k] = p.g[WS_COLS + k] != 0u ? __uint_as_float(p.g[WS_COLS + k]) : p.wl[WS_COLS + k];
     }
 }
@@ -129,7 +142,7 @@
     __device__ __forceinline__ void init(const WeightArgs& a, size_t pz, int j0, int y_first)
     {
         const Geom& g = a.g;
-        chor = ws_window(a.chor + pz * g.plane, g.plane * sizeof(float));
+        chor = ws_window(a.chor ? a.chor + pz * g.plane : a.chor, a.chor ? g.plane * sizeof(float) : 0);
         cvert = ws_window(a.cvert + pz * g.plane, g.plane * sizeof(float));
         strip = a.cvert_orient == ORIENT_STRIP;
 #pragma unroll
@@ -159,7 +172,7 @@
     }
 };
 
-template <int CH>
+template <int CH, bool HOR = true>
 __device__ __forceinline__ void weights_stream_body(const WeightArgs& a, int bx, int by, int nby, size_t pz, WsShared<CH>& sh, bool active)
 {
     static_assert(CH == 1 || CH == 3, "guides have one or three channels");
@@ -183,7 +196,7 @@
     const unsigned col_off = gd.mis + (unsigned)((g.rx + x0) * CH);
     const unsigned lane_off = (unsigned)(tid * WS_COLS * CH);
     auto row_off = [&](int n) -> unsigned { return col_off + (unsigned)(min(y0 + n, g.rh - 1) - y0) * gd.stride; };
-    auto load = [&](int n) -> WsWin<CH> { return ws_load<CH>(gd, (row_off(n) & ~3u) + lane_off); };
+    auto load = [&](int n) -> WsWin<CH> { return ws_load<CH, HOR>(gd, (row_off(n) & ~3u) + lane_off); };
 
     WsOut out;
     out.init(a, pz, j0, y0);
@@ -197,8 +210,8 @@
     WsPending pend;
     {
         int hidx[WS_COLS], vidx[WS_COLS];
-        ws_indices<CH>(nxt[0], row_off(0) & 3u, pv, hidx, vidx);
-        ws_lookup_issue(lut_head, lutwin, hidx, vidx, pend);
+        ws_indices<CH, HOR>(nxt[0], row_off(0) & 3u, pv, hidx, vidx);
+        ws_lookup_issue<HOR>(lut_head, lutwin, hidx, vidx, pend);
     }
     for (int n0 = 0; n0 < nrows; n0 += WS_U) {
 #pragma unroll
@@ -214,12 +227,12 @@
             WsPending ahead;
             {
                 int hidx[WS_COLS], vidx[WS_COLS];
-                ws_indices<CH>(s + 1 < WS_U ? cur[s + 1 < WS_U ? s + 1 : 0] : nxt[0], row_off(min(n + 1, nrows - 1)) & 3u, pv, hidx, vidx);
-                ws_lookup_issue(lut_head, lutwin, hidx, vidx, ahead);
+                ws_indices<CH, HOR>(s + 1 < WS_U ? cur[s + 1 < WS_U ? s + 1 : 0] : nxt[0], row_off(min(n + 1, nrows - 1)) & 3u, pv, hidx, vidx);
+                ws_lookup_issue<HOR>(lut_head, lutwin, hidx, vidx, ahead);
             }
             float wh[WS_COLS], wv[WS_COLS];
-            ws_lookup_finish(pend, wh, wv);
-            out.store_h(n, wh, n < nrows - 1);
+            ws_lookup_finish<HOR>(pend, wh, wv);
+            if constexpr (HOR) out.store_h(n, wh, n < nrows - 1);
             out.store_v(n - 1, wv, y0 + n - 1 == g.rh - 1, n >= 1 && n < nrows);
             pend = ahead;
         }
diff --git a/addingdisparityfiltering_amd/csrc/weights_kernels.hip b/addingdisparityfiltering_amd/csrc/weights_kernels.hip
--- a/addingdisparityfiltering_amd/csrc/weights_kernels.hip
+++ b/addingdisparityfiltering_amd/csrc/weights_kernels.hip
@@ -96,11 +96,11 @@
     }
 }
 
-template <int CH>
+template <int CH, bool HOR>
 __global__ void __launch_bounds__(prep::WS_NT) weights_stream_kernel(WeightArgs a)
 {
     __shared__ prep::WsShared<CH> sh;
-    prep::weights_stream_body<CH>(a, blockIdx.x, blockIdx.y, gridDim.y, blockIdx.z, sh, true);
+    prep::weights_stream_body<CH, HOR>(a, blockIdx.x, blockIdx.y, gridDim.y, blockIdx.z, sh, true);
 }
 
 __global__ void __launch_bounds__(256) transpose_n_to_t_kernel(const float* __restrict__ src, float* __restrict__ dst, Geom g)
@@ -130,8 +130,15 @@
 
 }
 
+bool weights_stream_fits(const WeightArgs& a)
+{
+    static const bool force_generic = [] { const char* e = getenv("ADF_WEIGHTS_GENERIC"); return e && atoi(e) != 0; }();
+    return !force_generic && a.chor_orient == ORIENT_N && a.stride > 0 && a.stride < ((ptrdiff_t)1 << 29) && (size_t)a.g.W * a.ch < ((size_t)1 << 29);
+}
+
 hipError_t launch_weights(const WeightArgs& a, int n_pairs, hipStream_t st)
 {
+    const bool hor = a.chor != nullptr;
     if (a.chor_orient == ORIENT_T && a.cvert_orient == ORIENT_N && a.scratch) {
         WeightArgs b = a;
         b.chor = a.scratch; b.chor_orient = ORIENT_N; b.scratch = nullptr;
@@ -142,8 +149,7 @@
         return hipGetLastError();
     }
     if (a.cvert_orient != ORIENT_N && !(a.cvert_orient == ORIENT_STRIP && a.chor_orient == ORIENT_N)) return hipErrorInvalidValue;
-    static const bool force_generic = [] { const char* e = getenv("ADF_WEIGHTS_GENERIC"); return e && atoi(e) != 0; }();
-    if (!force_generic && a.chor_orient == ORIENT_N && a.stride > 0 && a.stride < ((ptrdiff_t)1 << 29) && (size_t)a.g.W * a.ch < ((size_t)1 << 29)) {
+    if (weights_stream_fits(a)) {
         dim3 sgrid((a.g.rw + prep::WS_BCOLS - 1) / prep::WS_BCOLS, 1, n_pairs);
         {
             int rpb = 128;
@@ -152,11 +158,14 @@
             while (rpb > 1 && (size_t)(rpb + 1) * (size_t)a.stride >= ((size_t)1 << 30)) rpb >>= 1;
             sgrid.y = (a.g.rh + rpb - 1) / rpb;
         }
-        if (a.ch == 1) hipLaunchKernelGGL(weights_stream_kernel<1>, sgrid, dim3(prep::WS_NT), 0, st, a);
-        else if (a.ch == 3) hipLaunchKernelGGL(weights_stream_kernel<3>, sgrid, dim3(prep::WS_NT), 0, st, a);
+        if (a.ch == 1 && hor) hipLaunchKernelGGL((weights_stream_kernel<1, true>), sgrid, dim3(prep::WS_NT), 0, st, a);
+        else if (a.ch == 1) hipLaunchKernelGGL((weights_stream_kernel<1, false>), sgrid, dim3(prep::WS_NT), 0, st, a);
+        else if (a.ch == 3 && hor) hipLaunchKernelGGL((weights_stream_kernel<3, true>), sgrid, dim3(prep::WS_NT), 0, st, a);
+        else if (a.ch == 3) hipLaunchKernelGGL((weights_stream_kernel<3, false>), sgrid, dim3(prep::WS_NT), 0, st, a);
         else return hipErrorInvalidValue;
         return hipGetLastError();
     }
+    if (!hor) return hipErrorInvalidValue;
     dim3 grid((a.g.rw + TX - 1) / TX, (a.g.rh + TY - 1) / TY, n_pairs);
     if (a.ch == 1) hipLaunchKernelGGL(weights_kernel<1>, grid, dim3(NT), 0, st, a);
     else if (a.ch == 3) hipLaunchKernelGGL(weights_kernel<3>, grid, dim3(NT), 0, st, a);
diff --git a/addingdisparityfiltering_amd/ximgproc.py b/addingdisparityfiltering_amd/ximgproc.py
--- a/addingdisparityfiltering_amd/ximgproc.py
+++ b/addingdisparityfiltering_amd/ximgproc.py
@@ -5,7 +5,7 @@
 
 from . import _lib
 from ._lib import SGBM_COST_BT, SGBM_COST_CENSUS_DENSE, SGBM_COST_CENSUS_SPARSE
-from ._lib import AdfError, PATH_CONF_BAND, PATH_FUSED_FIRST_PASS, PATH_MERGED_PREP, PATH_SCALED_FUSED, PATH_SCALED_HALF, Rect, SOLVER_EXACT, SOLVER_WAVE
+from ._lib import AdfError, PATH_CONF_BAND, PATH_FUSED_FIRST_PASS, PATH_MERGED_PREP, PATH_ROW_WEIGHTS_GUIDE, PATH_SCALED_FUSED, PATH_SCALED_HALF, Rect, SOLVER_EXACT, SOLVER_WAVE
 
 try:
     import torch
@@ -187,6 +187,9 @@
 
     def getLastPath(self):
         return _read(_lib.lib().adf_wls_get_last_path, C.c_int, self._h)
+
+    def getLastSolverPath(self):
+        return _read(_lib.lib().adf_wls_get_last_solver_path, C.c_int, self._h)
 
     def enableProfiling(self, on=True):
         _lib.check(_lib.lib().adf_wls_profile_enable(self._h, int(bool(on))))
diff --git a/include/adf_wls.h b/include/adf_wls.h
--- a/include/adf_wls.h
+++ b/include/adf_wls.h
@@ -57,6 +57,8 @@
 #define ADF_PATH_SCALED_FUSED 8
 #define ADF_PATH_SCALED_HALF 16
 int adf_wls_get_last_path(const adf_wls_t* h, int* path_flags);
+#define ADF_PATH_ROW_WEIGHTS_GUIDE 32
+int adf_wls_get_last_solver_path(const adf_wls_t* h, int* path_flags);
 
 int adf_wls_filter_device(adf_wls_t* h, int n_pairs,
                           const int16_t* disp_left, ptrdiff_t disp_left_stride, ptrdiff_t disp_left_pair_stride,
```

New measurement: 42400 (median of 6 runs). 1.04x the previous value.
